# YunjiKim/Unsupervised-Keypoint-Learning-for-Guiding-Class-conditional-Video-Prediction

Measured on AMD Instinct MI355X. Metric: detector_translator train frames/sec @128x128 K=15, higher is better.
Workload: dtype f32

## Files before the change

### include/kpx.h

```cpp
#ifndef KPX_H
#define KPX_H

#include <stddef.h>
#include <stdint.h>

#ifdef __cplusplus
extern "C" {
#endif

#define KPX_EINVAL (-1)
#define KPX_ABI_VERSION 15

enum { KPX_ACT_NONE = 0, KPX_ACT_RELU = 1, KPX_ACT_LRELU = 2 , KPX_ACT_TANH = 3  };

int kpx_abi_version(void);

int kpx_reload_env(void);

enum { KPX_ARITH_F32 = 0, KPX_ARITH_BF16 = 1 };

size_t kpx_conv2d_fwd_workspace_bytes(int N, int Ho, int Wo, int Cin, int Cout, int KH, int KW);
int kpx_conv2d_fwd_f32(const float* x, int N, int Hi, int Wi, int Cin, int ldx,
                       const float* w_hwio, int KH, int KW, const float* bias,
                       float* y, int Ho, int Wo, int Cout, int ldy,
                       int stride, int pad_t, int pad_l, int act, int arith,
                       void* workspace, size_t workspace_bytes, void* stream);

typedef struct KpxWinoDesc { const float* w; float* u; int cin, cout, dgrad, reserved; } KpxWinoDesc;
size_t kpx_wino_u_bytes(int Cin, int Cout);
int kpx_wino_filter_transform_f32(const float* w_hwio, int Cin, int Cout, int dgrad, float* u, void* stream);
int kpx_wino_filter_transform_batch_f32(const void* descs, int n, void* stream);
int kpx_conv3x3_wino_eligible(int N, int H, int W, int K, int Nn, int ldin, const void* in);
int kpx_conv3x3_wino_f32(const float* in, int N, int H, int W, int K, int ldin, const float* u, const float* bias,
                         float* out, int Nn, int ldout, int act, float* tile_stats, const float* bn_y, int ld_bn_y,
                         const float* bn_beta, void* stream);
size_t kpx_conv3x3_wino_stats_tiles(int N, int H, int W);

size_t kpx_conv3x3_bf16s_weights_bytes(int K, int Nn);
int kpx_conv3x3_bf16s_eligible(int N, int H, int W, int K, int Nn, int ldin, const void* in);
int kpx_conv3x3_bf16s_stats_tiles(int N, int H, int W, int K, int Nn);
int kpx_conv3x3_bf16s_prepare_f32(const float* w_hwio, int Cin, int Cout, int dgrad, void* wf, void* stream);
int kpx_conv3x3_bf16s_prepare_batch_f32(const void* table, int ndesc, void* stream);
int kpx_conv3x3_bf16s(const void* in, int N, int H, int W, int K, int ldin, const void* wf, const float* bias,
                      void* out, int Nn, int ldout, int out_f32, int act, const void* mask, int ldmask, float* stats, void* stream);
int kpx_conv3x3_bf16s_bnbwd(const void* in, int N, int H, int W, int K, int ldin, const void* wf, void* out, int Nn, int ldout,
                            const void* bn_y, int ld_bn_y, const float* beta, float* stats, void* stream);

size_t kpx_conv2d_dgrad_workspace_bytes(int N, int Hi, int Wi, int Cin, int Cout, int KH, int KW, int stride);
int kpx_conv2d_dgrad_f32(const float* dy, int N, int Ho, int Wo, int Cout, int lddy,
                         const float* w_hwio, int KH, int KW,
                         float* dx, int Hi, int Wi, int Cin, int lddx,
                         int stride, int pad_t, int pad_l, int arith,
                         void* workspace, size_t workspace_bytes, void* stream);

int kpx_conv2d_dgrad_act_f32(const float* dy, int N, int Ho, int Wo, int Cout, int lddy,
                             const float* w_hwio, int KH, int KW,
                             float* dx, int Hi, int Wi, int Cin, int lddx,
                             int stride, int pad_t, int pad_l, int arith,
                             const float* y_in, int ld_y_in, int act_in,
                             void* workspace, size_t workspace_bytes, void* stream);

size_t kpx_conv2d_wgrad_workspace_bytes(int N, int Ho, int Wo, int Cin, int Cout, int KH, int KW);
int kpx_conv2d_wgrad_f32(const float* x, int N, int Hi, int Wi, int Cin, int ldx,
                         const float* dy, int Ho, int Wo, int Cout, int lddy,
                         float* dw_hwio, int KH, int KW, int stride, int pad_t, int pad_l, int arith,
                         void* workspace, size_t workspace_bytes, void* stream);

enum KpxWgradFamily {
    KPX_WGRAD_WSMALL = 0,
    KPX_WGRAD_WINO,
    KPX_WGRAD_ROWS_MERGED,
    KPX_WGRAD_ROWS,
    KPX_WGRAD_GEMM3,
    KPX_WGRAD_TAP_ROWS,
    KPX_WGRAD_GENERIC
};
int kpx_conv2d_wgrad_plan(const float* x, int N, int Hi, int Wi, int Cin, int ldx,
                          const float* dy, int Ho, int Wo, int Cout, int lddy,
                          int KH, int KW, int stride, int pad_t, int pad_l, int arith,
                          int* family, int* splits, size_t* workspace_bytes);

int kpx_act_bwd_f32(const float* dy, const float* y, float* dz, size_t n, int act, void* stream);

size_t kpx_chan_reduce_scratch_bytes(int C);
int kpx_chan_sum_f32(const float* x, size_t P, int C, int ldx, float* sum_out, void* scratch, void* stream);

size_t kpx_bn_train_scratch_bytes(int C, int groups);
int kpx_bn_train_fwd_f32(const float* x, size_t P, int groups, int C, int ldx, const float* tile_stats, size_t tiles_per_group,
                         float eps, const float* gamma, const float* beta, float* mean, float* invstd,
                         float* moving_mean, float* moving_var, float decay, float* y, int ldy, int act, void* scratch, void* stream);
int kpx_bn_train_bwd_f32(const float* dy, int lddy, const float* x, int ldx, size_t P, int groups, int C,
                         const float* mean, const float* invstd, const float* gamma, const float* beta, int act,
                         float* dx, int lddx, float* dgamma, float* dbeta, int accumulate,
                         const float* tile_stats, size_t tiles_per_group, void* scratch, void* stream);
int kpx_bn_train_fwd_bf16(const void* x, size_t P, int groups, int C, int ldx, const float* tile_stats, size_t tiles_per_group,
                          float eps, const float* gamma, const float* beta, float* mean, float* invstd,
                          float* moving_mean, float* moving_var, float decay, void* y, int ldy, int y_f32, int act, void* scratch, void* stream);
int kpx_bn_train_bwd_bf16(const void* dy, int lddy, int dy_f32, const void* x, int ldx, size_t P, int groups, int C,
                          const float* mean, const float* invstd, const float* gamma, const float* beta, int act,
                          void* dx, int lddx, float* dgamma, float* dbeta, int accumulate,
                          const float* tile_stats, size_t tiles_per_group, void* scratch, void* stream);
int kpx_bn_invstd_f32(const float* var, int C, float eps, float* invstd, void* stream);
int kpx_bn_apply_f32(const float* x, size_t P, int C, int ldx, const float* mean, const float* invstd,
                     const float* gamma, const float* beta, float* y, int ldy, int act, void* stream);
int kpx_bn_fold_conv_f32(const float* w, const float* bias, size_t rows, int C, const float* gamma, const float* beta,
                         const float* moving_mean, const float* moving_var, float eps, float* w_out, float* b_out, void* stream);

int kpx_conv3x3_wino43_eligible(int N, int H, int W, int K, int Nn, int ldin, const void* in_ptr);
size_t kpx_wino43_u_bytes(int Cin, int Cout);
int kpx_wino43_filter_transform_f32(const float* w_hwio, int Cin, int Cout, int dgrad, float* u, void* stream);
int kpx_wino43_filter_transform_batch_f32(const void* descs_dev, int n, void* stream);
int kpx_conv3x3_wino43_f32(const float* in, int N, int H, int W, int K, int ldin, const float* u, const float* bias,
                           float* out, int Nn, int ldout, int act, const float* mask_y, int ld_mask, float* pool_y, int ld_pool,
                           float* tile_stats, const float* bn_y, int ld_bn_y, const float* bn_beta, void* stream);
size_t kpx_conv3x3_wino43_stats_tiles(int N, int H, int W);
int kpx_conv3x3_wino43b_eligible(int N, int H, int W, int K, int Nn, int ldin, const void* in_ptr);
size_t kpx_wino43b_u_bytes(int Cin, int Cout);
int kpx_wino43b_filter_transform_f32(const float* w_hwio, int Cin, int Cout, int dgrad, void* u, void* stream);
int kpx_wino43b_filter_transform_batch_f32(const void* descs_dev, int n, void* stream);
int kpx_conv3x3_wino43b_f32(const float* in, int N, int H, int W, int K, int ldin, const void* u, const float* bias,
                            float* out, int Nn, int ldout, int act, const float* mask_y, int ld_mask, float* pool_y, int ld_pool,
                            float* tile_stats, const float* bn_y, int ld_bn_y, const float* bn_beta, void* stream);
int kpx_conv3x3_c16_eligible(int N, int H, int W, int K, int Nn, int ldin, int ldout, const void* in_ptr);
int kpx_conv3x3_c16_f32(const float* in, int N, int H, int W, int K, int ldin, const float* w_hwio, int dgrad, const float* bias,
                        float* out, int ldout, int act, float* tile_stats, void* stream);
int kpx_resize2x_fwd_f32(const float* x, int N, int H, int W, int C, int ldx, float* y, int ldy, void* stream);
int kpx_resize2x_bwd_f32(const float* dy, int N, int H, int W, int C, int lddy, float* dx, int lddx, void* stream);

int kpx_copy_channels_f32(const float* src, int ldsrc, float* dst, int lddst, size_t P, int C, void* stream);

size_t kpx_keypoint_head_scratch_bytes(int B, int H, int W, int K);
int kpx_keypoint_head_fwd_f32(const float* logits, int B, int H, int W, int K,
                              float* mu, float* prob_y, float* prob_x, void* scratch, void* stream);
int kpx_keypoint_head_bwd_f32(const float* dmu, const float* mu, const float* prob_y, const float* prob_x,
                              int B, int H, int W, int K, float* dlogits, void* stream);

size_t kpx_keypoint_head_proj_scratch_bytes(int B, int H, int W, int C, int K);
int kpx_keypoint_head_proj_eligible(int B, int H, int W, int C, int K);
int kpx_keypoint_head_proj_fwd_f32(const float* x, const float* wk, const float* bias, int B, int H, int W, int C, int K,
                                   float* mu, float* prob_y, float* prob_x, float* xs_y, float* xs_x, void* scratch, void* stream);
int kpx_keypoint_head_proj_bwd_f32(const float* dmu, const float* mu, const float* prob_y, const float* prob_x,
                                   const float* xs_y, const float* xs_x, const float* wk, int B, int H, int W, int C, int K,
                                   float* dx, float* dw, float* db, int accumulate, void* scratch, void* stream);

int kpx_gaussian_maps_fwd_f32(const float* mu, int B, int K, int H, int W, double inv_std, float* maps, int ldy, void* stream);
int kpx_gaussian_maps_bwd_f32(const float* dmaps, int lddy, const float* mu, int B, int K, int H, int W, double inv_std,
                              float* dmu, void* stream);

int kpx_point_maps_rgb_f32(const float* mu, int N, int K, int H, int W, double inv_std, const float* colors, float* out, void* stream);

int kpx_point_seq_strip_rgb_f32(const float* mu, int N, int T, int K, int H, int W, double inv_std, const float* colors, int recolour,
                                float* out, void* stream);

#define KPX_SUMMARY_SLICES 64
enum { KPX_PREMAP_IDENTITY = 0, KPX_PREMAP_X255 = 1, KPX_PREMAP_UNIT255 = 2, KPX_PREMAP_UNIT255_CLIP = 3 };
int kpx_summary_image_u8_f32(const float* x, int N, int H, int W, int C, int premap, float* work, uint8_t* out, void* stream);

int kpx_frame_metrics_f32(const float* a, const float* b, int N, int H, int W, int C, float L, int png8, float* out, void* stream);

size_t kpx_feature_pair_metrics_workspace_bytes(int N, int H, int W, int C);
int kpx_feature_pair_metrics_f32(const float* fa, const float* fb, int N, int H, int W, int C, float* work, float* out, void* stream);

int kpx_draw_moments_add_f32(const float* x, size_t n, uint32_t* sum, uint32_t* sumsq, void* stream);
int kpx_draw_diversity_f32(const uint32_t* sum, const uint32_t* sumsq, int N, int H, int W, int C, int D, float* div_mse ,
                           uint8_t* std_map , void* stream);
int kpx_keypoint_draw_metrics_f32(const float* pts , const float* real , int D, int N, int T, int K,
                                  float* l2 , float* div , void* stream);

#define KPX_SHEET_MAX_FRAMES 64
enum { KPX_SHEET_UNIT = 0, KPX_SHEET_RAW = 1 };
int kpx_sheet_paste_u8_f32(const float* src , int B, int F, int H, int W, int C, const int* frames , int J,
                           uint8_t* canvas , int rows, int cols, int row, int col, int premap, void* stream);

enum { KPX_RETARGET_HOLD = 0, KPX_RETARGET_ABSOLUTE = 1, KPX_RETARGET_RELATIVE = 2, KPX_RETARGET_RELATIVE_SCALED = 3 };
int kpx_points_retarget_f32(const float* src_first , const float* drv_first , const float* drv_seq ,
                            int B, int T, int K, int shift, int mode, float* out , void* stream);

int kpx_head_blend_fwd_f32(const float* im, const float* raw4, size_t P, float* final_out, float* crude_out, float* mask_out, void* stream);
int kpx_head_blend_bwd_f32(const float* dfinal, const float* im, const float* raw4, size_t P, float* draw4, void* stream);

int kpx_vgg_prep_fwd_f32(const float* rgb, size_t P, float* bgr, void* stream);
int kpx_vgg_prep_bwd_f32(const float* dbgr, size_t P, float* drgb, void* stream);
int kpx_vgg_prep_png8_f32(const float* rgb, size_t P, float* bgr, void* stream);

int kpx_maxpool2_fwd_f32(const float* x, int N, int H, int W, int C, float* y, void* stream);
int kpx_maxpool2_bwd_f32(const float* dy, const float* x, int N, int H, int W, int C, float* dx, void* stream);

int kpx_l1_pair_fwd_f32(const float* f, size_t half, float* loss_out, void* scratch, void* stream);
int kpx_l1_pair_bwd_f32(const float* f, size_t half, const float* gscale_dev, float gscale_host, float* dpred, void* stream);
int kpx_vgg_feat_bwd_f32(const float* f, size_t half, const float* gscale_dev, float gscale_host, const float* dy_pooled,
                         int B, int H, int W, int C, float* d, void* stream);

int kpx_sigmoid_xent_fwd_f32(const float* logits, size_t n0, float label0, size_t n1, float label1, float* loss_out, void* stream);
int kpx_sigmoid_xent_bwd_f32(const float* logits, size_t n0, float label0, size_t n1, float label1,
                             const float* gscale_dev, float gscale_host, float* dlogits, void* stream);

int kpx_adam_tf_flat_f32(float* p, const float* g, float* m, float* v, size_t n,
                         float alpha, float beta1, float beta2, float eps, float gscale, void* stream);
int kpx_adam_tf_flat_dev_alpha_f32(float* p, const float* g, float* m, float* v, size_t n,
                                   const float* alpha_dev, float beta1, float beta2, float eps, float gscale, void* stream);

int kpx_lstm_pointwise_f32(const float* gates, const float* c_prev, float forget_bias, float* c_out, float* h_out,
                           int B, int U, void* stream);
int kpx_tile_batch_f32(const float* src, int ldsrc, int B, int T, int pix, int C, float* dst, int lddst, void* stream);
int kpx_head_blend_tiled_fwd_f32(const float* im, const float* raw4, size_t P, int HW, int T, int clip,
                                 float* final_out, float* crude_out, float* mask_out, void* stream);

int kpx_fill_f32(float* p, size_t n, float value, void* stream);
int kpx_axpy_f32(float* y, const float* x, size_t n, float a, void* stream);

int kpx_lstm_pointwise_bwd_f32(const float* gates, const float* c_prev, const float* dh, const float* dc_in, float forget_bias,
                               float* dgates, float* dc_prev, int B, int U, void* stream);
int kpx_lstm_layer_fwd_f32(const float* x, int T, int B, int In, const float* kernel, const float* bias, int U,
// ... 78 lines not shown
```

### unsupervised-keypoint-learning-for-guiding-class-conditional-video-prediction_amd/_lib.py

```python
import ctypes
import os
from ctypes import c_double, c_float, c_int, c_size_t, c_void_p

import torch

_HERE = os.path.dirname(os.path.abspath(__file__))
LIB_PATH = os.environ.get('KPX_LIB') or os.path.join(_HERE, 'libkpx_hip.so')


class KpxError(RuntimeError):
    pass


if not os.path.exists(LIB_PATH):
    raise ImportError(
        'libkpx_hip.so not found at %s -- build it first: python -c "import __graft_entry__ as g; g.build()" '
        '(or `make -C %s/csrc`). There is no CPU / PyTorch fallback for the hot path.' % (LIB_PATH, _HERE))

lib = ctypes.CDLL(LIB_PATH)

P = c_void_p
ABI_VERSION = 15
SIGNATURES = {
    'kpx_abi_version': (c_int, []),
    'kpx_reload_env': (c_int, []),
    'kpx_conv2d_fwd_workspace_bytes': (c_size_t, [c_int, c_int, c_int, c_int, c_int, c_int, c_int]),
    'kpx_conv2d_fwd_f32': (c_int, [P, c_int, c_int, c_int, c_int, c_int, P, c_int, c_int, P,
                                   P, c_int, c_int, c_int, c_int, c_int, c_int, c_int, c_int, c_int, P, c_size_t, P]),
    'kpx_conv2d_dgrad_workspace_bytes': (c_size_t, [c_int, c_int, c_int, c_int, c_int, c_int, c_int, c_int]),
    'kpx_conv2d_dgrad_f32': (c_int, [P, c_int, c_int, c_int, c_int, c_int, P, c_int, c_int,
                                     P, c_int, c_int, c_int, c_int, c_int, c_int, c_int, c_int, P, c_size_t, P]),
    'kpx_conv2d_dgrad_act_f32': (c_int, [P, c_int, c_int, c_int, c_int, c_int, P, c_int, c_int,
                                         P, c_int, c_int, c_int, c_int, c_int, c_int, c_int, c_int, P, c_int, c_int, P, c_size_t, P]),
    'kpx_conv2d_wgrad_workspace_bytes': (c_size_t, [c_int, c_int, c_int, c_int, c_int, c_int, c_int]),
    'kpx_conv2d_wgrad_f32': (c_int, [P, c_int, c_int, c_int, c_int, c_int, P, c_int, c_int, c_int, c_int,
                                     P, c_int, c_int, c_int, c_int, c_int, c_int, P, c_size_t, P]),
    'kpx_conv2d_wgrad_plan': (c_int, [P, c_int, c_int, c_int, c_int, c_int, P, c_int, c_int, c_int, c_int,
                                      c_int, c_int, c_int, c_int, c_int, c_int, P, P, P]),
    'kpx_wino_u_bytes': (c_size_t, [c_int, c_int]),
    'kpx_wino_filter_transform_f32': (c_int, [P, c_int, c_int, c_int, P, P]),
    'kpx_wino_filter_transform_batch_f32': (c_int, [P, c_int, P]),
    'kpx_conv3x3_wino_eligible': (c_int, [c_int, c_int, c_int, c_int, c_int, c_int, P]),
    'kpx_conv3x3_wino_f32': (c_int, [P, c_int, c_int, c_int, c_int, c_int, P, P, P, c_int, c_int, c_int, P, P, c_int, P, P]),
    'kpx_conv3x3_c16_eligible': (c_int, [c_int, c_int, c_int, c_int, c_int, c_int, c_int, P]),
    'kpx_conv3x3_c16_f32': (c_int, [P, c_int, c_int, c_int, c_int, c_int, P, c_int, P, P, c_int, c_int, P, P]),
    'kpx_conv3x3_wino43_eligible': (c_int, [c_int, c_int, c_int, c_int, c_int, c_int, P]),
    'kpx_wino43_u_bytes': (c_size_t, [c_int, c_int]),
    'kpx_wino43_filter_transform_f32': (c_int, [P, c_int, c_int, c_int, P, P]),
    'kpx_wino43_filter_transform_batch_f32': (c_int, [P, c_int, P]),
    'kpx_conv3x3_wino43_f32': (c_int, [P, c_int, c_int, c_int, c_int, c_int, P, P, P, c_int, c_int, c_int, P, c_int, P, c_int, P, P, c_int, P, P]),
    'kpx_conv3x3_wino43b_eligible': (c_int, [c_int, c_int, c_int, c_int, c_int, c_int, P]),
    'kpx_wino43b_u_bytes': (c_size_t, [c_int, c_int]),
    'kpx_wino43b_filter_transform_f32': (c_int, [P, c_int, c_int, c_int, P, P]),
    'kpx_wino43b_filter_transform_batch_f32': (c_int, [P, c_int, P]),
    'kpx_conv3x3_wino43b_f32': (c_int, [P, c_int, c_int, c_int, c_int, c_int, P, P, P, c_int, c_int, c_int, P, c_int, P, c_int, P, P, c_int, P, P]),
    'kpx_conv3x3_wino43_stats_tiles': (c_size_t, [c_int, c_int, c_int]),
    'kpx_conv3x3_wino_stats_tiles': (c_size_t, [c_int, c_int, c_int]),
    'kpx_conv3x3_bf16s_weights_bytes': (c_size_t, [c_int, c_int]),
    'kpx_conv3x3_bf16s_eligible': (c_int, [c_int, c_int, c_int, c_int, c_int, c_int, P]),
    'kpx_conv3x3_bf16s_stats_tiles': (c_int, [c_int, c_int, c_int, c_int, c_int]),
    'kpx_conv3x3_bf16s_prepare_f32': (c_int, [P, c_int, c_int, c_int, P, P]),
    'kpx_conv3x3_bf16s_prepare_batch_f32': (c_int, [P, c_int, P]),
    'kpx_conv3x3_bf16s': (c_int, [P, c_int, c_int, c_int, c_int, c_int, P, P, P, c_int, c_int, c_int, c_int, P, c_int, P, P]),
    'kpx_conv2d_fwd_bf16': (c_int, [P, c_int, c_int, c_int, c_int, c_int, P, c_int, c_int, P, P, c_int, c_int, c_int, c_int, c_int, c_int, c_int, c_int, c_int, P, c_size_t, P]),
    'kpx_conv2d_dgrad_bf16': (c_int, [P, c_int, c_int, c_int, c_int, c_int, P, c_int, c_int, P, c_int, c_int, c_int, c_int, c_int, c_int, c_int, c_int, P, c_int, c_int, P, c_size_t, P]),
    'kpx_conv2d_wgrad_bf16': (c_int, [P, c_int, c_int, c_int, c_int, c_int, P, c_int, c_int, c_int, c_int, P, c_int, c_int, c_int, c_int, c_int, P, c_size_t, P]),
    'kpx_conv_image_fwd_bf16': (c_int, [P, c_int, c_int, c_int, c_int, P, c_int, c_int, P, P, c_int, c_int, c_int, c_int, c_int, c_int, c_int, c_int, P]),
    'kpx_conv_image_dgrad_bf16': (c_int, [P, c_int, c_int, c_int, c_int, c_int, P, c_int, c_int, P, c_int, c_int, c_int, c_int, c_int, c_int, c_int, P]),
    'kpx_conv_image_wgrad_bf16': (c_int, [P, c_int, c_int, c_int, c_int, c_int, P, c_int, c_int, c_int, c_int, P, c_int, c_int, c_int, c_int, c_int, P, c_size_t, P]),
    'kpx_conv3x3_wgrad_bf16_eligible': (c_int, [c_int, c_int, c_int, c_int, c_int, c_int, c_int, P, P]),
    'kpx_conv3x3_wgrad_bf16_workspace_bytes': (c_size_t, [c_int, c_int, c_int, c_int, c_int]),
    'kpx_conv3x3_wgrad_bf16': (c_int, [P, c_int, c_int, c_int, c_int, c_int, P, c_int, c_int, P, P, c_size_t, P]),
    'kpx_conv3x3_bf16s_bnbwd': (c_int, [P, c_int, c_int, c_int, c_int, c_int, P, P, c_int, c_int, P, c_int, P, P, P]),
    'kpx_cast_channels': (c_int, [P, c_int, P, c_int, c_size_t, c_int, c_int, P]),
    'kpx_chan_sum_bf16': (c_int, [P, c_size_t, c_int, c_int, P, P, P]),
    'kpx_bn_train_fwd_bf16': (c_int, [P, c_size_t, c_int, c_int, c_int, P, c_size_t, c_float, P, P, P, P, P, P, c_float, P, c_int, c_int, c_int, P, P]),
    'kpx_bn_train_bwd_bf16': (c_int, [P, c_int, c_int, P, c_int, c_size_t, c_int, c_int, P, P, P, P, c_int, P, c_int, P, P, c_int, P, c_size_t, P, P]),
    'kpx_act_bwd_bf16': (c_int, [P, P, P, c_size_t, c_int, P]),
    'kpx_resize2x_fwd_bf16': (c_int, [P, c_int, c_int, c_int, c_int, c_int, P, c_int, P]),
    'kpx_resize2x_bwd_bf16': (c_int, [P, c_int, c_int, c_int, c_int, c_int, P, c_int, P]),
    'kpx_maxpool2_fwd_bf16': (c_int, [P, c_int, c_int, c_int, c_int, P, P]),
    'kpx_vgg_feat_bwd_bf16': (c_int, [P, c_size_t, P, c_float, P, c_int, c_int, c_int, c_int, P, P]),
    'kpx_l1_pair_fwd_bf16': (c_int, [P, c_size_t, P, P, P]),
    'kpx_act_bwd_f32': (c_int, [P, P, P, c_size_t, c_int, P]),
    'kpx_chan_reduce_scratch_bytes': (c_size_t, [c_int]),
    'kpx_chan_sum_f32': (c_int, [P, c_size_t, c_int, c_int, P, P, P]),
    'kpx_bn_invstd_f32': (c_int, [P, c_int, c_float, P, P]),
    'kpx_bn_fold_conv_f32': (c_int, [P, P, c_size_t, c_int, P, P, P, P, c_float, P, P, P]),
    'kpx_bn_train_scratch_bytes': (c_size_t, [c_int, c_int]),
    'kpx_bn_train_fwd_f32': (c_int, [P, c_size_t, c_int, c_int, c_int, P, c_size_t, c_float, P, P, P, P, P, P, c_float, P, c_int, c_int, P, P]),
    'kpx_bn_train_bwd_f32': (c_int, [P, c_int, P, c_int, c_size_t, c_int, c_int, P, P, P, P, c_int, P, c_int, P, P, c_int, P, c_size_t, P, P]),
    'kpx_bn_apply_f32': (c_int, [P, c_size_t, c_int, c_int, P, P, P, P, P, c_int, c_int, P]),
    'kpx_resize2x_fwd_f32': (c_int, [P, c_int, c_int, c_int, c_int, c_int, P, c_int, P]),
    'kpx_resize2x_bwd_f32': (c_int, [P, c_int, c_int, c_int, c_int, c_int, P, c_int, P]),
    'kpx_copy_channels_f32': (c_int, [P, c_int, P, c_int, c_size_t, c_int, P]),
    'kpx_keypoint_head_scratch_bytes': (c_size_t, [c_int, c_int, c_int, c_int]),
    'kpx_keypoint_head_fwd_f32': (c_int, [P, c_int, c_int, c_int, c_int, P, P, P, P, P]),
    'kpx_keypoint_head_bwd_f32': (c_int, [P, P, P, P, c_int, c_int, c_int, c_int, P, P]),
    'kpx_keypoint_head_proj_scratch_bytes': (c_size_t, [c_int, c_int, c_int, c_int, c_int]),
    'kpx_keypoint_head_proj_eligible': (c_int, [c_int, c_int, c_int, c_int, c_int]),
    'kpx_keypoint_head_proj_fwd_f32': (c_int, [P, P, P, c_int, c_int, c_int, c_int, c_int, P, P, P, P, P, P, P]),
    'kpx_keypoint_head_proj_bwd_f32': (c_int, [P, P, P, P, P, P, P, c_int, c_int, c_int, c_int, c_int, P, P, P, c_int, P, P]),
    'kpx_gaussian_maps_fwd_f32': (c_int, [P, c_int, c_int, c_int, c_int, c_double, P, c_int, P]),
    'kpx_gaussian_maps_bwd_f32': (c_int, [P, c_int, P, c_int, c_int, c_int, c_int, c_double, P, P]),
    'kpx_point_maps_rgb_f32': (c_int, [P, c_int, c_int, c_int, c_int, c_double, P, P, P]),
    'kpx_point_seq_strip_rgb_f32': (c_int, [P, c_int, c_int, c_int, c_int, c_int, c_double, P, c_int, P, P]),
    'kpx_summary_image_u8_f32': (c_int, [P, c_int, c_int, c_int, c_int, c_int, P, P, P]),
    'kpx_frame_metrics_f32': (c_int, [P, P, c_int, c_int, c_int, c_int, c_float, c_int, P, P]),
    'kpx_feature_pair_metrics_workspace_bytes': (c_size_t, [c_int, c_int, c_int, c_int]),
    'kpx_feature_pair_metrics_f32': (c_int, [P, P, c_int, c_int, c_int, c_int, P, P, P]),
    'kpx_draw_moments_add_f32': (c_int, [P, c_size_t, P, P, P]),
    'kpx_draw_diversity_f32': (c_int, [P, P, c_int, c_int, c_int, c_int, c_int, P, P, P]),
    'kpx_keypoint_draw_metrics_f32': (c_int, [P, P, c_int, c_int, c_int, c_int, P, P, P]),
    'kpx_sheet_paste_u8_f32': (c_int, [P, c_int, c_int, c_int, c_int, c_int, P, c_int, P, c_int, c_int, c_int, c_int, c_int, P]),
    'kpx_points_retarget_f32': (c_int, [P, P, P, c_int, c_int, c_int, c_int, c_int, P, P]),
    'kpx_head_blend_fwd_f32': (c_int, [P, P, c_size_t, P, P, P, P]),
    'kpx_head_blend_bwd_f32': (c_int, [P, P, P, c_size_t, P, P]),
    'kpx_vgg_prep_fwd_f32': (c_int, [P, c_size_t, P, P]),
    'kpx_vgg_prep_bwd_f32': (c_int, [P, c_size_t, P, P]),
    'kpx_vgg_prep_png8_f32': (c_int, [P, c_size_t, P, P]),
    'kpx_maxpool2_fwd_f32': (c_int, [P, c_int, c_int, c_int, c_int, P, P]),
    'kpx_maxpool2_bwd_f32': (c_int, [P, P, c_int, c_int, c_int, c_int, P, P]),
    'kpx_l1_pair_fwd_f32': (c_int, [P, c_size_t, P, P, P]),
    'kpx_l1_pair_bwd_f32': (c_int, [P, c_size_t, P, c_float, P, P]),
    'kpx_vgg_feat_bwd_f32': (c_int, [P, c_size_t, P, c_float, P, c_int, c_int, c_int, c_int, P, P]),
    'kpx_sigmoid_xent_fwd_f32': (c_int, [P, c_size_t, c_float, c_size_t, c_float, P, P]),
    'kpx_sigmoid_xent_bwd_f32': (c_int, [P, c_size_t, c_float, c_size_t, c_float, P, c_float, P, P]),
    'kpx_adam_tf_flat_f32': (c_int, [P, P, P, P, c_size_t, c_float, c_float, c_float, c_float, c_float, P]),
    'kpx_adam_tf_flat_dev_alpha_f32': (c_int, [P, P, P, P, c_size_t, P, c_float, c_float, c_float, c_float, P]),
    'kpx_lstm_pointwise_f32': (c_int, [P, P, c_float, P, P, c_int, c_int, P]),
    'kpx_tile_batch_f32': (c_int, [P, c_int, c_int, c_int, c_int, c_int, P, c_int, P]),
    'kpx_head_blend_tiled_fwd_f32': (c_int, [P, P, c_size_t, c_int, c_int, c_int, P, P, P, P]),
    'kpx_fill_f32': (c_int, [P, c_size_t, c_float, P]),
    'kpx_axpy_f32': (c_int, [P, P, c_size_t, c_float, P]),
    'kpx_lstm_pointwise_bwd_f32': (c_int, [P, P, P, P, c_float, P, P, c_int, c_int, P]),
    'kpx_lstm_layer_fwd_f32': (c_int, [P, c_int, c_int, c_int, P, P, c_int, P, P, P, P, P, P, c_size_t, P]),
    'kpx_lstm_layer_bwd_f32': (c_int, [P, c_int, c_int, c_int, P, c_int, P, P, P, P, P, P, P, P, P, c_size_t, P]),
    'kpx_vae_sample_kl_fwd_f32': (c_int, [P, P, P, P, c_int, c_int, P]),
    'kpx_vae_sample_kl_bwd_f32': (c_int, [P, P, P, P, c_float, P, c_int, c_int, P]),
    'kpx_u8_to_unit_f32': (c_int, [P, c_size_t, P, P]),
    'kpx_crc32c_host': (ctypes.c_uint, [ctypes.c_uint, P, c_size_t]),
    'kpx_augment_geometry_u8': (c_int, [P, P, P, c_int, P, c_int, P, P, P]),
    'kpx_augment_filter_f32': (c_int, [P, P, P, c_int, P, P, P]),
    'kpx_keypoint_seq_augment_f32': (c_int, [P, P, P, c_int, c_int, c_int, P, P, P, P, P]),
}

for _name, (_res, _args) in SIGNATURES.items():
    try:
        _fn = getattr(lib, _name)
    except AttributeError as e:
        raise ImportError('libkpx_hip.so does not export %s (stale build?)' % _name) from e
    _fn.restype = _res
    _fn.argtypes = _args

if lib.kpx_abi_version() != ABI_VERSION:
    raise ImportError('libkpx_hip.so ABI version mismatch')


abi_calls = [0]


def check(rc, what):
    abi_calls[0] += 1
    if rc != 0:
        raise KpxError('%s failed with code %d (%s)' % (what, rc, 'bad argument' if rc == -1 else 'hipError %d' % -rc))
```

### unsupervised-keypoint-learning-for-guiding-class-conditional-video-prediction_amd/csrc/conv_gemm3.hip

```cpp
#include "kpx_internal.h"
#include "kpx_bf16.h"
#include "kpx_env.h"

#define G3_PITCH 80

template <int BM, int BN, int WM, int WN, bool BT, int TERMS, bool IO16 = false>
__global__ __launch_bounds__(WM * WN * 64, 2) void conv_gemm3_kernel(const ConvGeom g) {
    static_assert(!IO16 || TERMS == 1, "bf16 tensors carry one term");
    constexpr int NT = WM * WN * 64, BK = 32, ESZ = IO16 ? 2 : 4;
    constexpr int TM = BM / (WM * 32), TN = BN / (WN * 32);
    constexpr int APL = BM * G3_PITCH, BPL = BN * G3_PITCH;
    constexpr int ASZ = TERMS * APL;
    constexpr int RA = BM * 4 / NT;
    constexpr int KU = BN * 4 >= NT ? 8 : 4, CW = BN * 4 >= NT ? 4 : 2;
    constexpr int RB = BT ? BN * 32 / KU / NT : 16 * BN / CW / NT;
    static_assert(TM >= 1 && TN >= 1 && BM % (WM * 32) == 0 && BN % (WN * 32) == 0 && RA >= 1 && RB >= 1, "tile shape");
    static_assert(RA * NT == BM * 4 && RB * NT == (BT ? BN * 32 / KU : 16 * BN / CW), "whole units per thread");
    extern __shared__ __attribute__((aligned(16))) unsigned char smem[];
    unsigned char* const Asm = smem;
    unsigned char* const Bsm = smem + ASZ;

    const int t = threadIdx.x, lane = t & 63, wave = t >> 6;
    const int li = lane & 31, lh = lane >> 5;
    const int wm = wave / WN, wn = wave % WN;
    const ConvClass k = g.cls[blockIdx.y];
    const int L = kpx_xcd_remap(blockIdx.x, gridDim.x);
    if (L >= k.mt * g.nt) return;
    const int m0 = (L / g.nt) * BM, n0 = (L % g.nt) * BN;
    const int HW = k.Ha * k.Wa;
    const int wrow = wm * TM * 32, wcol = wn * TN * 32;

    const __amdgpu_buffer_rsrc_t rs_a = __builtin_amdgcn_make_buffer_rsrc(const_cast<float*>(g.x), 0,
                                            (int)((size_t)g.N * g.Hi * g.Wi * g.ldx * ESZ), 0x00020000);
    const size_t w_bytes = (size_t)g.KW * ((size_t)k.wr0 + (size_t)(k.Tr > 0 ? k.Tr - 1 : 0) * g.wrs + 1) * g.wts * 4;
    const __amdgpu_buffer_rsrc_t rs_b = __builtin_amdgcn_make_buffer_rsrc(const_cast<float*>(g.w), 0, (int)(w_bytes < 0x7fffffffu ? w_bytes : 0x7fffffffu), 0x00020000);

    int a_voff[RA], a_st[RA], a_k[RA];
    unsigned a_vm[RA];
#pragma unroll
    for (int i = 0; i < RA; ++i) {
        const int u = t + NT * i, oct = u & 3, row = u >> 2;
        const int m = m0 + row;
        const bool ok = m < k.M;
        const int mm = ok ? m : 0;
        const int n = mm / HW, rem = mm - n * HW, a = rem / k.Wa, b = rem - a * k.Wa;
        const int ih0 = a * g.isy + k.iy0, iw0 = b * g.isx + k.ix0;
        a_voff[i] = ((n * g.Hi * g.Wi + ih0 * g.Wi + iw0) * g.ldx + oct * 8) * ESZ;
        unsigned vm = 0;
        for (int r = 0; r < k.Tr; ++r)
            for (int q = 0; q < k.Tq; ++q)
                if (ok && (unsigned)(ih0 + r * g.ity) < (unsigned)g.Hi && (unsigned)(iw0 + q * g.itx) < (unsigned)g.Wi) vm |= 1u << (r * k.Tq + q);
        a_vm[i] = vm;
        a_st[i] = row * G3_PITCH + oct * 16;
        a_k[i] = oct * 8;
    }
    int b_voff[RB], b_st[RB], b_k[RB];
    bool b_ok[RB];
#pragma unroll
    for (int i = 0; i < RB; ++i) {
        const int u = t + NT * i;
        if (BT) {
            const int ku = u % (32 / KU), nn = u / (32 / KU), n = n0 + nn;
            b_ok[i] = n < g.Cout;
            b_voff[i] = (n * g.ldw + ku * KU) * 4;
            b_st[i] = nn * G3_PITCH + ku * KU * 2;
            b_k[i] = ku * KU;
        } else {
            const int kp = u & 15, nq = u >> 4, n = n0 + nq * CW;
            b_ok[i] = n < g.Cout;
            b_voff[i] = ((kp * 2) * g.ldw + n) * 4;
            b_st[i] = (nq * CW) * G3_PITCH + kp * 4;
            b_k[i] = kp * 2;
        }
    }
    int a_rd[TM], b_rd[TN];
#pragma unroll
    for (int i = 0; i < TM; ++i) a_rd[i] = (wrow + i * 32 + li) * G3_PITCH + lh * 16;
#pragma unroll
    for (int j = 0; j < TN; ++j) b_rd[j] = (wcol + j * 32 + li) * G3_PITCH + lh * 16;

    f32x16 acc[TM][TN];
#pragma unroll
    for (int i = 0; i < TM; ++i)
#pragma unroll
        for (int j = 0; j < TN; ++j)
#pragma unroll
            for (int r = 0; r < 16; ++r) acc[i][j][r] = 0.f;

    const int nck = (g.Cin + BK - 1) / BK;
    int nchunks = k.Tr * k.Tq * nck;
    int tr = 0, tq = 0, c0 = 0;
    if (g.ksplit > 1) {
        const int cps = (nchunks + g.ksplit - 1) / g.ksplit;
        const int cb = blockIdx.z * cps, ce = min(nchunks, cb + cps);
        const int tap0 = cb / nck;
        c0 = (cb - tap0 * nck) * BK; tr = tap0 / k.Tq; tq = tap0 - tr * k.Tq;
        nchunks = ce > cb ? ce - cb : 0;
    }
    int left = nchunks;

    f32x4 ra[RA][2], rb[RB][2];
    auto load_chunk = [&]() {
        const int a_off = (((tr * g.ity) * g.Wi + tq * g.itx) * g.ldx + c0) * ESZ;
        const int tapbit = tr * k.Tq + tq;
        const int tap = (k.wr0 + tr * g.wrs) * g.KW + (k.wq0 + tq * g.wqs);
        const int b_off = (tap * g.wts + (BT ? c0 : c0 * g.ldw)) * 4;
        const bool live = left > 0;
#pragma unroll
        for (int i = 0; i < RA; ++i) {
            const bool va = live & (((a_vm[i] >> tapbit) & 1u) != 0) & (c0 + a_k[i] < g.Cin);
            const int av = va ? a_voff[i] + a_off : KPX_BUF_OOB;
            ra[i][0] = __builtin_bit_cast(f32x4, __builtin_amdgcn_raw_buffer_load_b128(rs_a, av, 0, 0));
            if (!IO16) ra[i][1] = __builtin_bit_cast(f32x4, __builtin_amdgcn_raw_buffer_load_b128(rs_a, av + 16, 0, 0));
        }
#pragma unroll
        for (int i = 0; i < RB; ++i) {
            if (BT) {
                const bool vb = live & b_ok[i] & (c0 + b_k[i] < g.Cin);
                const int bv = vb ? b_voff[i] + b_off : KPX_BUF_OOB;
                rb[i][0] = __builtin_bit_cast(f32x4, __builtin_amdgcn_raw_buffer_load_b128(rs_b, bv, 0, 0));
                if (KU == 8) rb[i][1] = __builtin_bit_cast(f32x4, __builtin_amdgcn_raw_buffer_load_b128(rs_b, bv + 16, 0, 0));
            } else {
#pragma unroll
                for (int j = 0; j < 2; ++j) {
                    const bool vb = live & b_ok[i] & (c0 + b_k[i] + j < g.Cin);
                    const int bv = vb ? b_voff[i] + b_off + j * g.ldw * 4 : KPX_BUF_OOB;
                    if (CW == 4) rb[i][j] = __builtin_bit_cast(f32x4, __builtin_amdgcn_raw_buffer_load_b128(rs_b, bv, 0, 0));
                    else {
                        rb[i][j][0] = __builtin_bit_cast(float, __builtin_amdgcn_raw_buffer_load_b32(rs_b, bv, 0, 0));
                        rb[i][j][1] = __builtin_bit_cast(float, __builtin_amdgcn_raw_buffer_load_b32(rs_b, bv + 4, 0, 0));
                    }
                }
            }
        }
        --left;
        c0 += BK;
        const bool wrap = c0 >= g.Cin;
        c0 = wrap ? 0 : c0;
        tq += wrap ? 1 : 0;
        const bool wrapq = tq == k.Tq;
        tq = wrapq ? 0 : tq;
        tr += wrapq ? 1 : 0;
    };
    auto store_ab = [&]() {
#pragma unroll
        for (int i = 0; i < RA; ++i) {
            unsigned char* const Ab = Asm + a_st[i];
            if (IO16) { *reinterpret_cast<u32x4*>(Ab) = __builtin_bit_cast(u32x4, ra[i][0]); continue; }
            unsigned p[4][3];
            kpx_split2<TERMS>(ra[i][0][0], ra[i][0][1], p[0]); kpx_split2<TERMS>(ra[i][0][2], ra[i][0][3], p[1]);
            kpx_split2<TERMS>(ra[i][1][0], ra[i][1][1], p[2]); kpx_split2<TERMS>(ra[i][1][2], ra[i][1][3], p[3]);
#pragma unroll
            for (int tm = 0; tm < TERMS; ++tm) *reinterpret_cast<u32x4*>(Ab + tm * APL) = u32x4{p[0][tm], p[1][tm], p[2][tm], p[3][tm]};
        }
#pragma unroll
        for (int i = 0; i < RB; ++i) {
            unsigned char* const Bb = Bsm + b_st[i];
            if (BT) {
                unsigned p[4][3];
                kpx_split2<TERMS>(rb[i][0][0], rb[i][0][1], p[0]); kpx_split2<TERMS>(rb[i][0][2], rb[i][0][3], p[1]);
                if (KU == 8) {
                    kpx_split2<TERMS>(rb[i][1][0], rb[i][1][1], p[2]); kpx_split2<TERMS>(rb[i][1][2], rb[i][1][3], p[3]);
#pragma unroll
                    for (int tm = 0; tm < TERMS; ++tm) *reinterpret_cast<u32x4*>(Bb + tm * BPL) = u32x4{p[0][tm], p[1][tm], p[2][tm], p[3][tm]};
                } else {
#pragma unroll
                    for (int tm = 0; tm < TERMS; ++tm) *reinterpret_cast<u32x2*>(Bb + tm * BPL) = u32x2{p[0][tm], p[1][tm]};
                }
            } else {
#pragma unroll
                for (int c = 0; c < CW; ++c) {
                    unsigned p[3];
                    kpx_split2<TERMS>(rb[i][0][c], rb[i][1][c], p);
#pragma unroll
                    for (int tm = 0; tm < TERMS; ++tm) *reinterpret_cast<unsigned*>(Bb + tm * BPL + c * G3_PITCH) = p[tm];
                }
            }
        }
    };

    struct Frag { bf16x8 a[TM][TERMS], b[TN][TERMS]; };
    auto read_frag = [&](int s, Frag& f) {
        const unsigned char* const Ab = Asm + s * 32;
        const unsigned char* const Bb = Bsm + s * 32;
#pragma unroll
        for (int i = 0; i < TM; ++i)
#pragma unroll
            for (int tm = 0; tm < TERMS; ++tm) f.a[i][tm] = *reinterpret_cast<const bf16x8*>(Ab + tm * APL + a_rd[i]);
#pragma unroll
        for (int j = 0; j < TN; ++j)
#pragma unroll
            for (int tm = 0; tm < TERMS; ++tm) f.b[j][tm] = *reinterpret_cast<const bf16x8*>(Bb + tm * BPL + b_rd[j]);
    };
    auto mfma_frag = [&](const Frag& f) {
#pragma unroll
        for (int i = 0; i < TM; ++i)
#pragma unroll
            for (int j = 0; j < TN; ++j) {
                f32x16 c = acc[i][j];
                if (TERMS > 2) {
                    c = __builtin_amdgcn_mfma_f32_32x32x16_bf16(f.a[i][2], f.b[j][0], c, 0, 0, 0);
                    c = __builtin_amdgcn_mfma_f32_32x32x16_bf16(f.a[i][0], f.b[j][2], c, 0, 0, 0);
                    c = __builtin_amdgcn_mfma_f32_32x32x16_bf16(f.a[i][1], f.b[j][1], c, 0, 0, 0);
                }
                if (TERMS > 1) {
                    c = __builtin_amdgcn_mfma_f32_32x32x16_bf16(f.a[i][1], f.b[j][0], c, 0, 0, 0);
                    c = __builtin_amdgcn_mfma_f32_32x32x16_bf16(f.a[i][0], f.b[j][1], c, 0, 0, 0);
                }
                acc[i][j] = __builtin_amdgcn_mfma_f32_32x32x16_bf16(f.a[i][0], f.b[j][0], c, 0, 0, 0);
            }
    };
    auto chunk = [&]() {
        Frag f;
        read_frag(0, f);
        load_chunk();
        mfma_frag(f);
        read_frag(1, f);
        mfma_frag(f);
        __syncthreads();
        store_ab();
        __syncthreads();
    };

    load_chunk();
    store_ab();
    __syncthreads();
    for (int ch = 0; ch < nchunks; ++ch) chunk();

    int* rowpix = reinterpret_cast<int*>(smem);
    if (t < BM) {
        const int m = m0 + t;
        int pix = -1;
        if (m < k.M) {
            const int n = m / HW, rem = m - n * HW, a = rem / k.Wa, b = rem - a * k.Wa;
            pix = (n * g.Ho + a * g.osy + k.oy0) * g.Wo + b * g.osx + k.ox0;
        }
        rowpix[t] = pix;
    }
    __syncthreads();
    if (g.ksplit > 1) {
        float* wsl = g.ws + (size_t)blockIdx.z * g.ws_slab;
#pragma unroll
        for (int n = 0; n < TN; ++n) {
            const int col = n0 + wcol + n * 32 + li;
#pragma unroll
            for (int i = 0; i < TM; ++i)
#pragma unroll
                for (int r = 0; r < 16; ++r) {
                    const int pix = rowpix[wrow + i * 32 + (r & 3) + 8 * (r >> 2) + 4 * lh];
                    if (col < g.Cout && pix >= 0) wsl[(size_t)pix * g.Cout + col] = acc[i][n][r];
                }
        }
        return;
    }
#pragma unroll
    for (int n = 0; n < TN; ++n) {
        const int col = n0 + wcol + n * 32 + li;
        const bool cok = col < g.Cout;
        const float bv = (cok && g.bias) ? g.bias[col] : 0.f;
#pragma unroll
        for (int i = 0; i < TM; ++i) {
#pragma unroll
            for (int r = 0; r < 16; ++r) {
                const int pix = rowpix[wrow + i * 32 + (r & 3) + 8 * (r >> 2) + 4 * lh];
                if (cok && pix >= 0) {
                    float v = acc[i][n][r] + bv;
                    if (g.act == KPX_ACT_RELU) v = fmaxf(v, 0.f);
                    else if (g.act == KPX_ACT_LRELU) v = v > 0.f ? v : 0.01f * v;
                    else if (g.act == KPX_ACT_TANH) v = tanhf(v);
                    if (g.mul_y) {
                        const float my = (g.io16 & 4) ? kpx_float((unsigned)reinterpret_cast<const unsigned short*>(g.mul_y)[(size_t)pix * g.ld_mul + col] << 16)
                                                      : g.mul_y[(size_t)pix * g.ld_mul + col];
                        v *= kpx_act_grad_from_y(my, g.mul_act);
                    }
                    if (g.io16 & 2) { const __bf16 b = (__bf16)v; reinterpret_cast<unsigned short*>(g.y)[(size_t)pix * g.ldy + col] = __builtin_bit_cast(unsigned short, b); }
                    else g.y[(size_t)pix * g.ldy + col] = v;
                }
            }
        }
    }
}

static std::atomic<unsigned long long> g3_attr_mask{0};

template <int BN> struct g3_waves { static constexpr int wm = BN == 128 ? 2 : 4, wn = BN == 128 ? 4 : 2; };
template <int BM, int BN, bool BT, int TERMS, bool IO16 = false>
static int g3_launch_one(const ConvGeom& g, dim3 grid, hipStream_t s) {
    constexpr int lds = TERMS * (BM + BN) * G3_PITCH;
    hipLaunchKernelGGL((conv_gemm3_kernel<BM, BN, g3_waves<BN>::wm, g3_waves<BN>::wn, BT, TERMS, IO16>), grid, dim3(g3_waves<BN>::wm * g3_waves<BN>::wn * 64), lds, s, g);
    return kpx_launch_status();
}
template <int BM, int BN, bool BT, int TERMS, bool IO16 = false>
static hipError_t g3_set_attr() {
    constexpr int lds = TERMS * (BM + BN) * G3_PITCH;
    return hipFuncSetAttribute(reinterpret_cast<const void*>(conv_gemm3_kernel<BM, BN, g3_waves<BN>::wm, g3_waves<BN>::wn, BT, TERMS, IO16>),
                               hipFuncAttributeMaxDynamicSharedMemorySize, lds);
}

extern "C" __attribute__((visibility("hidden"))) int kpx_gemm3_eligible(const ConvGeom* g) {
    const KpxEnv* e = kpx_env();
    if (e->no_gemm3 || g->merge || !g->vecA || !g->vecB) return 0;
    if (g->Cin % 8 != 0 || g->Cin < 16 || g->Cout % 4 != 0 || g->Cout < 16 || g->ldx % 4 != 0 || g->ldw % 4 != 0) return 0;
    if ((g->io16 & 1) && (g->ldx % 8 != 0 || g->terms != 1)) return 0;
    return 1;
}

extern "C" __attribute__((visibility("hidden"))) int kpx_gemm3_launch(ConvGeom g, int bt, int terms, hipStream_t s) {
    if (kpx_first_use_on_device(&g3_attr_mask)) {
        hipError_t e = g3_set_attr<128, 128, false, 3>();
        if (e == hipSuccess) e = g3_set_attr<128, 128, true, 3>();
        if (e == hipSuccess) e = g3_set_attr<128, 64, false, 3>();
        if (e == hipSuccess) e = g3_set_attr<128, 64, true, 3>();
        if (e == hipSuccess) e = g3_set_attr<128, 128, false, 1>();
        if (e == hipSuccess) e = g3_set_attr<128, 128, true, 1>();
        if (e == hipSuccess) e = g3_set_attr<128, 64, false, 1>();
        if (e == hipSuccess) e = g3_set_attr<128, 64, true, 1>();
        if (e == hipSuccess) e = g3_set_attr<128, 128, false, 1, true>();
        if (e == hipSuccess) e = g3_set_attr<128, 128, true, 1, true>();
        if (e == hipSuccess) e = g3_set_attr<128, 64, false, 1, true>();
        if (e == hipSuccess) e = g3_set_attr<128, 64, true, 1, true>();
        if (e != hipSuccess) return -(int)e;
    }
    if (g.ncls <= 0) { g.ncls = 1; g.cls[0] = ConvClass{g.Ha, g.Wa, g.oy0, g.ox0, g.Tr, g.Tq, g.iy0, g.ix0, g.wr0, g.wq0, 0, 0}; }
    g.M = 0;
    for (int i = 0; i < g.ncls; ++i) { g.cls[i].M = g.N * g.cls[i].Ha * g.cls[i].Wa; if (g.cls[i].M > g.M) g.M = g.cls[i].M; }
    if (g.M <= 0 || g.Cout <= 0) return 0;
    const int BM = 128, BN = g.Cout > 64 ? 128 : 64;
    g.nt = (g.Cout + BN - 1) / BN;
    int mtmax = 0;
    for (int i = 0; i < g.ncls; ++i) { g.cls[i].mt = (g.cls[i].M + BM - 1) / BM; if (g.cls[i].mt > mtmax) mtmax = g.cls[i].mt; }
    g.mt = mtmax;
    const dim3 grid((unsigned)(g.mt * g.nt), (unsigned)g.ncls, (unsigned)(g.ksplit > 1 ? g.ksplit : 1));
#define G3_GO(bn, btv, tv) return g3_launch_one<128, bn, btv, tv>(g, grid, s)
    if (g.io16 & 1) {
        if (BN == 128) { if (bt) return g3_launch_one<128, 128, true, 1, true>(g, grid, s); return g3_launch_one<128, 128, false, 1, true>(g, grid, s); }
        if (bt) return g3_launch_one<128, 64, true, 1, true>(g, grid, s);
        return g3_launch_one<128, 64, false, 1, true>(g, grid, s);
    }
    if (terms == 1) {
        if (BN == 128) { if (bt) G3_GO(128, true, 1); else G3_GO(128, false, 1); }
        else { if (bt) G3_GO(64, true, 1); else G3_GO(64, false, 1); }
    }
    if (BN == 128) { if (bt) G3_GO(128, true, 3); else G3_GO(128, false, 3); }
    if (bt) G3_GO(64, true, 3);
    G3_GO(64, false, 3);
#undef G3_GO
}

template <int BM, int WM, int WN, int TERMS, bool IO16 = false>
__global__ __launch_bounds__(WM * WN * 64, 2) void conv_wgrad3_kernel(const WgradGeom g) {
    static_assert(!IO16 || TERMS == 1, "bf16 tensors carry one term");
    constexpr int NT = WM * WN * 64, BKP = 32, BN = BM, ESZ = IO16 ? 2 : 4;
    constexpr int TM = BM / (WM * 32), TN = BN / (WN * 32);
    constexpr int APL = BM * G3_PITCH, BPL = BN * G3_PITCH;
    constexpr int ASZ = TERMS * APL;
    static_assert(NT == 16 * (BM / 4), "one A unit and one B unit (2 pixels x 4 channels) per thread");
    extern __shared__ __attribute__((aligned(16))) unsigned char smem[];
    unsigned char* const Asm = smem;
    unsigned char* const Bsm = smem + ASZ;

    const int t = threadIdx.x, lane = t & 63, wave = t >> 6;
    const int li = lane & 31, lh = lane >> 5;
    const int wm = wave / WN, wn = wave % WN;
    int L = kpx_xcd_remap(blockIdx.x, gridDim.x);
    const int taps = g.KH * g.KW;
    const int kti = L % g.kt; L /= g.kt;
    const int cti = L % g.ct; L /= g.ct;
    const int tap = L % taps; L /= taps;
    const int split = L;
    const int r = tap / g.KW, q = tap - r * g.KW;
    const int cbase = cti * BM, kbase = kti * BN;
    const int pbeg = split * g.pps;
    const int pend = min(g.P, pbeg + g.pps);
    const int wrow = wm * TM * 32, wcol = wn * TN * 32;

    const __amdgpu_buffer_rsrc_t rs_a = __builtin_amdgcn_make_buffer_rsrc(const_cast<float*>(g.x), 0, (int)((size_t)g.N * g.Hi * g.Wi * g.ldx * ESZ), 0x00020000);
    const __amdgpu_buffer_rsrc_t rs_b = __builtin_amdgcn_make_buffer_rsrc(const_cast<float*>(g.dy), 0, (int)((size_t)g.P * g.lddy * ESZ), 0x00020000);
    const bool isB16 = IO16 && t >= NT / 2;
    const int tt = IO16 ? (isB16 ? t - NT / 2 : t) : t;
    const int kp = tt & 15, cq = tt >> 4;
    const int ac = cbase + cq * (IO16 ? 8 : 4), bc = kbase + cq * (IO16 ? 8 : 4);
    const bool a_cok = ac < g.Cin, b_cok = bc < g.Cout;
    const int a_st = (cq * (IO16 ? 8 : 4)) * G3_PITCH + kp * 4, b_st = a_st;
    int pn[2], pho[2], pwo[2];
#pragma unroll
    for (int j = 0; j < 2; ++j) {
        const int p = pbeg + 2 * kp + j;
        pn[j] = p / (g.Ho * g.Wo);
        const int rem = p - pn[j] * g.Ho * g.Wo;
        pho[j] = rem / g.Wo;
        pwo[j] = rem - pho[j] * g.Wo;
    }
    int p0 = pbeg + 2 * kp;

    int a_rd[TM], b_rd[TN];
#pragma unroll
    for (int i = 0; i < TM; ++i) a_rd[i] = (wrow + i * 32 + li) * G3_PITCH + lh * 16;
#pragma unroll
    for (int j = 0; j < TN; ++j) b_rd[j] = (wcol + j * 32 + li) * G3_PITCH + lh * 16;

    f32x16 acc[TM][TN];
#pragma unroll
    for (int i = 0; i < TM; ++i)
#pragma unroll
        for (int j = 0; j < TN; ++j)
#pragma unroll
            for (int e = 0; e < 16; ++e) acc[i][j][e] = 0.f;

    f32x4 ra[2], rb[2];
    auto load_chunk = [&]() {
#pragma unroll
        for (int j = 0; j < 2; ++j) {
            const int ih = pho[j] * g.stride + r - g.pad_t, iw = pwo[j] * g.stride + q - g.pad_l;
            const bool va = a_cok & (p0 + j < pend) & ((unsigned)ih < (unsigned)g.Hi) & ((unsigned)iw < (unsigned)g.Wi);
            const int av = va ? (((pn[j] * g.Hi + ih) * g.Wi + iw) * g.ldx + ac) * ESZ : KPX_BUF_OOB;
            const bool vb = b_cok & (p0 + j < pend);
            const int bv = vb ? ((p0 + j) * g.lddy + bc) * ESZ : KPX_BUF_OOB;
            if (IO16) {
                ra[j] = __builtin_bit_cast(f32x4, isB16 ? __builtin_amdgcn_raw_buffer_load_b128(rs_b, bv, 0, 0) : __builtin_amdgcn_raw_buffer_load_b128(rs_a, av, 0, 0));
            } else {
                ra[j] = __builtin_bit_cast(f32x4, __builtin_amdgcn_raw_buffer_load_b128(rs_a, av, 0, 0));
                rb[j] = __builtin_bit_cast(f32x4, __builtin_amdgcn_raw_buffer_load_b128(rs_b, bv, 0, 0));
            }
            pwo[j] += BKP;
            while (pwo[j] >= g.Wo) {
                pwo[j] -= g.Wo;
                if (++pho[j] == g.Ho) { pho[j] = 0; ++pn[j]; }
            }
        }
        p0 += BKP;
    };
    auto store_ab = [&]() {
        unsigned char* const Ab = Asm + a_st;
        unsigned char* const Bb = Bsm + b_st;
        if (IO16) {
            unsigned char* const Ob = isB16 ? Bb : Ab;
            const u32x4 v0 = __builtin_bit_cast(u32x4, ra[0]), v1 = __builtin_bit_cast(u32x4, ra[1]);
#pragma unroll
            for (int c = 0; c < 8; ++c) {
                const unsigned pr = (c & 1) ? __builtin_amdgcn_perm(v1[c >> 1], v0[c >> 1], 0x07060302u) : __builtin_amdgcn_perm(v1[c >> 1], v0[c >> 1], 0x05040100u);
                *reinterpret_cast<unsigned*>(Ob + c * G3_PITCH) = pr;
            }
            return;
        }
#pragma unroll
        for (int c = 0; c < 4; ++c) {
            unsigned pa[3], pb[3];
            kpx_split2<TERMS>(ra[0][c], ra[1][c], pa);
            kpx_split2<TERMS>(rb[0][c], rb[1][c], pb);
#pragma unroll
            for (int tm = 0; tm < TERMS; ++tm) {
                *reinterpret_cast<unsigned*>(Ab + tm * APL + c * G3_PITCH) = pa[tm];
                *reinterpret_cast<unsigned*>(Bb + tm * BPL + c * G3_PITCH) = pb[tm];
            }
        }
    };
    struct Frag { bf16x8 a[TM][TERMS], b[TN][TERMS]; };
    auto read_frag = [&](int s, Frag& f) {
        const unsigned char* const Ab = Asm + s * 32;
        const unsigned char* const Bb = Bsm + s * 32;
#pragma unroll
        for (int i = 0; i < TM; ++i)
#pragma unroll
            for (int tm = 0; tm < TERMS; ++tm) f.a[i][tm] = *reinterpret_cast<const bf16x8*>(Ab + tm * APL + a_rd[i]);
#pragma unroll
        for (int j = 0; j < TN; ++j)
#pragma unroll
            for (int tm = 0; tm < TERMS; ++tm) f.b[j][tm] = *reinterpret_cast<const bf16x8*>(Bb + tm * BPL + b_rd[j]);
    };
    auto mfma_frag = [&](const Frag& f) {
#pragma unroll
        for (int i = 0; i < TM; ++i)
#pragma unroll
            for (int j = 0; j < TN; ++j) {
                f32x16 c = acc[i][j];
                if (TERMS > 2) {
                    c = __builtin_amdgcn_mfma_f32_32x32x16_bf16(f.a[i][2], f.b[j][0], c, 0, 0, 0);
                    c = __builtin_amdgcn_mfma_f32_32x32x16_bf16(f.a[i][0], f.b[j][2], c, 0, 0, 0);
                    c = __builtin_amdgcn_mfma_f32_32x32x16_bf16(f.a[i][1], f.b[j][1], c, 0, 0, 0);
                }
                if (TERMS > 1) {
                    c = __builtin_amdgcn_mfma_f32_32x32x16_bf16(f.a[i][1], f.b[j][0], c, 0, 0, 0);
                    c = __builtin_amdgcn_mfma_f32_32x32x16_bf16(f.a[i][0], f.b[j][1], c, 0, 0, 0);
                }
                acc[i][j] = __builtin_amdgcn_mfma_f32_32x32x16_bf16(f.a[i][0], f.b[j][0], c, 0, 0, 0);
// ... 60 lines not shown
```

### unsupervised-keypoint-learning-for-guiding-class-conditional-video-prediction_amd/csrc/conv_geom.h

```cpp
#pragma once
#include "kpx_common.h"

struct ConvClass { int Ha, Wa, oy0, ox0, Tr, Tq, iy0, ix0, wr0, wq0, M, mt; };

struct ConvGeom {
    const float* x; float* y; const float* w; const float* bias;
    int N, Hi, Wi, Cin, ldx;
    int Ho, Wo, Cout, ldy;
    int Ha, Wa;
    int osy, oy0, osx, ox0;
    int isy, iy0, isx, ix0;
    int Tr, Tq, ity, itx;
    int wr0, wrs, wq0, wqs, KW;
    int wts, ldw;
    int act, vecA, vecB;
    int M, mt, nt;
    ConvClass cls[4]; int ncls;
    int ksplit; float* ws;
    size_t ws_slab;
    const float* mul_y; int ld_mul, mul_act;
    int terms;
    int merge;
    int io16;
};


struct WgradGeom {
    const float* x; const float* dy; float* out;
    int N, Hi, Wi, Cin, ldx;
    int Ho, Wo, Cout, lddy;
    int KH, KW, stride, pad_t, pad_l;
    int P, S, pps;
    int ct, kt;
    int vecA, vecB;
    int terms;
    int merge;
    size_t slab;
    int io16;
};
```

### unsupervised-keypoint-learning-for-guiding-class-conditional-video-prediction_amd/csrc/conv_igemm.hip

```cpp
#include "kpx_internal.h"
#include "kpx_bf16.h"

__device__ __attribute__((aligned(16))) float kpx_zero16[4] = {0.f, 0.f, 0.f, 0.f};

template <int BM, int BN, int WM, int WN, bool BT, bool VEC, bool MERGE, bool TAIL>
__global__ __launch_bounds__(WM * WN * 64) void conv_igemm_kernel(const ConvGeom g) {
    constexpr int NT = WM * WN * 64;
    constexpr int BK = 32;
    constexpr int TM = BM / (WM * 32), TN = BN / (WN * 32);
    constexpr int RA = (BM * 8) / NT;
    constexpr int RB = (BN * 8 + NT - 1) / NT;
    constexpr int BU = BN * 8;
    constexpr int ASZ = BM * BK, BSZ = BK * BN;
    static_assert(TM >= 1 && TN >= 1 && RA >= 1 && (BM * 8) % NT == 0, "tile/wave shape");
    __shared__ __attribute__((aligned(16))) float As[2 * ASZ];
    __shared__ __attribute__((aligned(16))) float Bs[2 * BSZ];

    const int t = threadIdx.x, lane = t & 63, wave = t >> 6;
    const int li = lane & 31, lh = lane >> 5;
    const int wm = wave / WN, wn = wave % WN;
    const ConvClass k = g.cls[blockIdx.y];
    const int L = kpx_xcd_remap(blockIdx.x, gridDim.x);
    if (L >= k.mt * g.nt) return;
    const int m0 = (L / g.nt) * BM, n0 = (L % g.nt) * BN;
// ... 302 lines not shown
    const size_t npix = (size_t)g.N * g.Ho * g.Wo;
    size_t nb = (npix * (g.Cout / 4) + 255) / 256; if (nb > 2048) nb = 2048;
    hipLaunchKernelGGL(splitk_reduce_kernel, dim3((unsigned)nb), dim3(256), 0, s, (const float*)g.ws, g.ws_slab, g.ksplit, npix, g.Cout,
                       g.bias, g.act, g.y, g.ldy, g.mul_y, g.ld_mul, g.mul_act, g.io16);
    return kpx_launch_status();
}

template <bool BT, bool VEC, bool MERGE, bool TAIL>
static int launch_gather_conv_v(ConvGeom g, hipStream_t s) {
    if (g.ncls <= 0) { g.ncls = 1; g.cls[0] = ConvClass{g.Ha, g.Wa, g.oy0, g.ox0, g.Tr, g.Tq, g.iy0, g.ix0, g.wr0, g.wq0, 0, 0}; }
    g.M = 0;
    for (int i = 0; i < g.ncls; ++i) { g.cls[i].M = g.N * g.cls[i].Ha * g.cls[i].Wa; if (g.cls[i].M > g.M) g.M = g.cls[i].M; }
    if (g.M <= 0 || g.Cout <= 0) return 0;
    if (g.ksplit > 1) {
        const int BMs = 128, BNs = g.Cout > 64 ? 128 : 64;
        g.nt = (g.Cout + BNs - 1) / BNs;
        int mtmax = 0;
        for (int i = 0; i < g.ncls; ++i) { g.cls[i].mt = (g.cls[i].M + BMs - 1) / BMs; if (g.cls[i].mt > mtmax) mtmax = g.cls[i].mt; }
        g.mt = mtmax;
        const dim3 nblk((unsigned)(g.mt * g.nt), (unsigned)g.ncls, (unsigned)g.ksplit);
        if (BNs == 128) hipLaunchKernelGGL((conv_igemm_kernel<128, 128, 2, 4, BT, VEC, MERGE, TAIL>), nblk, dim3(512), 0, s, g);
        else hipLaunchKernelGGL((conv_igemm_kernel<128, 64, 4, 2, BT, VEC, MERGE, TAIL>), nblk, dim3(512), 0, s, g);
        const int rc = kpx_launch_status();
        return rc ? rc : launch_splitk_reduce(g, s);
    }
    int BN = 128;
    {
        auto pad = [&](int b) { return (g.Cout + b - 1) / b * b; };
        if (pad(64) < pad(BN)) BN = 64;
        if (pad(32) < pad(BN)) BN = 32;
    }
    auto blocks = [&](int bm, int bn) {
        long b = 0;
        for (int i = 0; i < g.ncls; ++i) b += (long)((g.cls[i].M + bm - 1) / bm) * ((g.Cout + bn - 1) / bn);
        return b;
    };
    int BM = 128;
    if (BN != 32) {
        struct Cand { int bm, bn, occ; double eff; };
        const Cand c128[] = {{128, 128, 2, 1.0}, {64, 128, 3, 0.92}, {128, 64, 3, 0.92}, {64, 64, 5, 0.85}};
        const Cand c64[] = {{128, 64, 3, 1.0}, {64, 64, 5, 0.92}};
        const Cand* cs = BN == 128 ? c128 : c64;
        const int nc = BN == 128 ? 4 : 2;
        double best = -1;
        for (int i = 0; i < nc; ++i) {
            const long nb = blocks(cs[i].bm, cs[i].bn), slots = 256L * cs[i].occ;
            const long rounds = (nb + slots - 1) / slots;
            const double score = cs[i].eff * (double)nb / (double)(rounds * slots);
            if (score > best) { best = score; BM = cs[i].bm; BN = cs[i].bn; }
        }
    }
    g.nt = (g.Cout + BN - 1) / BN;
    int mtmax = 0;
    for (int i = 0; i < g.ncls; ++i) { g.cls[i].mt = (g.cls[i].M + BM - 1) / BM; if (g.cls[i].mt > mtmax) mtmax = g.cls[i].mt; }
    g.mt = mtmax;
    const dim3 nblk((unsigned)(g.mt * g.nt), (unsigned)g.ncls);
#define KPX_LAUNCH(bm, bn, wm, wn) \
    hipLaunchKernelGGL((conv_igemm_kernel<bm, bn, wm, wn, BT, VEC, MERGE, TAIL>), nblk, dim3((wm) * (wn) * 64), 0, s, g)
    if (BM == 128 && BN == 128) KPX_LAUNCH(128, 128, 2, 4);
    else if (BM == 64 && BN == 128) KPX_LAUNCH(64, 128, 2, 4);
    else if (BM == 128 && BN == 64) KPX_LAUNCH(128, 64, 4, 2);
    else if (BM == 64 && BN == 64) KPX_LAUNCH(64, 64, 2, 2);
    else KPX_LAUNCH(128, 32, 4, 1);
#undef KPX_LAUNCH
    return kpx_launch_status();
}

template <bool BT>
static int launch_gather_conv(const ConvGeom& g, hipStream_t s) {
    if (kpx_gemm3_eligible(&g)) {
        int rc = kpx_gemm3_launch(g, BT ? 1 : 0, g.terms == 1 ? 1 : 3, s);
        return rc || g.ksplit <= 1 ? rc : launch_splitk_reduce(g, s);
    }
    if (g.io16) return KPX_EINVAL;
    if (g.merge) return launch_gather_conv_v<false, false, true, true>(g, s);
    if (g.vecA && g.vecB) {
        if (g.Cin % 4 == 0 && g.Cout % 4 == 0) return launch_gather_conv_v<BT, true, false, false>(g, s);
        return launch_gather_conv_v<BT, true, false, true>(g, s);
    }
    return launch_gather_conv_v<BT, false, false, true>(g, s);
}

__global__ __launch_bounds__(256) void conv_small_cout_kernel(const ConvGeom g) {
    const int lane = threadIdx.x & 63;
    const int m = blockIdx.x * 4 + (threadIdx.x >> 6);
    if (m >= g.M) return;
    const int HW = g.Ha * g.Wa;
    const int n = m / HW, rem = m - n * HW, a = rem / g.Wa, b = rem - a * g.Wa;
    float acc[4] = {0.f, 0.f, 0.f, 0.f};
    for (int tr = 0; tr < g.Tr; ++tr) {
        const int ih = a * g.isy + g.iy0 + tr * g.ity;
        if ((unsigned)ih >= (unsigned)g.Hi) continue;
        for (int tq = 0; tq < g.Tq; ++tq) {
            const int iw = b * g.isx + g.ix0 + tq * g.itx;
            if ((unsigned)iw >= (unsigned)g.Wi) continue;
            const float* xp = g.x + ((size_t)(n * g.Hi + ih) * g.Wi + iw) * g.ldx;
            const float* wp = g.w + (size_t)((g.wr0 + tr * g.wrs) * g.KW + g.wq0 + tq * g.wqs) * g.wts;
            for (int c = lane * 4; c < g.Cin; c += 256) {
                const f32x4 xv = *reinterpret_cast<const f32x4*>(xp + c);
#pragma unroll
                for (int j = 0; j < 4; ++j)
                    for (int o = 0; o < g.Cout; ++o) acc[o] = fmaf(xv[j], wp[(size_t)(c + j) * g.ldw + o], acc[o]);
            }
        }
    }
    const int pix = (n * g.Ho + a * g.osy + g.oy0) * g.Wo + b * g.osx + g.ox0;
    for (int o = 0; o < g.Cout; ++o) {
        float v = kpx_wave_sum(acc[o]);
        if (lane == 0) {
            v += g.bias ? g.bias[o] : 0.f;
            if (g.act == KPX_ACT_RELU) v = fmaxf(v, 0.f);
            else if (g.act == KPX_ACT_LRELU) v = v > 0.f ? v : 0.01f * v;
            else if (g.act == KPX_ACT_TANH) v = tanhf(v);
            g.y[(size_t)pix * g.ldy + o] = v;
        }
    }
}
static int launch_small_cout(ConvGeom g, hipStream_t s) {
    g.M = g.N * g.Ha * g.Wa;
    hipLaunchKernelGGL(conv_small_cout_kernel, dim3((unsigned)((g.M + 3) / 4)), dim3(256), 0, s, g);
    return kpx_launch_status();
}

static int dgrad_splitk_plan(int N, int Hi, int Wi, int Cin, int Cout, int KH, int KW, int stride) {
    const long Mcls = (long)N * ((Hi + stride - 1) / stride) * ((Wi + stride - 1) / stride);
    const long chunks = (long)(KH / stride > 0 ? KH / stride : 1) * (KW / stride > 0 ? KW / stride : 1) * ((Cout + 31) / 32);
    if (Cin % 4 != 0) return 1;
    int S = conv_splitk_plan(Mcls * stride * stride, Cin, chunks);
    return S;
}

static inline size_t wino_ws_bytes(int Cin, int Cout) {
    const size_t a = (size_t)((Cin + 7) & ~7) * ((Cout + 31) & ~31), b = (size_t)((Cout + 7) & ~7) * ((Cin + 31) & ~31);
    return 16 * 4 * (a > b ? a : b);
}

extern "C" size_t kpx_conv2d_fwd_workspace_bytes(int N, int Ho, int Wo, int Cin, int Cout, int KH, int KW) {
    if (Cin % 4 != 0) return 0;
    const int S = conv_splitk_plan((long)N * Ho * Wo, Cout, (long)KH * KW * ((Cin + 31) / 32));
    size_t b = S > 1 ? (size_t)S * N * Ho * Wo * Cout * 4 : 0;
    if (KH == 3 && KW == 3 && b < wino_ws_bytes(Cin, Cout)) b = wino_ws_bytes(Cin, Cout);
    return b;
}

extern "C" size_t kpx_conv2d_dgrad_workspace_bytes(int N, int Hi, int Wi, int Cin, int Cout, int KH, int KW, int stride) {
    const int S = dgrad_splitk_plan(N, Hi, Wi, Cin, Cout, KH, KW, stride);
    size_t b = S > 1 ? (size_t)S * N * Hi * Wi * Cin * 4 : 0;
    if (KH == 3 && KW == 3 && stride == 1 && b < wino_ws_bytes(Cin, Cout)) b = wino_ws_bytes(Cin, Cout);
    return b;
}

static int fwd_impl(const float* x, int N, int Hi, int Wi, int Cin, int ldx, const float* w, int KH, int KW, const float* bias,
                    float* y, int Ho, int Wo, int Cout, int ldy, int stride, int pad_t, int pad_l, int act, int arith, int io16,
                    void* workspace, size_t workspace_bytes, void* stream);
extern "C" int kpx_conv2d_fwd_f32(const float* x, int N, int Hi, int Wi, int Cin, int ldx,
                                  const float* w, int KH, int KW, const float* bias,
                                  float* y, int Ho, int Wo, int Cout, int ldy,
                                  int stride, int pad_t, int pad_l, int act, int arith, void* workspace, size_t workspace_bytes, void* stream) {
    return fwd_impl(x, N, Hi, Wi, Cin, ldx, w, KH, KW, bias, y, Ho, Wo, Cout, ldy, stride, pad_t, pad_l, act, arith, 0, workspace, workspace_bytes, stream);
}
extern "C" int kpx_conv2d_fwd_bf16(const void* x, int N, int Hi, int Wi, int Cin, int ldx, const float* w, int KH, int KW, const float* bias,
                                   void* y, int y_f32, int Ho, int Wo, int Cout, int ldy, int stride, int pad_t, int pad_l, int act,
                                   void* workspace, size_t workspace_bytes, void* stream) {
    if (ldx % 8 || !kpx_aligned16(x) || !kpx_aligned16(y) || (!y_f32 && ldy % 4)) return KPX_EINVAL;
    return fwd_impl((const float*)x, N, Hi, Wi, Cin, ldx, w, KH, KW, bias, (float*)y, Ho, Wo, Cout, ldy, stride, pad_t, pad_l, act, KPX_ARITH_BF16, 1 | (y_f32 ? 0 : 2),
                    workspace, workspace_bytes, stream);
}
static int fwd_impl(const float* x, int N, int Hi, int Wi, int Cin, int ldx, const float* w, int KH, int KW, const float* bias,
                    float* y, int Ho, int Wo, int Cout, int ldy, int stride, int pad_t, int pad_l, int act, int arith, int io16,
                    void* workspace, size_t workspace_bytes, void* stream) {
    if (!x || !w || !y || N <= 0 || Hi <= 0 || Wi <= 0 || Cin <= 0 || Cout <= 0 || Ho <= 0 || Wo <= 0 ||
        KH <= 0 || KW <= 0 || stride <= 0 || ldx < Cin || ldy < Cout || act < 0 || act > 3 || arith < 0 || arith > 1)
        return KPX_EINVAL;
    if (io16) goto gather;
    if (KH == 3 && KW == 3 && stride == 1 && pad_t == 1 && pad_l == 1 && Ho == Hi && Wo == Wi && act != KPX_ACT_TANH &&
        kpx_conv3x3_c16_eligible(N, Hi, Wi, Cin, Cout, ldx, ldy, x))
        return kpx_conv3x3_c16_f32(x, N, Hi, Wi, Cin, ldx, w, 0, bias, y, ldy, act, nullptr, stream);
    if (Cout <= 4 && Cin <= 128 && (size_t)N * Ho * Wo >= 65536) {
        const int rc = kpx_conv_few_fwd(x, N, Hi, Wi, Cin, ldx, w, KH, KW, bias, y, Ho, Wo, Cout, ldy, stride, pad_t, pad_l, act, kpx_stream(stream));
        if (rc != -2) return rc;
    }
    if (KH == 3 && KW == 3 && stride == 1 && pad_t == 1 && pad_l == 1 && Ho == Hi && Wo == Wi && act != KPX_ACT_TANH && kpx_aligned16(w) &&
        workspace && workspace_bytes >= wino_ws_bytes(Cin, Cout) && kpx_wino_eligible(N, Hi, Wi, Cin, Cout, ldx, x))
        return kpx_wino_conv3x3(x, N, Hi, Wi, Cin, ldx, w, Cin, Cout, 0, bias, act, y, Cout, ldy, (float*)workspace, kpx_stream(stream));
    if (Cin <= 4 && ldx == Cin && stride <= 2 && Cout <= 64 && Ho * Wo >= 256) {
        const int rc = kpx_conv_rgb_fwd(x, N, Hi, Wi, Cin, w, KH, KW, bias, y, Ho, Wo, Cout, ldy, stride, pad_t, pad_l, act, kpx_stream(stream));
        if (rc != -2) return rc;
    }
gather:
    ConvGeom g{};
    g.x = x; g.y = y; g.w = w; g.bias = bias; g.io16 = io16;
    g.N = N; g.Hi = Hi; g.Wi = Wi; g.Cin = Cin; g.ldx = ldx;
    g.Ho = Ho; g.Wo = Wo; g.Cout = Cout; g.ldy = ldy;
    g.Ha = Ho; g.Wa = Wo; g.osy = 1; g.oy0 = 0; g.osx = 1; g.ox0 = 0;
    g.isy = stride; g.iy0 = -pad_t; g.isx = stride; g.ix0 = -pad_l;
    g.Tr = KH; g.Tq = KW; g.ity = 1; g.itx = 1;
    g.wr0 = 0; g.wrs = 1; g.wq0 = 0; g.wqs = 1; g.KW = KW;
    g.wts = Cin * Cout; g.ldw = Cout; g.act = act; g.terms = arith == KPX_ARITH_BF16 ? 1 : 3;
    g.vecA = (ldx % 4 == 0) && kpx_aligned16(x);
    g.vecB = (Cout % 4 == 0) && kpx_aligned16(w);
    if (Cin % 4 != 0 && ldx == Cin && KW > 1 && KW * Cin <= 64) {
        g.merge = Cin; g.Tq = 1; g.KW = 1; g.Cin = KW * Cin; g.wts = KW * Cin * Cout; g.vecA = 0;
    }
    if (io16 && !kpx_gemm3_eligible(&g)) return KPX_EINVAL;
    if (!io16 && Cout <= 4 && Cin % 4 == 0 && Cin >= 256 && g.vecA && g.vecB == (Cout == 4))
        return launch_small_cout(g, kpx_stream(stream));
    if (g.vecA && g.vecB && !g.merge && Cin % 4 == 0) {
        const int S = conv_splitk_plan((long)N * Ho * Wo, Cout, (long)KH * KW * ((Cin + 31) / 32));
        g.ws_slab = (size_t)N * Ho * Wo * Cout;
        if (S > 1 && workspace && workspace_bytes >= (size_t)S * g.ws_slab * 4) { g.ksplit = S; g.ws = (float*)workspace; }
    }
    return launch_gather_conv<false>(g, kpx_stream(stream));
}

static int dgrad_impl(const float* dy, int N, int Ho, int Wo, int Cout, int lddy, const float* w, int KH, int KW,
                      float* dx, int Hi, int Wi, int Cin, int lddx, int stride, int pad_t, int pad_l, int arith,
                      const float* y_in, int ld_y_in, int act_in, void* workspace, size_t workspace_bytes, void* stream, int io16 = 0);

extern "C" int kpx_conv2d_dgrad_f32(const float* dy, int N, int Ho, int Wo, int Cout, int lddy,
                                    const float* w, int KH, int KW,
                                    float* dx, int Hi, int Wi, int Cin, int lddx,
                                    int stride, int pad_t, int pad_l, int arith, void* workspace, size_t workspace_bytes, void* stream) {
    return dgrad_impl(dy, N, Ho, Wo, Cout, lddy, w, KH, KW, dx, Hi, Wi, Cin, lddx, stride, pad_t, pad_l, arith, nullptr, 0, KPX_ACT_NONE,
                      workspace, workspace_bytes, stream);
}

extern "C" int kpx_conv2d_dgrad_act_f32(const float* dy, int N, int Ho, int Wo, int Cout, int lddy,
                                        const float* w, int KH, int KW,
                                        float* dx, int Hi, int Wi, int Cin, int lddx,
                                        int stride, int pad_t, int pad_l, int arith,
                                        const float* y_in, int ld_y_in, int act_in, void* workspace, size_t workspace_bytes, void* stream) {
    if (!y_in || ld_y_in < Cin || (act_in != KPX_ACT_RELU && act_in != KPX_ACT_LRELU)) return KPX_EINVAL;
    return dgrad_impl(dy, N, Ho, Wo, Cout, lddy, w, KH, KW, dx, Hi, Wi, Cin, lddx, stride, pad_t, pad_l, arith, y_in, ld_y_in, act_in,
                      workspace, workspace_bytes, stream);
}

extern "C" int kpx_conv_image_fwd_bf16(const float* x, int N, int Hi, int Wi, int Cin, const float* w, int KH, int KW, const float* bias,
                                       void* y, int Ho, int Wo, int Cout, int ldy, int stride, int pad_t, int pad_l, int act, void* stream) {
    if (!x || !w || !y || N <= 0 || Hi <= 0 || Wi <= 0 || Cin <= 0 || Cin > 4 || Cout <= 0 || Cout > 64 || Ho * Wo < 256 || stride < 1 || stride > 2 ||
        ldy < Cout || act < 0 || act > 3)
        return KPX_EINVAL;
    const int rc = kpx_conv_rgb_fwd(x, N, Hi, Wi, Cin, w, KH, KW, bias, (float*)y, Ho, Wo, Cout, ldy, stride, pad_t, pad_l, act, kpx_stream(stream), 1);
    return rc == -2 ? KPX_EINVAL : rc;
}
extern "C" int kpx_conv_image_dgrad_bf16(const void* dy, int N, int Ho, int Wo, int Cout, int lddy, const float* w, int KH, int KW,
                                         float* dx, int Hi, int Wi, int Cin, int lddx, int stride, int pad_t, int pad_l, void* stream) {
    if (!dy || !w || !dx || N <= 0 || Hi <= 0 || Wi <= 0 || Cin <= 0 || Cin > 4 || Cout <= 0 || Ho <= 0 || Wo <= 0 || lddy < Cout || lddx < Cin)
        return KPX_EINVAL;
    const int rc = kpx_conv_rgb_dgrad((const float*)dy, N, Ho, Wo, Cout, lddy, w, KH, KW, dx, Hi, Wi, Cin, lddx, stride, pad_t, pad_l, kpx_stream(stream), 1);
    return rc == -2 ? KPX_EINVAL : rc;
}

extern "C" int kpx_conv2d_dgrad_bf16(const void* dy, int N, int Ho, int Wo, int Cout, int lddy, const float* w, int KH, int KW,
                                     void* dx, int dx_f32, int Hi, int Wi, int Cin, int lddx, int stride, int pad_t, int pad_l,
                                     const void* y_in, int ld_y_in, int act_in, void* workspace, size_t workspace_bytes, void* stream) {
    if (lddy % 8 || !kpx_aligned16(dy) || !kpx_aligned16(dx) || (!dx_f32 && lddx % 4)) return KPX_EINVAL;
    if (y_in && (ld_y_in < Cin || (act_in != KPX_ACT_RELU && act_in != KPX_ACT_LRELU))) return KPX_EINVAL;
    return dgrad_impl((const float*)dy, N, Ho, Wo, Cout, lddy, w, KH, KW, (float*)dx, Hi, Wi, Cin, lddx, stride, pad_t, pad_l, KPX_ARITH_BF16,
                      (const float*)y_in, ld_y_in, y_in ? act_in : KPX_ACT_NONE, workspace, workspace_bytes, stream, 1 | (dx_f32 ? 0 : 2) | (y_in ? 4 : 0));
}

static int dgrad_act_pass(int rc, float* dx, int N, int Hi, int Wi, int Cin, int lddx, const float* y_in, int ld_y_in, int act_in, void* stream) {
    if (rc || !y_in) return rc;
    if (lddx != Cin || ld_y_in != Cin) return KPX_EINVAL;
    return kpx_act_bwd_f32(dx, y_in, dx, (size_t)N * Hi * Wi * Cin, act_in, stream);
}

static int dgrad_impl(const float* dy, int N, int Ho, int Wo, int Cout, int lddy, const float* w, int KH, int KW,
                      float* dx, int Hi, int Wi, int Cin, int lddx, int stride, int pad_t, int pad_l, int arith,
                      const float* y_in, int ld_y_in, int act_in, void* workspace, size_t workspace_bytes, void* stream, int io16) {
    if (!dy || !w || !dx || N <= 0 || Hi <= 0 || Wi <= 0 || Cin <= 0 || Cout <= 0 || Ho <= 0 || Wo <= 0 ||
        KH <= 0 || KW <= 0 || stride <= 0 || lddy < Cout || lddx < Cin || arith < 0 || arith > 1)
        return KPX_EINVAL;
    if (stride > 2) return KPX_EINVAL;
    if (io16) goto gather;
    if (KH == 3 && KW == 3 && stride == 1 && pad_t == 1 && pad_l == 1 && Ho == Hi && Wo == Wi &&
        kpx_conv3x3_c16_eligible(N, Hi, Wi, Cout, Cin, lddy, lddx, dy))
        return dgrad_act_pass(kpx_conv3x3_c16_f32(dy, N, Hi, Wi, Cout, lddy, w, 1, nullptr, dx, lddx, KPX_ACT_NONE, nullptr, stream),
                              dx, N, Hi, Wi, Cin, lddx, y_in, ld_y_in, act_in, stream);
    if (Cin <= 4) {
        const int rc = kpx_conv_rgb_dgrad(dy, N, Ho, Wo, Cout, lddy, w, KH, KW, dx, Hi, Wi, Cin, lddx, stride, pad_t, pad_l, kpx_stream(stream));
        if (rc != -2) return dgrad_act_pass(rc, dx, N, Hi, Wi, Cin, lddx, y_in, ld_y_in, act_in, stream);
    }
    if (KH == 3 && KW == 3 && stride == 1 && pad_t == 1 && pad_l == 1 && Ho == Hi && Wo == Wi &&
        workspace && workspace_bytes >= wino_ws_bytes(Cin, Cout) && kpx_wino_eligible(N, Hi, Wi, Cout, Cin, lddy, dy))
        return dgrad_act_pass(kpx_wino_conv3x3(dy, N, Hi, Wi, Cout, lddy, w, Cin, Cout, 1, nullptr, KPX_ACT_NONE, dx, Cin, lddx, (float*)workspace, kpx_stream(stream)),
                              dx, N, Hi, Wi, Cin, lddx, y_in, ld_y_in, act_in, stream);
gather:
    ConvGeom g{};
    g.x = dy; g.y = dx; g.w = w; g.bias = nullptr; g.io16 = io16;
    g.mul_y = y_in; g.ld_mul = ld_y_in; g.mul_act = act_in;
    g.N = N; g.Hi = Ho; g.Wi = Wo; g.Cin = Cout; g.ldx = lddy;
    g.Ho = Hi; g.Wo = Wi; g.Cout = Cin; g.ldy = lddx;
    g.osy = stride; g.osx = stride;
    g.isy = 1; g.ity = -1; g.isx = 1; g.itx = -1;
    g.wrs = stride; g.wqs = stride; g.KW = KW;
    g.wts = Cin * Cout; g.ldw = Cout; g.act = KPX_ACT_NONE; g.terms = arith == KPX_ARITH_BF16 ? 1 : 3;
    g.vecA = (lddy % 4 == 0) && kpx_aligned16(dy);
    g.vecB = (Cout % 4 == 0) && kpx_aligned16(w);
    g.ncls = 0;
    for (int ph = 0; ph < stride; ++ph) {
        for (int pw = 0; pw < stride; ++pw) {
            if (ph >= Hi || pw >= Wi) continue;
            ConvClass c{};
            c.Ha = (Hi - ph + stride - 1) / stride; c.Wa = (Wi - pw + stride - 1) / stride;
            c.oy0 = ph; c.ox0 = pw;
            const int r0 = (ph + pad_t) % stride, q0 = (pw + pad_l) % stride;
            c.Tr = r0 < KH ? (KH - r0 + stride - 1) / stride : 0;
            c.Tq = q0 < KW ? (KW - q0 + stride - 1) / stride : 0;
            if (c.Tr == 0 || c.Tq == 0) { c.Tr = 0; c.Tq = 0; }
            c.iy0 = (ph + pad_t - r0) / stride;
            c.ix0 = (pw + pad_l - q0) / stride;
            c.wr0 = r0; c.wq0 = q0;
            g.cls[g.ncls++] = c;
        }
    }
    if (io16 && !kpx_gemm3_eligible(&g)) return KPX_EINVAL;
    if (g.vecA && g.vecB && Cout % 4 == 0) {
        const int S = dgrad_splitk_plan(N, Hi, Wi, Cin, Cout, KH, KW, stride);
        g.ws_slab = (size_t)N * Hi * Wi * Cin;
        if (S > 1 && workspace && workspace_bytes >= (size_t)S * g.ws_slab * 4) { g.ksplit = S; g.ws = (float*)workspace; }
    }
    return launch_gather_conv<true>(g, kpx_stream(stream));
}
```

### unsupervised-keypoint-learning-for-guiding-class-conditional-video-prediction_amd/csrc/pointwise.hip

```cpp
#include "kpx_bf16.h"

#define KPX_MAX_BLOCKS 2048
#define KPX_RED_BLOCKS 1024

static inline unsigned grid_for(size_t work_items) {
    size_t b = (work_items + 255) / 256;
    if (b < 1) b = 1;
    if (b > KPX_MAX_BLOCKS) b = KPX_MAX_BLOCKS;
    return (unsigned)b;
}

__global__ __launch_bounds__(256) void fill_kernel(float* p, size_t n, float v) {
    for (size_t i = (size_t)blockIdx.x * 256 + threadIdx.x; i < n; i += (size_t)gridDim.x * 256) p[i] = v;
}
extern "C" int kpx_fill_f32(float* p, size_t n, float value, void* stream) {
    if (!p) return KPX_EINVAL;
    if (n == 0) return 0;
    hipLaunchKernelGGL(fill_kernel, dim3(grid_for(n)), dim3(256), 0, kpx_stream(stream), p, n, value);
    return kpx_launch_status();
}

__global__ __launch_bounds__(256) void u8_to_unit_kernel(const unsigned char* __restrict__ src, size_t n, float* __restrict__ dst) {
    for (size_t i = (size_t)blockIdx.x * 256 + threadIdx.x; i < n; i += (size_t)gridDim.x * 256) dst[i] = kpx_u8_to_unit(src[i]);
}
// ... 57 lines not shown

struct RedArgs {
    const float* x; int ldx; const float* dy; int lddy;
    size_t P; int C;
    const float* mean; const float* invstd; const float* gamma; const float* beta; int act;
    double* part;
    size_t part_gstride;
};

template <int MODE, bool VEC>
__global__ __launch_bounds__(256) void chan_reduce_kernel(const RedArgs a) {
    constexpr int W = VEC ? 4 : 1;
    const int G = VEC ? a.C / 4 : a.C;
    const int Gb = G < 256 ? G : 256;
    const int PPB = 256 / Gb;
    const int t = threadIdx.x;
    const int cgl = t % Gb, prow = t / Gb;
    const int cg = blockIdx.y * Gb + cgl;
    const bool active = prow < PPB && cg < G;
    const int grp = blockIdx.z;
    const float* const gx = a.x + (size_t)grp * a.P * a.ldx;
    const float* const gdy = MODE == 2 ? a.dy + (size_t)grp * a.P * a.lddy : nullptr;
    double s0[W], s1[W];
#pragma unroll
    for (int j = 0; j < W; ++j) { s0[j] = 0.0; s1[j] = 0.0; }
    float mu[W], is[W], ga[W], be[W];
    if (MODE == 2 && active) {
#pragma unroll
        for (int j = 0; j < W; ++j) {
            const int c = cg * W + j;
            mu[j] = a.mean[grp * a.C + c]; is[j] = a.invstd[grp * a.C + c]; ga[j] = a.gamma[c]; be[j] = a.beta[c];
        }
    }
    if (active) {
        constexpr int U = VEC ? 4 : 1;
        const size_t step = (size_t)gridDim.x * PPB;
        for (size_t p0 = (size_t)blockIdx.x * PPB + prow; p0 < a.P; p0 += step * U) {
            float xv[U][W], gv[U][W];
#pragma unroll
            for (int u = 0; u < U; ++u) {
                const size_t p = p0 + u * step;
                const bool in = p < a.P;
                if (VEC) {
                    const f32x4 v = in ? *reinterpret_cast<const f32x4*>(gx + p * a.ldx + cg * 4) : f32x4{0.f, 0.f, 0.f, 0.f};
#pragma unroll
                    for (int j = 0; j < W; ++j) xv[u][j] = v[j];
                    if (MODE == 2) {
                        const f32x4 d = in ? *reinterpret_cast<const f32x4*>(gdy + p * a.lddy + cg * 4) : f32x4{0.f, 0.f, 0.f, 0.f};
#pragma unroll
                        for (int j = 0; j < W; ++j) gv[u][j] = d[j];
                    }
                } else {
                    xv[u][0] = gx[p * a.ldx + cg];
                    if (MODE == 2) gv[u][0] = gdy[p * a.lddy + cg];
                }
            }
#pragma unroll
            for (int u = 0; u < U; ++u) {
                if (p0 + u * step >= a.P) break;
#pragma unroll
                for (int j = 0; j < W; ++j) {
                    if (MODE == 0) s0[j] += (double)xv[u][j];
                    if (MODE == 1) { s0[j] += (double)xv[u][j]; s1[j] += (double)xv[u][j] * (double)xv[u][j]; }
                    if (MODE == 2) {
                        const float xh = (xv[u][j] - mu[j]) * is[j];
                        const float yv = fmaf(xh, ga[j], be[j]);
                        const float dz = (a.act == KPX_ACT_RELU && !(yv > 0.f)) ? 0.f : gv[u][j];
                        s0[j] += (double)dz; s1[j] += (double)dz * (double)xh;
                    }
                }
            }
        }
    }
    __shared__ double sm[2][256 * W];
#pragma unroll
    for (int j = 0; j < W; ++j) { sm[0][t * W + j] = s0[j]; sm[1][t * W + j] = s1[j]; }
    __syncthreads();
    if (t < Gb && blockIdx.y * Gb + t < G) {
#pragma unroll
        for (int j = 0; j < W; ++j) {
            double r0 = 0.0, r1 = 0.0;
            for (int pr = 0; pr < PPB; ++pr) { r0 += sm[0][(pr * Gb + t) * W + j]; r1 += sm[1][(pr * Gb + t) * W + j]; }
            const int c = (blockIdx.y * Gb + t) * W + j;
            double* const gp = a.part + (size_t)grp * a.part_gstride;
            gp[((size_t)blockIdx.x * 2 + 0) * a.C + c] = r0;
            gp[((size_t)blockIdx.x * 2 + 1) * a.C + c] = r1;
        }
    }
}

static dim3 chan_reduce_grid(size_t P, int G, int groups, int* nb_out) {
    const int Gb = G < 256 ? G : 256, PPB = 256 / Gb;
    size_t nb = P / ((size_t)PPB * 8);
    if (nb < 1) nb = 1;
    if (nb > KPX_RED_BLOCKS) nb = KPX_RED_BLOCKS;
    *nb_out = (int)nb;
    return dim3((unsigned)nb, (unsigned)((G + Gb - 1) / Gb), (unsigned)groups);
}

static int launch_chan_reduce(int mode, RedArgs a, int* nb_out, hipStream_t s, int groups = 1) {
    const bool vec = (a.C % 4 == 0) && (a.ldx % 4 == 0) && (((uintptr_t)a.x) & 15) == 0 &&
                     (mode != 2 || ((a.lddy % 4 == 0) && (((uintptr_t)a.dy) & 15) == 0));
    const dim3 grid = chan_reduce_grid(a.P, vec ? a.C / 4 : a.C, groups, nb_out), block(256);
#define KPX_RED(M) \
    do { if (vec) hipLaunchKernelGGL((chan_reduce_kernel<M, true>), grid, block, 0, s, a); \
         else hipLaunchKernelGGL((chan_reduce_kernel<M, false>), grid, block, 0, s, a); } while (0)
    if (mode == 0) KPX_RED(0); else if (mode == 1) KPX_RED(1); else KPX_RED(2);
#undef KPX_RED
    return kpx_launch_status();
}

extern "C" size_t kpx_chan_reduce_scratch_bytes(int C) {
    const size_t c = (size_t)(C > 0 ? C : 1);
    return (size_t)KPX_RED_BLOCKS * 2 * c * sizeof(double) + ((2 * c * sizeof(float) + 15) & ~(size_t)15);
}

__device__ __forceinline__ void chan_wave_sums(const double* part, int nb, const float* ts, size_t t0, size_t ntiles, bool on, int C, int c,
                                               double (&w)[2][4]) {
    const int t = threadIdx.x & 255;
    double a0 = 0.0, a1 = 0.0;
    if (on) {
        if (ts) {
            for (size_t b = t; b < ntiles; b += 256) {
                a0 += (double)ts[((t0 + b) * 2) * C + c];
                a1 += (double)ts[((t0 + b) * 2 + 1) * C + c];
            }
        } else {
            for (int b = t; b < nb; b += 256) {
                a0 += part[((size_t)b * 2) * C + c];
                a1 += part[((size_t)b * 2 + 1) * C + c];
            }
        }
    }
    a0 = kpx_wave_sum_d(a0);
    a1 = kpx_wave_sum_d(a1);
    __syncthreads();
    if ((t & 63) == 0) { w[0][t >> 6] = a0; w[1][t >> 6] = a1; }
    __syncthreads();
}
__device__ __forceinline__ double chan_sum4(const double (&w)[4]) { return (w[0] + w[1]) + (w[2] + w[3]); }

__global__ __launch_bounds__(256) void chan_sum_finalize_kernel(const double* part, int nb, int C, float* out) {
    const int c = blockIdx.x;
    __shared__ double sm[2][4];
    chan_wave_sums(part, nb, nullptr, 0, 0, true, C, c, sm);
    if (threadIdx.x == 0) out[c] = (float)chan_sum4(sm[0]);
}
extern "C" int kpx_chan_sum_f32(const float* x, size_t P, int C, int ldx, float* sum_out, void* scratch, void* stream) {
    if (!x || !sum_out || !scratch || C <= 0 || ldx < C || P == 0) return KPX_EINVAL;
    RedArgs a{}; a.x = x; a.ldx = ldx; a.P = P; a.C = C; a.part = (double*)scratch;
    int nb; int rc = launch_chan_reduce(0, a, &nb, kpx_stream(stream));
    if (rc) return rc;
    hipLaunchKernelGGL(chan_sum_finalize_kernel, dim3(C), dim3(256), 0, kpx_stream(stream), (const double*)scratch, nb, C, sum_out);
    return kpx_launch_status();
}

__global__ void bn_invstd_kernel(const float* var, int C, float eps, float* invstd) {
    const int c = blockIdx.x * blockDim.x + threadIdx.x;
    if (c < C) invstd[c] = 1.0f / sqrtf(var[c] + eps);
}
extern "C" int kpx_bn_invstd_f32(const float* var, int C, float eps, float* invstd, void* stream) {
    if (!var || !invstd || C <= 0) return KPX_EINVAL;
    hipLaunchKernelGGL(bn_invstd_kernel, dim3((C + 63) / 64), dim3(64), 0, kpx_stream(stream), var, C, eps, invstd);
    return kpx_launch_status();
}

__global__ __launch_bounds__(256) void bn_apply_kernel(const float* x, size_t P, int C, int ldx, const float* mean, const float* invstd,
                                                       const float* gamma, const float* beta, float* y, int ldy, int act) {
    x += (size_t)blockIdx.z * P * ldx; y += (size_t)blockIdx.z * P * ldy; mean += blockIdx.z * C; invstd += blockIdx.z * C;
    const size_t total = P * (size_t)C;
    for (size_t i = (size_t)blockIdx.x * 256 + threadIdx.x; i < total; i += (size_t)gridDim.x * 256) {
        const size_t p = i / C;
        const int c = (int)(i - p * C);
        const float xh = (x[p * ldx + c] - mean[c]) * invstd[c];
        float r = fmaf(xh, gamma[c], beta[c]);
        if (act == KPX_ACT_RELU) r = fmaxf(r, 0.f);
        y[p * ldy + c] = r;
    }
}
__global__ __launch_bounds__(256) void bn_bwd_apply_kernel(const float* dy, int lddy, const float* x, int ldx, size_t P, int C,
                                                           const float* mean, const float* invstd, const float* gamma, const float* beta,
                                                           int act, const float* sums, float inv_count, float* dx, int lddx) {
    dy += (size_t)blockIdx.z * P * lddy; x += (size_t)blockIdx.z * P * ldx; dx += (size_t)blockIdx.z * P * lddx;
    mean += blockIdx.z * C; invstd += blockIdx.z * C; sums += blockIdx.z * 2 * C;
    const size_t total = P * (size_t)C;
    for (size_t i = (size_t)blockIdx.x * 256 + threadIdx.x; i < total; i += (size_t)gridDim.x * 256) {
        const size_t p = i / C;
        const int c = (int)(i - p * C);
        const float xh = (x[p * ldx + c] - mean[c]) * invstd[c];
        const float yv = fmaf(xh, gamma[c], beta[c]);
        const float dz = (act == KPX_ACT_RELU && !(yv > 0.f)) ? 0.f : dy[p * lddy + c];
        dx[p * lddx + c] = gamma[c] * invstd[c] * (dz - sums[c] * inv_count - xh * (sums[C + c] * inv_count));
    }
}
__global__ __launch_bounds__(256) void bn_apply_strip_kernel(const float* __restrict__ x, size_t P, int C, int ldx, const float* __restrict__ mean,
                                                             const float* __restrict__ invstd, const float* __restrict__ gamma, const float* __restrict__ beta,
                                                             float* __restrict__ y, int ldy, int act) {
    const int G = C >> 2, Gb = G < 256 ? G : 256, PPB = 256 / Gb;
    const int t = threadIdx.x, cgl = t % Gb, prow = t / Gb;
    const int cg = blockIdx.y * Gb + cgl;
    if (prow >= PPB || cg >= G) return;
    x += (size_t)blockIdx.z * P * ldx; y += (size_t)blockIdx.z * P * ldy; mean += blockIdx.z * C; invstd += blockIdx.z * C;
    const f32x4 mu = *reinterpret_cast<const f32x4*>(mean + cg * 4), is = *reinterpret_cast<const f32x4*>(invstd + cg * 4);
    const f32x4 ga = *reinterpret_cast<const f32x4*>(gamma + cg * 4), be = *reinterpret_cast<const f32x4*>(beta + cg * 4);
    const size_t step = (size_t)gridDim.x * PPB;
    for (size_t p0 = (size_t)blockIdx.x * PPB + prow; p0 < P; p0 += step * 4) {
        f32x4 v[4];
#pragma unroll
        for (int u = 0; u < 4; ++u) { const size_t p = p0 + u * step; if (p < P) v[u] = *reinterpret_cast<const f32x4*>(x + p * ldx + cg * 4); }
#pragma unroll
        for (int u = 0; u < 4; ++u) {
            const size_t p = p0 + u * step;
            if (p >= P) break;
            f32x4 r;
#pragma unroll
            for (int j = 0; j < 4; ++j) {
                const float xh = (v[u][j] - mu[j]) * is[j];
                r[j] = fmaf(xh, ga[j], be[j]);
                if (act == KPX_ACT_RELU) r[j] = fmaxf(r[j], 0.f);
            }
            *reinterpret_cast<f32x4*>(y + p * ldy + cg * 4) = r;
        }
    }
}
__global__ __launch_bounds__(256) void bn_bwd_apply_strip_kernel(const float* __restrict__ dy, int lddy, const float* __restrict__ x, int ldx, size_t P, int C,
                                                                 const float* __restrict__ mean, const float* __restrict__ invstd, const float* __restrict__ gamma,
                                                                 const float* __restrict__ beta, int act, const float* __restrict__ sums, float inv_count,
                                                                 float* __restrict__ dx, int lddx) {
    const int G = C >> 2, Gb = G < 256 ? G : 256, PPB = 256 / Gb;
    const int t = threadIdx.x, cgl = t % Gb, prow = t / Gb;
    const int cg = blockIdx.y * Gb + cgl;
    if (prow >= PPB || cg >= G) return;
    dy += (size_t)blockIdx.z * P * lddy; x += (size_t)blockIdx.z * P * ldx; dx += (size_t)blockIdx.z * P * lddx;
    mean += blockIdx.z * C; invstd += blockIdx.z * C; sums += blockIdx.z * 2 * C;
    const f32x4 mu = *reinterpret_cast<const f32x4*>(mean + cg * 4), is = *reinterpret_cast<const f32x4*>(invstd + cg * 4);
    const f32x4 ga = *reinterpret_cast<const f32x4*>(gamma + cg * 4), be = *reinterpret_cast<const f32x4*>(beta + cg * 4);
    const f32x4 s0 = *reinterpret_cast<const f32x4*>(sums + cg * 4), s1 = *reinterpret_cast<const f32x4*>(sums + C + cg * 4);
    f32x4 gi, m0, m1;
#pragma unroll
    for (int j = 0; j < 4; ++j) { gi[j] = ga[j] * is[j]; m0[j] = s0[j] * inv_count; m1[j] = s1[j] * inv_count; }
    const size_t step = (size_t)gridDim.x * PPB;
    for (size_t p0 = (size_t)blockIdx.x * PPB + prow; p0 < P; p0 += step * 4) {
        f32x4 xv[4], gv[4];
#pragma unroll
        for (int u = 0; u < 4; ++u) {
            const size_t p = p0 + u * step;
            if (p < P) { xv[u] = *reinterpret_cast<const f32x4*>(x + p * ldx + cg * 4); gv[u] = *reinterpret_cast<const f32x4*>(dy + p * lddy + cg * 4); }
        }
#pragma unroll
        for (int u = 0; u < 4; ++u) {
            const size_t p = p0 + u * step;
            if (p >= P) break;
            f32x4 r;
#pragma unroll
            for (int j = 0; j < 4; ++j) {
                const float xh = (xv[u][j] - mu[j]) * is[j];
                const float yv = fmaf(xh, ga[j], be[j]);
                const float dz = (act == KPX_ACT_RELU && !(yv > 0.f)) ? 0.f : gv[u][j];
                r[j] = gi[j] * (dz - m0[j] - xh * m1[j]);
            }
            *reinterpret_cast<f32x4*>(dx + p * lddx + cg * 4) = r;
        }
    }
}
static inline dim3 strip_grid(size_t P, int C, int W, int groups) {
    const int G = C / W, Gb = G < 256 ? G : 256, PPB = 256 / Gb;
    size_t nb = (P + (size_t)PPB * 4 - 1) / ((size_t)PPB * 4);
    if (nb < 1) nb = 1;
    if (nb > KPX_MAX_BLOCKS) nb = KPX_MAX_BLOCKS;
    return dim3((unsigned)nb, (unsigned)((G + Gb - 1) / Gb), (unsigned)groups);
}

extern "C" int kpx_bn_apply_f32(const float* x, size_t P, int C, int ldx, const float* mean, const float* invstd,
                                const float* gamma, const float* beta, float* y, int ldy, int act, void* stream) {
    if (!x || !y || !mean || !invstd || !gamma || !beta || C <= 0 || ldx < C || ldy < C || act < 0 || act > 1) return KPX_EINVAL;
    if (P == 0) return 0;
    const bool vec = (C % 4 == 0) && (ldx % 4 == 0) && (ldy % 4 == 0) && ((((uintptr_t)x) | ((uintptr_t)y)) & 15) == 0;
    if (vec) hipLaunchKernelGGL(bn_apply_strip_kernel, strip_grid(P, C, 4, 1), dim3(256), 0, kpx_stream(stream), x, P, C, ldx, mean, invstd, gamma, beta, y, ldy, act);
    else hipLaunchKernelGGL(bn_apply_kernel, dim3(grid_for(P * C)), dim3(256), 0, kpx_stream(stream), x, P, C, ldx, mean, invstd, gamma, beta, y, ldy, act);
    return kpx_launch_status();
}

__global__ __launch_bounds__(256) void bn_fold_conv_kernel(const float* __restrict__ w, const float* __restrict__ bias, size_t rows, int C,
                                                          const float* __restrict__ gamma, const float* __restrict__ beta, const float* __restrict__ mm,
                                                          const float* __restrict__ mv, float eps, float* __restrict__ w_out, float* __restrict__ b_out) {
    const size_t total = rows * (size_t)C;
    for (size_t i = (size_t)blockIdx.x * 256 + threadIdx.x; i < total; i += (size_t)gridDim.x * 256) {
        const int c = (int)(i % C);
        const float sc = gamma[c] * (1.0f / sqrtf(mv[c] + eps));
        w_out[i] = w[i] * sc;
        if (i < (size_t)C) b_out[c] = ((bias ? bias[c] : 0.f) - mm[c]) * sc + beta[c];
    }
}
extern "C" int kpx_bn_fold_conv_f32(const float* w, const float* bias, size_t rows, int C, const float* gamma, const float* beta,
                                    const float* moving_mean, const float* moving_var, float eps, float* w_out, float* b_out, void* stream) {
    if (!w || !gamma || !beta || !moving_mean || !moving_var || !w_out || !b_out || rows == 0 || C <= 0) return KPX_EINVAL;
    hipLaunchKernelGGL(bn_fold_conv_kernel, dim3(grid_for(rows * C)), dim3(256), 0, kpx_stream(stream), w, bias, rows, C, gamma, beta,
                       moving_mean, moving_var, eps, w_out, b_out);
    return kpx_launch_status();
}

__global__ __launch_bounds__(1024) void bn_stats_finalize_groups_kernel(const double* part, size_t part_gstride, int nb, const float* __restrict__ ts, size_t tiles_per_group,
                                                                       int groups, int C, double count, float eps, float* mean, float* invstd,
                                                                       float* mm, float* mv, float decay) {
    const int c = blockIdx.x, sg = threadIdx.x >> 8, nseg = blockDim.x >> 8;
    __shared__ double sm[4][2][4];
// ... 912 lines not shown
```

### unsupervised-keypoint-learning-for-guiding-class-conditional-video-prediction_amd/layers.py

```python
import torch

from . import ops
from .variables import Sym, default_store, is_sym

ACT_NONE, ACT_RELU, ACT_LRELU = ops.ACT_NONE, ops.ACT_RELU, ops.ACT_LRELU
EXACT_ZERO_BIAS_GRAD = True
import os as _os
FOLD_BN_INFERENCE = True
TRACE = None
F32_OUT_SCOPES = set()


def conv(x, channels, kernel=4, stride=2, pad=0, use_bias=True, scope='conv_0', act=ACT_NONE, cin=None, head31=False, bias_grad=True, bn_stats=False,
         f43_fwd=True, input_act=ACT_NONE, act_bwd_by_consumer=False, out_f32=False):
    st = default_store()
    channels = int(channels)
    cin_ = int(cin) if cin is not None else int(x.shape[-1])
    with st.variable_scope(scope), st.variable_scope('conv2d'):
        kname = st.get_variable('kernel', (kernel, kernel, cin_, channels), 'kernel_head31' if head31 else 'kernel')
        bname = st.get_variable('bias', (channels,), 'zeros') if use_bias else None
    if not st.materialised:
        st.layer_attrs.setdefault(kname, {})['f43_fwd'] = bool(f43_fwd)
    if is_sym(x):
        n, h, w, _ = x.shape
        _, _, ho = ops.same_pad(h + 2 * pad, kernel, stride)
        _, _, wo = ops.same_pad(w + 2 * pad, kernel, stride)
        return Sym(n, ho, wo, channels)
    w_, wg = st.param(kname)
    b_, bg = st.param(bname) if use_bias else (None, None)
    return ops.conv2d(x, w_, b_, stride=stride, pad=pad, act=act, cin=cin, w_grad_out=wg, b_grad_out=bg, bias_grad=bias_grad, bn_stats=bn_stats,
                      input_act=input_act, act_bwd_by_consumer=act_bwd_by_consumer, out_dtype=torch.float32 if out_f32 else None)


def conv1x1_keypoints(x, channels, scope='conv_0'):
    st = default_store()
    channels = int(channels)
    cin_ = int(x.shape[-1])
    with st.variable_scope(scope), st.variable_scope('conv2d'):
        kname = st.get_variable('kernel', (1, 1, cin_, channels), 'kernel')
        bname = st.get_variable('bias', (channels,), 'zeros')
    if is_sym(x):
        n, h, w, _ = x.shape
        return Sym(n, channels, 2), Sym(n, h, channels), Sym(n, w, channels)
    w_, wg = st.param(kname)
    b_, bg = st.param(bname)
    return ops.keypoint_head_proj(x, w_, b_, w_grad_out=wg, b_grad_out=bg)


def batch_norm(x, train_mode, scope='batch_norm', act=ACT_NONE, groups=1, update_moving=True, out_f32=False):
    st = default_store()
    c = int(x.shape[-1])
    with st.variable_scope(scope):
        beta = st.get_variable('beta', (c,), 'zeros')
        gamma = st.get_variable('gamma', (c,), 'ones')
        mm = st.get_variable('moving_mean', (c,), 'moving_zeros')
        mv = st.get_variable('moving_variance', (c,), 'moving_ones')
    if is_sym(x):
        return Sym(*x.shape)
    g_, gg = st.param(gamma)
    b_, bg = st.param(beta)
    return ops.batch_norm(x, g_, b_, st[mm], st[mv], train=bool(train_mode), act=act, groups=groups,
                          update_moving=update_moving and bool(train_mode), g_grad_out=gg, b_grad_out=bg, out_f32=out_f32)


def conv_bn_relu(x, channels, kernel, stride, train_mode, conv_scope, bn_scope, groups=1, update_moving=True, cin=None, f43_fwd=True, out_f32=False):
    if not train_mode and not is_sym(x) and FOLD_BN_INFERENCE and x.is_cuda and not torch.is_grad_enabled():
        st = default_store()
        with st.variable_scope(conv_scope), st.variable_scope('conv2d'):
            kname, bname = st.scoped('kernel'), st.scoped('bias')
        with st.variable_scope(bn_scope):
            names = [st.scoped(n) for n in ('gamma', 'beta', 'moving_mean', 'moving_variance')]
        if all(n in st.vars for n in [kname, bname] + names):
            wf, bf = st.folded_conv_bn(kname, bname, names[0], names[1], names[2], names[3], ops.BN_EPS)
            return ops.conv2d(x, wf, bf, stride=stride, pad=0, act=ACT_RELU, cin=cin)
    x = conv(x, channels, kernel=kernel, stride=stride, scope=conv_scope, cin=cin, bias_grad=not (EXACT_ZERO_BIAS_GRAD and train_mode),
             bn_stats=bool(train_mode), f43_fwd=f43_fwd)
    if (TRACE is not None or F32_OUT_SCOPES) and not is_sym(x):
        st = default_store()
        with st.variable_scope(conv_scope):
            full = st.scoped('')
        y = batch_norm(x, train_mode, scope=bn_scope, act=ACT_RELU, groups=groups, update_moving=update_moving, out_f32=out_f32 or full.rstrip('/') in F32_OUT_SCOPES)
        if TRACE is not None:
            TRACE.append((full.rstrip('/'), y.detach()))
        return y
    return batch_norm(x, train_mode, scope=bn_scope, act=ACT_RELU, groups=groups, update_moving=update_moving, out_f32=out_f32)


def fully_connected(x, num_outputs, scope='fully_connected', act=ACT_RELU, trainable=False):
    st = default_store()
    with st.variable_scope(scope):
        wn = st.get_variable('weights', (int(x.shape[-1]), int(num_outputs)), 'glorot2d')
        bn = st.get_variable('biases', (int(num_outputs),), 'zeros')
    if is_sym(x):
        return Sym(x.shape[0], num_outputs)
    if trainable:
        (w_, wg), (b_, bg) = st.param(wn), st.param(bn)
        return ops.dense_train(x, w_, b_, act=act, w_grad_out=wg, b_grad_out=bg)
    return ops.dense(x, st[wn].detach(), st[bn].detach(), act=act)


class _LstmStack:

    def __init__(self, units):
        self.units = [int(u) for u in units]

    def zero_state(self, batch, device):
        return [(torch.zeros((batch, u), dtype=torch.float32, device=device), torch.zeros((batch, u), dtype=torch.float32, device=device))
                for u in self.units]

    def declare(self, input_size):
        st = default_store()
        names, prev = [], int(input_size)
        for i, u in enumerate(self.units):
            with st.variable_scope('multi_rnn_cell'), st.variable_scope('cell_%d' % i), st.variable_scope('basic_lstm_cell'):
                names.append((st.get_variable('kernel', (prev + u, 4 * u), 'glorot2d'), st.get_variable('bias', (4 * u,), 'zeros')))
            prev = u
        return names

    def sequence(self, x_seq, scope_prefix=None):
        st = default_store()
        names = self.declare(x_seq.shape[-1])
        if is_sym(x_seq):
            return Sym(x_seq.shape[0], x_seq.shape[1], self.units[-1])
        for kn, bn in names:
            (k_, kg), (b_, bg) = st.param(kn), st.param(bn)
            x_seq = ops.lstm_layer(x_seq, k_, b_, w_grad_out=kg, b_grad_out=bg)
        return x_seq

    def __call__(self, x, state):
        st = default_store()
        names = self.declare(x.shape[-1])
        new_state = []
        for (kn, bn), (c, h) in zip(names, state):
            h2, c2 = ops.lstm_cell(x, h, c, st[kn].detach(), st[bn].detach())
            new_state.append((c2, h2))
            x = h2
        return x, new_state


def lstm_model(layers_):
    return _LstmStack(layers_)


def to_coord(input_, input_size, output_size, stddev=0.02, bias_start=0.0, trainable=False):
    st = default_store()
    with st.variable_scope('fully_connected'):
        wn = st.get_variable('W', (int(input_size), int(output_size)), 'normal002')
        bn = st.get_variable('b', (int(output_size),), 'zeros')
    if is_sym(input_):
        return Sym(input_.shape[0], output_size)
    if trainable:
        (w_, wg), (b_, bg) = st.param(wn), st.param(bn)
        return ops.dense_train(input_, w_, b_, act=ops.ACT_TANH, w_grad_out=wg, b_grad_out=bg)
    return ops.dense(input_, st[wn].detach(), st[bn].detach(), act=ops.ACT_TANH)
```

### unsupervised-keypoint-learning-for-guiding-class-conditional-video-prediction_amd/ops.py

```python
import collections as _collections
import os as _os
import struct as _struct
import weakref as _weakref
from fractions import Fraction

import torch

from . import _lib
from ._lib import lib, check

ACT_NONE, ACT_RELU, ACT_LRELU, ACT_TANH = 0, 1, 2, 3
BN_EPS = 1e-5
BN_DECAY = 0.999


_raw_stream = getattr(torch._C, '_cuda_getCurrentRawStream', None)
_cur_device = getattr(torch._C, '_cuda_getDevice', None)


def _stream():
    if _raw_stream is not None and _cur_device is not None:
        return _raw_stream(_cur_device())
    return torch.cuda.current_stream().cuda_stream


def _ptr(t):
    return t.data_ptr() if t is not None else None


def _require_gpu(t):
    if not t.is_cuda:
        raise _lib.KpxError('kpx ops run on MI355X only (got a %s tensor); there is no CPU fallback' % t.device)
    if t.dtype != torch.float32 and t.dtype != torch.bfloat16:
        raise _lib.KpxError('kpx ops take fp32 tensors, or bf16 activation tensors in the bf16 configuration (got %s)' % t.dtype)


def same_pad(in_size, k, s):
    out = -(-in_size // s)
    total = max((out - 1) * s + k - in_size, 0)
    return total // 2, total - total // 2, out


def _nhwc(t):
    _require_gpu(t)
    assert t.dim() == 4
    n, h, w, c = t.shape
    ld = t.stride(2) if w > 1 else (t.stride(1) if h > 1 else (t.stride(0) if n > 1 else c))
    ok = (c == 1 or t.stride(3) == 1) and ld >= c
    ok = ok and (w == 1 or t.stride(2) == ld) and (h == 1 or t.stride(1) == w * ld) and (n == 1 or t.stride(0) == h * w * ld)
    if not ok:
        t = t.contiguous()
        ld = c
    return t, ld


class _Scratch:

    def __init__(self):
        self._bufs = {}

    def get(self, key, nbytes, device):
        k = (key, device, _stream())
        b = self._bufs.get(k)
        if b is None or b.numel() < nbytes:
            b = torch.empty(int(max(nbytes, 1 << 16)), dtype=torch.uint8, device=device)
            self._bufs[k] = b
        return b

    def reduce(self, c, device):
        return self.get('reduce', lib.kpx_chan_reduce_scratch_bytes(int(c)), device)


scratch = _Scratch()


def _workspace(key, nbytes, device):
    return (scratch.get(key, nbytes, device).data_ptr() if nbytes else None), nbytes


def _took(rc, entry):
    if rc == -1:
        return False
    check(rc, entry)
    return True

SIDE_WGRAD = True
FUSE_BN_STATS = True
FUSE_ACT_BWD = True
FUSE_BN_BWD = True
FORK_BEFORE_DGRAD = 'capture'
_side_streams = {}
_side_dirty = {}
_side_keep = []


_inline_wgrad = [False]


class inline_wgrad:

    def __enter__(self):
        self.old, _inline_wgrad[0] = _inline_wgrad[0], True

    def __exit__(self, *exc):
        _inline_wgrad[0] = self.old
        return False


def _side_stream(device, origin):
    key = (device, origin)
    st = _side_streams.get(key)
    if st is None:
        st = torch.cuda.Stream(device=device)
        _side_streams[key] = st
    return key, st


_grad_epoch = [0]
_grad_written = {}


def begin_backward():
    _grad_epoch[0] += 1
    if len(_grad_written) > 4096:
        _grad_written.clear()
    _pending_bwd_stats.clear()


def _claim_grad(dst):
    key = (dst.data_ptr(), dst.numel())
    first = _grad_written.get(key) != _grad_epoch[0]
    _grad_written[key] = _grad_epoch[0]
    return first


def reset_after_failed_capture():
    _side_dirty.clear()
    _side_keep.clear()
    _pending_stats.clear()
    _pending_bwd_stats.clear()


def graph_knobs():
    return (_compute_dtype[0], SIDE_WGRAD, FUSE_BN_STATS, FUSE_BN_BWD, FUSE_ACT_BWD, FORK_BEFORE_DGRAD, WINO43, WINO43_MIN_WORKGROUPS, WINO43_NMIN)


def normalize_device(device):
    dev = torch.device(device)
    if dev.type == 'cuda' and dev.index is None:
        dev = torch.device('cuda', torch.cuda.current_device())
    return dev


def join_side_stream(device=None):
    if device is not None:
        device = normalize_device(device)
    for key in list(_side_dirty):
        dev, origin = key
        if device is not None and dev != device:
            continue
        torch.cuda.current_stream(dev).wait_stream(_side_streams[key])
        del _side_dirty[key]
    if not _side_dirty:
        _side_keep.clear()


_compute_dtype = [_os.environ.get('KPX_DTYPE', 'f32')]
BF16 = torch.bfloat16
fallback_uses = {'conv_fwd': 0, 'conv_dgrad': 0, 'conv_wgrad': 0, 'other': 0}


def set_compute_dtype(name):
    if name not in ('f32', 'bf16'):
        raise ValueError("compute dtype must be 'f32' or 'bf16'")
    _compute_dtype[0] = name


def compute_dtype():
    return _compute_dtype[0]


def act_dtype():
    return BF16 if _compute_dtype[0] == 'bf16' else torch.float32


def _arith():
    return 1 if _compute_dtype[0] == 'bf16' else 0


def cast_channels_raw(src_ptr, ldsrc, dst_ptr, lddst, pixels, c, kind):
    check(lib.kpx_cast_channels(src_ptr, ldsrc, dst_ptr, lddst, pixels, c, kind, _stream()), 'kpx_cast_channels')


def cast(t, dtype):
    if t.dtype == dtype:
        return t
    t = t.contiguous()
    out = torch.empty(t.shape, dtype=dtype, device=t.device)
    n = t.numel()
    c = next(k for k in (4096, 512, 64, 8, 1) if n % k == 0)
    if n:
        cast_channels_raw(t.data_ptr(), c, out.data_ptr(), c, n // c, c, 0 if dtype == BF16 else 1)
    return out


def _esz(t):
    return 2 if t.dtype == BF16 else 4


def _slice_f32(x, ldx, cin):
    n, h, w = x.shape[0], x.shape[1], x.shape[2]
    out = torch.empty((n, h, w, cin), dtype=torch.float32, device=x.device)
    if x.dtype == BF16:
        cast_channels_raw(x.data_ptr(), ldx, out.data_ptr(), cin, n * h * w, cin, 1)
    else:
        copy_channels_raw(x.data_ptr(), ldx, out.data_ptr(), cin, n * h * w, cin)
    return out


Launched = _collections.namedtuple('Launched', 'stats')


def _bf16s_gathered(inp, ld_in, k):
    if k % 32 == 0 or k in (8, 16):
        return k
    k0, k = k, 8 if k < 8 else 16 if k < 16 else (k + 31) // 32 * 32
    if ld_in < k:
        return 0
    if DEBUG_FINITE and not bool(torch.isfinite(inp.reshape(-1, inp.shape[-1])[:, k0:k].float()).all()):
        raise _lib.KpxError('bf16 3x3 conv: non-finite values in the pad channels %d..%d of a %d-wide buffer' % (k0, k, inp.shape[-1]))
    return k


def _bf16s_bnbwd(dy, lddy, k, w, dx, lddx, nn, bn_y, beta):
    n, h, wd = dy.shape[0], dy.shape[1], dy.shape[2]
    k = _bf16s_gathered(dy, lddy, k)
    if (not k or bn_y.dtype != BF16 or not bn_y.is_contiguous() or bn_y.shape[3] != nn or nn % 8 or lddx % 8
            or not lib.kpx_conv3x3_bf16s_eligible(n, h, wd, k, nn, lddy, dy.data_ptr())):
        return None
    wf = _bf16s_prepared(w, True)
    tiles = lib.kpx_conv3x3_bf16s_stats_tiles(n, h, wd, k, nn)
    slab = torch.empty(tiles * 2 * nn, dtype=torch.float32, device=dy.device)
    rc = lib.kpx_conv3x3_bf16s_bnbwd(dy.data_ptr(), n, h, wd, k, lddy, wf.data_ptr(), dx.data_ptr(), nn, lddx, bn_y.data_ptr(), nn, beta.data_ptr(), slab.data_ptr(), _stream())
    if not _took(rc, 'kpx_conv3x3_bf16s_bnbwd'):
        return None
    conv_kernel_uses_bf16s[0] += 1
    return Launched((slab, Fraction(tiles, n)))


conv_kernel_uses_bf16s = [0]


def _bf16s_prepared(w, dgrad):
    ent = _cached_u('bf16s', w, dgrad)
    if ent is None:
        cin, cout = int(w.shape[2]), int(w.shape[3])
        k, nn = (cout, cin) if dgrad else (cin, cout)
        wf = scratch.get('bf16s_w%d' % (1 if dgrad else 0), lib.kpx_conv3x3_bf16s_weights_bytes(k, nn), w.device)
        check(lib.kpx_conv3x3_bf16s_prepare_f32(w.data_ptr(), cin, cout, 1 if dgrad else 0, wf.data_ptr(), _stream()), 'kpx_conv3x3_bf16s_prepare_f32')
        return wf
    if ent[1] is not None:
        ent[1].ensure_fresh('bf16s')
    return ent[0]


def _bf16s_conv(inp, ld_in, k, w, bias, out, ld_out, nn, act, dgrad, want_stats=False, mask=None):
    n, h, wd = inp.shape[0], inp.shape[1], inp.shape[2]
    out_f32 = out.dtype == torch.float32
    k = _bf16s_gathered(inp, ld_in, k)
    if not k:
        return None
    g = 4 if out_f32 else 8
    if nn % g:
        nn = (nn + g - 1) // g * g
        if ld_out < nn:
            return None
    if ld_out % g or not lib.kpx_conv3x3_bf16s_eligible(n, h, wd, k, nn, ld_in, inp.data_ptr()):
        return None
    if out.data_ptr() % 16 or (mask is not None and (out_f32 or mask.dtype != BF16 or mask.data_ptr() % 16)):
        return None
    wf = _bf16s_prepared(w, dgrad)
    slab = None
    if want_stats:
        tiles = lib.kpx_conv3x3_bf16s_stats_tiles(n, h, wd, k, nn)
        slab = torch.empty(tiles * 2 * nn, dtype=torch.float32, device=inp.device)
    check(lib.kpx_conv3x3_bf16s(inp.data_ptr(), n, h, wd, k, ld_in, wf.data_ptr(), _ptr(bias), out.data_ptr(), nn, ld_out, 1 if out_f32 else 0, act,
                                _ptr(mask), mask.stride(2) if mask is not None else 0, _ptr(slab), _stream()), 'kpx_conv3x3_bf16s')
    conv_kernel_uses_bf16s[0] += 1
    return Launched((slab, Fraction(tiles, n)) if want_stats else None)


conv_kernel_uses ={'wino43': 0, 'wino43b': 0}

WINO43 = _os.environ.get('KPX_WINO43', '1') != '0'
DEBUG_FINITE = _os.environ.get('KPX_DEBUG_FINITE', '0') == '1'
WINO43_MIN_WORKGROUPS = 0
WINO43_NMIN = 33
# ... 79 lines not shown
    def _refresh(self, form):
        _, table, n = self.tables[form]
        if n:
            check(getattr(lib, _FORMS[form].transform_batch)(table.data_ptr(), n, _stream()), _FORMS[form].transform_batch)

    def ensure_fresh(self, form=None):
        if not self.filters:
            return
        if form is None:
            form = 'bf16s' if _compute_dtype[0] == 'bf16' else 'wino'
            if form == 'bf16s' and FilterBank.wino_needed_in_bf16:
                self.ensure_fresh('wino')
        if form == 'bf16s':
            if self.synced['bf16s'] != self.version:
                if 'bf16s' not in self.tables:
                    self._build('bf16s')
                self._refresh('bf16s')
                self.synced['bf16s'] = self.version
            return
        if self.synced['wino'] != self.version:
            for f in _WINO_FORMS:
                self._refresh(f)
            self.synced['wino'] = self.version
            self._wino_fresh_ev = None
            if _compute_dtype[0] == 'bf16' and not torch.cuda.is_current_stream_capturing():
                ev = torch.cuda.Event()
                ev.record(torch.cuda.current_stream())
                self._wino_fresh_ev = (ev, torch.cuda.current_stream().cuda_stream)
                FilterBank.wino_needed_in_bf16 = True
        elif self._wino_fresh_ev is not None and torch.cuda.current_stream().cuda_stream != self._wino_fresh_ev[1]:
            torch.cuda.current_stream().wait_event(self._wino_fresh_ev[0])

    def keys(self):
        return [(w.data_ptr(), dgrad) for _, w in self.filters for dgrad in (0, 1)]


def register_constant_filter(w, name='', f43_fwd=True):
    if w.dim() != 4 or w.shape[0] != 3 or w.shape[1] != 3 or not w.is_cuda:
        return []
    cin, cout = int(w.shape[2]), int(w.shape[3])
    for dgrad in (0, 1):
        for form, f in _FORMS.items():
            if not f.wanted(*_kn(cin, cout, dgrad), dgrad, f43_fwd) or (form == 'bf16s' and not (_compute_dtype[0] == 'bf16' and cin % 8 == 0)):
                continue
            u = torch.empty(f.nbytes(cin, cout, dgrad) // f.dtype.itemsize, dtype=f.dtype, device=w.device)
            check(getattr(lib, f.transform)(w.data_ptr(), cin, cout, dgrad, u.data_ptr(), _stream()), f.transform)
            _filter_forms[(form, w.data_ptr(), dgrad)] = (u, None, _weakref.ref(w.untyped_storage()), (cin, cout))
    return [(w.data_ptr(), dgrad) for dgrad in (0, 1)]


def release_filters(keys):
    for ptr, dgrad in keys:
        for form in _FORMS:
            _filter_forms.pop((form, ptr, dgrad), None)


def _wino43_plan(n, h, wd, k, nn, ld_in, in_ptr, dgrad, forms, want_stats=False, bn_src=False, vgg=False):
    if not (WINO43 and 'wino43' in forms):
        return []
    wgs = (n // 2 if wd == 16 else n * (h // 16) * (wd // 32)) * ((nn + 63) // 64)
    f32 = bool(lib.kpx_conv3x3_wino43_eligible(n, h, wd, k, nn, ld_in, in_ptr))
    if wgs <= WINO43_MIN_WORKGROUPS or (vgg and (nn % 64 or not f32)):
        return []
    if want_stats and not lib.kpx_conv3x3_wino43_stats_tiles(n, h, wd):
        return []
    bn = bool(bn_src and dgrad and nn % 64 == 0 and wd != 16)
    plan = []
    if WINO43B and 'wino43b' in forms and lib.kpx_conv3x3_wino43b_eligible(n, h, wd, k, nn, ld_in, in_ptr):
        plan.append(('wino43b', bn))
    if f32:
        plan += [('wino43', bn)] + ([('wino43', False)] if bn else [])
    return plan


def _wino43_run(plan, forms, inp, ld_in, k, bias, out, ld_out, nn, act, want_stats=False, bn_src=None, mask=None, pool=None):
    n, h, wd = inp.shape[0], inp.shape[1], inp.shape[2]
    for form, bn in plan:
        entry = 'kpx_conv3x3_wino43b_f32' if form == 'wino43b' else 'kpx_conv3x3_wino43_f32'
        tiles = lib.kpx_conv3x3_wino43_stats_tiles(n, h, wd)
        slab = torch.empty(tiles * 2 * nn, dtype=torch.float32, device=inp.device) if (want_stats or bn) else None
        rc = getattr(lib, entry)(inp.data_ptr(), n, h, wd, k, ld_in, forms[form][0].data_ptr(), None if bn else _ptr(bias), out.data_ptr(), nn,
                                 ld_out, ACT_NONE if bn else act, _ptr(mask), mask.shape[3] if mask is not None else 0, _ptr(pool),
                                 pool.shape[3] if pool is not None else 0, _ptr(slab), bn_src[0].data_ptr() if bn else None,
                                 bn_src[0].shape[3] if bn else 0, bn_src[1].data_ptr() if bn else None, _stream())
        if _took(rc, entry):
            conv_kernel_uses['wino43'] += 1
            if form == 'wino43b':
                conv_kernel_uses['wino43b'] += 1
            return Launched((slab, Fraction(tiles, n)) if slab is not None else None)
    return None


def _f43_forms(w, dgrad):
    return {form: ent for form in ('wino43', 'wino43b') if (ent := _cached_u(form, w, dgrad)) is not None}


def _wino_pretransformed(inp, ld_in, k, w, bias, out, ld_out, nn, act, dgrad, want_stats=False, bn_src=None, mask=None, pool_out=None):
    n, h, wd = inp.shape[0], inp.shape[1], inp.shape[2]
    vgg = mask is not None or pool_out is not None
    ent = _cached_u('wino', w, dgrad)
    if not vgg and (ent is None or not lib.kpx_conv3x3_wino_eligible(n, h, wd, k, nn, ld_in, inp.data_ptr())):
        return None
    forms = _f43_forms(w, dgrad)
    plan = _wino43_plan(n, h, wd, k, nn, ld_in, inp.data_ptr(), dgrad, forms, want_stats=want_stats, bn_src=bn_src is not None, vgg=vgg)
    if vgg and not plan:
        return None
    bank = (forms['wino43'] if vgg else ent)[1]
    if bank is not None:
        bank.ensure_fresh('wino')
    r = _wino43_run(plan, forms, inp, ld_in, k, bias, out, ld_out, nn, act, want_stats=want_stats, bn_src=bn_src, mask=mask, pool=pool_out)
    if r is not None or vgg:
        return r
    bn = bn_src is not None and dgrad and h % 16 == 0 and wd % 16 == 0
    stats = bn or (want_stats and h % 16 == 0 and wd % 16 == 0)
    tiles = lib.kpx_conv3x3_wino_stats_tiles(n, h, wd)
    slab = torch.empty(tiles * 2 * nn, dtype=torch.float32, device=inp.device) if stats else None
    check(lib.kpx_conv3x3_wino_f32(inp.data_ptr(), n, h, wd, k, ld_in, ent[0].data_ptr(), None if bn else _ptr(bias), out.data_ptr(), nn, ld_out,
                                   ACT_NONE if bn else act, _ptr(slab), bn_src[0].data_ptr() if bn else None, bn_src[0].shape[3] if bn else 0,
                                   bn_src[1].data_ptr() if bn else None, _stream()), 'kpx_conv3x3_wino_f32')
    return Launched((slab, Fraction(tiles, n)) if stats else None)


def conv3x3_same(inp, ld_in, k, w, bias, out, ld_out, nn, act, dgrad, *, want_stats=False, bn_src=None, mask=None, pool_out=None):
    if act == ACT_TANH:
        return None
    n, h, wd = inp.shape[0], inp.shape[1], inp.shape[2]
    if inp.dtype == BF16:
        if pool_out is not None:
            return None
        if dgrad and bn_src is not None and mask is None and out.dtype == BF16:
            r = _bf16s_bnbwd(inp, ld_in, k, w, out, ld_out, nn, bn_src[0], bn_src[1])
            if r is not None:
                return r
        return _bf16s_conv(inp, ld_in, k, w, bias, out, ld_out, nn, act, dgrad, want_stats=want_stats, mask=mask)
    if out.dtype != torch.float32:
        return None
    if mask is not None or pool_out is not None:
        return _wino_pretransformed(inp, ld_in, k, w, bias, out, ld_out, nn, act, dgrad, mask=mask, pool_out=pool_out)
    if nn == 16 and not (dgrad and bn_src is not None) and lib.kpx_conv3x3_c16_eligible(n, h, wd, k, nn, ld_in, ld_out, inp.data_ptr()):
        tiles = (h // 16) * (wd // 16)
        slab = torch.empty(n * tiles * 2 * 16, dtype=torch.float32, device=inp.device) if want_stats else None
        check(lib.kpx_conv3x3_c16_f32(inp.data_ptr(), n, h, wd, k, ld_in, w.data_ptr(), 1 if dgrad else 0, _ptr(bias), out.data_ptr(), ld_out, act,
                                      _ptr(slab), _stream()), 'kpx_conv3x3_c16_f32')
        return Launched((slab, Fraction(tiles)) if want_stats else None)
    if not dgrad and nn <= 4 and k <= 128 and n * h * wd >= 65536:
        return None
    return _wino_pretransformed(inp, ld_in, k, w, bias, out, ld_out, nn, act, dgrad, want_stats=want_stats, bn_src=bn_src)


def _is_3x3_same(kh, kw, stride, pad_t, pad_l, hi, wi, ho, wo):
    return kh == 3 and kw == 3 and stride == 1 and pad_t == 1 and pad_l == 1 and ho == hi and wo == wi


def conv_fwd_raw(x, ldx, cin, w, bias, y, ldy, stride, pad_t, pad_l, act, want_stats=False):
    n, hi, wi = x.shape[0], x.shape[1], x.shape[2]
    ho, wo = y.shape[1], y.shape[2]
    kh, kw, _, cout = w.shape
    same3 = _is_3x3_same(kh, kw, stride, pad_t, pad_l, hi, wi, ho, wo)
    yf, ldyf = y, ldy
    if x.dtype == BF16 or y.dtype == BF16:
        if same3 and (r := conv3x3_same(x, ldx, cin, w, bias, y, ldy, cout, act, False, want_stats=want_stats)) is not None:
            return r.stats
        if x.dtype == torch.float32 and cin <= 4 and ldx == cin and _took(lib.kpx_conv_image_fwd_bf16(
                x.data_ptr(), n, hi, wi, cin, w.data_ptr(), kh, kw, _ptr(bias), y.data_ptr(), ho, wo, cout, ldy, stride, pad_t, pad_l, act, _stream()),
                'kpx_conv_image_fwd_bf16'):
            return None
        if x.dtype == BF16 and act != ACT_TANH and _took(lib.kpx_conv2d_fwd_bf16(
                x.data_ptr(), n, hi, wi, cin, ldx, w.data_ptr(), kh, kw, _ptr(bias), y.data_ptr(), 1 if y.dtype == torch.float32 else 0, ho, wo, cout, ldy,
                stride, pad_t, pad_l, act, *_workspace('splitk', lib.kpx_conv2d_fwd_workspace_bytes(n, ho, wo, cin, cout, kh, kw), x.device), _stream()),
                'kpx_conv2d_fwd_bf16'):
            return None
        want_stats = False
        if x.dtype == BF16:
            fallback_uses['conv_fwd'] += 1
            x, ldx = _slice_f32(x, ldx, cin), cin
        if y.dtype == BF16:
            yf, ldyf = torch.empty((n, ho, wo, cout), dtype=torch.float32, device=x.device), cout
    r = conv3x3_same(x, ldx, cin, w, bias, yf, ldyf, cout, act, False, want_stats=want_stats) if same3 else None
    if r is None:
        check(lib.kpx_conv2d_fwd_f32(x.data_ptr(), n, hi, wi, cin, ldx, w.data_ptr(), kh, kw, _ptr(bias), yf.data_ptr(), ho, wo, cout, ldyf, stride, pad_t, pad_l, act,
                                     _arith(), *_workspace('splitk', lib.kpx_conv2d_fwd_workspace_bytes(n, ho, wo, cin, cout, kh, kw), x.device), _stream()),
              'kpx_conv2d_fwd_f32')
    if yf is not y:
        cast_channels_raw(yf.data_ptr(), cout, y.data_ptr(), ldy, n * ho * wo, cout, 0)
    return r.stats if r is not None else None


def conv_dgrad_raw(dy, lddy, w, dx, lddx, cin, stride, pad_t, pad_l, bn_src=None, mul=None):
    n, ho, wo = dy.shape[0], dy.shape[1], dy.shape[2]
    hi, wi = dx.shape[1], dx.shape[2]
    kh, kw, _, cout = w.shape
    same3 = mul is None and _is_3x3_same(kh, kw, stride, pad_t, pad_l, hi, wi, ho, wo)
    dxf, lddxf = dx, lddx
    if dy.dtype == BF16 or dx.dtype == BF16:
        if same3 and (r := conv3x3_same(dy, lddy, cout, w, None, dx, lddx, cin, ACT_NONE, True, bn_src=bn_src)) is not None:
            return r.stats
        if dy.dtype == BF16 and (mul is None or mul[0].dtype == BF16) and _took(lib.kpx_conv2d_dgrad_bf16(
                dy.data_ptr(), n, ho, wo, cout, lddy, w.data_ptr(), kh, kw, dx.data_ptr(), 1 if dx.dtype == torch.float32 else 0, hi, wi, cin, lddx,
                stride, pad_t, pad_l, *((mul[0].data_ptr(), mul[0].shape[3], mul[1]) if mul is not None else (None, 0, 0)),
                *_workspace('splitk', lib.kpx_conv2d_dgrad_workspace_bytes(n, hi, wi, cin, cout, kh, kw, stride), dy.device), _stream()), 'kpx_conv2d_dgrad_bf16'):
            return None
        if dy.dtype == BF16 and dx.dtype == torch.float32 and cin <= 4 and mul is None and _took(lib.kpx_conv_image_dgrad_bf16(
                dy.data_ptr(), n, ho, wo, cout, lddy, w.data_ptr(), kh, kw, dx.data_ptr(), hi, wi, cin, lddx, stride, pad_t, pad_l, _stream()),
                'kpx_conv_image_dgrad_bf16'):
            return None
        bn_src = None
        if dy.dtype == BF16:
            fallback_uses['conv_dgrad'] += 1
            dy, lddy = _slice_f32(dy, lddy, cout), cout
        if dx.dtype == BF16:
            dxf, lddxf = torch.empty((n, hi, wi, cin), dtype=torch.float32, device=dy.device), cin
        if mul is not None and mul[0].dtype == BF16:
            mul = (cast(mul[0], torch.float32), mul[1])
    r = conv3x3_same(dy, lddy, cout, w, None, dxf, lddxf, cin, ACT_NONE, True, bn_src=bn_src) if same3 else None
    if r is None:
        ws = _workspace('splitk', lib.kpx_conv2d_dgrad_workspace_bytes(n, hi, wi, cin, cout, kh, kw, stride), dy.device)
        geom = (dy.data_ptr(), n, ho, wo, cout, lddy, w.data_ptr(), kh, kw, dxf.data_ptr(), hi, wi, cin, lddxf, stride, pad_t, pad_l, _arith())
        if mul is not None:
            check(lib.kpx_conv2d_dgrad_act_f32(*geom, mul[0].data_ptr(), mul[0].shape[3], mul[1], *ws, _stream()), 'kpx_conv2d_dgrad_act_f32')
        else:
            check(lib.kpx_conv2d_dgrad_f32(*geom, *ws, _stream()), 'kpx_conv2d_dgrad_f32')
    if dxf is not dx:
        cast_channels_raw(dxf.data_ptr(), cin, dx.data_ptr(), lddx, n * hi * wi, cin, 0)
    return r.stats if r is not None else None


def conv_wgrad_raw(x, ldx, cin, dy, lddy, dw, stride, pad_t, pad_l):
    n, hi, wi = x.shape[0], x.shape[1], x.shape[2]
    ho, wo = dy.shape[1], dy.shape[2]
    kh, kw, _, cout = dw.shape

    def generic(entry, *arith):
        return getattr(lib, entry)(x.data_ptr(), n, hi, wi, cin, ldx, dy.data_ptr(), ho, wo, cout, lddy, dw.data_ptr(), kh, kw, stride, pad_t, pad_l, *arith,
                                   *_workspace('wgrad', lib.kpx_conv2d_wgrad_workspace_bytes(n, ho, wo, cin, cout, kh, kw), x.device), _stream())

    if x.dtype == BF16 and dy.dtype == BF16:
        if (_is_3x3_same(kh, kw, stride, pad_t, pad_l, hi, wi, ho, wo)
                and lib.kpx_conv3x3_wgrad_bf16_eligible(n, hi, wi, cin, ldx, cout, lddy, x.data_ptr(), dy.data_ptr())):
            check(lib.kpx_conv3x3_wgrad_bf16(x.data_ptr(), n, hi, wi, cin, ldx, dy.data_ptr(), cout, lddy, dw.data_ptr(),
                                             *_workspace('wgrad', lib.kpx_conv3x3_wgrad_bf16_workspace_bytes(n, hi, wi, cin, cout), x.device), _stream()),
                  'kpx_conv3x3_wgrad_bf16')
            return
        if _took(generic('kpx_conv2d_wgrad_bf16'), 'kpx_conv2d_wgrad_bf16'):
            return
    if x.dtype == torch.float32 and dy.dtype == BF16 and cin <= 4 and _took(generic('kpx_conv_image_wgrad_bf16'), 'kpx_conv_image_wgrad_bf16'):
        return
    if x.dtype == BF16 or dy.dtype == BF16:
        fallback_uses['conv_wgrad'] += 1
        if x.dtype == BF16:
            x, ldx = _slice_f32(x, ldx, cin), cin
        if dy.dtype == BF16:
            dy, lddy = _slice_f32(dy, lddy, cout), cout
    check(generic('kpx_conv2d_wgrad_f32', _arith()), 'kpx_conv2d_wgrad_f32')


def chan_sum_raw(x, ldx, pixels, c, out):
    if x.dtype == BF16:
        if c % 8 == 0 and ldx % 8 == 0 and x.data_ptr() % 16 == 0:
            check(lib.kpx_chan_sum_bf16(x.data_ptr(), pixels, c, ldx, out.data_ptr(), scratch.reduce(c, x.device).data_ptr(), _stream()), 'kpx_chan_sum_bf16')
            return
        fallback_uses['other'] += 1
        xf = torch.empty((pixels, c), dtype=torch.float32, device=x.device)
        cast_channels_raw(x.data_ptr(), ldx, xf.data_ptr(), c, pixels, c, 1)
        x, ldx = xf, c
    check(lib.kpx_chan_sum_f32(x.data_ptr(), pixels, c, ldx, out.data_ptr(), scratch.reduce(c, x.device).data_ptr(), _stream()),
          'kpx_chan_sum_f32')


def act_bwd_raw(dy, y, dz, act):
    if dy.dtype == BF16:
        assert y.dtype == BF16 and dz.dtype == BF16 and dy.numel() % 8 == 0
        check(lib.kpx_act_bwd_bf16(dy.data_ptr(), y.data_ptr(), dz.data_ptr(), dy.numel(), act, _stream()), 'kpx_act_bwd_bf16')
        return
    check(lib.kpx_act_bwd_f32(dy.data_ptr(), y.data_ptr(), dz.data_ptr(), dy.numel(), act, _stream()), 'kpx_act_bwd_f32')


def act_bwd_raw_(dy, y, act):
    act_bwd_raw(dy, y, dy, act)


def axpy_raw_(y, x, a=1.0):
    check(lib.kpx_axpy_f32(y.data_ptr(), x.data_ptr(), y.numel(), a, _stream()), 'kpx_axpy_f32')


def fill_raw_(t, v=0.0):
    if t.dtype == BF16:
        assert v == 0.0 and t.numel() % 2 == 0, 'bf16 tensors are only ever zero-filled'
        check(lib.kpx_fill_f32(t.data_ptr(), t.numel() // 2, 0.0, _stream()), 'kpx_fill_f32')
        return
    check(lib.kpx_fill_f32(t.data_ptr(), t.numel(), v, _stream()), 'kpx_fill_f32')


def copy_channels_raw(src_ptr, ldsrc, dst_ptr, lddst, pixels, c):
    check(lib.kpx_copy_channels_f32(src_ptr, ldsrc, dst_ptr, lddst, pixels, c, _stream()), 'kpx_copy_channels_f32')


def flat_copy_tensor(src, dst_ptr):
    nbytes = src.numel() * _esz(src)
    assert nbytes % 4 == 0
    flat_copy_raw(src.data_ptr(), dst_ptr, nbytes // 4)


def flat_copy_raw(src_ptr, dst_ptr, n):
    if n % 4 == 0 and src_ptr % 16 == 0 and dst_ptr % 16 == 0:
        copy_channels_raw(src_ptr, 4, dst_ptr, 4, n // 4, 4)
    else:
        copy_channels_raw(src_ptr, 1, dst_ptr, 1, n, 1)


class Conv2dFn(torch.autograd.Function):

    @staticmethod
    def forward(ctx, x, w, b, w_grad_out, b_grad_out, stride, pad, act, cin, bias_grad, bn_stats=False, bn_src=None, input_act=ACT_NONE,
                act_bwd_by_consumer=False, out_dtype=None):
        x, ldx = _nhwc(x)
        ctx.input_act = input_act if (input_act != ACT_NONE and x.is_contiguous() and (cin is None or cin == x.shape[3])) else ACT_NONE
        if input_act != ACT_NONE and ctx.input_act == ACT_NONE:
            raise _lib.KpxError('input_act needs the whole contiguous activated tensor as the convolution input')
        ctx.act_bwd_by_consumer = bool(act_bwd_by_consumer) and act != ACT_NONE
        ctx.bn_src = bn_src if (bn_src is not None and x.is_contiguous() and (cin is None or cin == x.shape[3])) else None
        _require_gpu(w)
        w = w.contiguous()
        n, h, wd, cx = x.shape
        kh, kw, wcin, cout = w.shape
        cin = cx if cin is None else cin
        assert wcin == cin and cin <= cx
        pt, _, ho = same_pad(h + 2 * pad, kh, stride)
        pl, _, wo = same_pad(wd + 2 * pad, kw, stride)
        pad_t, pad_l = pad + pt, pad + pl
        y = torch.empty((n, ho, wo, cout), dtype=out_dtype if out_dtype is not None else act_dtype(), device=x.device)
        st = conv_fwd_raw(x, ldx, cin, w, b, y, cout, stride, pad_t, pad_l, act, want_stats=bn_stats and act == ACT_NONE)
        if st is not None:
            _pending_stats[y.data_ptr()] = st
        ctx.geom = (stride, pad_t, pad_l, act, cin, ldx)
        ctx.has_bias = b is not None and bias_grad
        ctx.w_grad_out, ctx.b_grad_out = w_grad_out, b_grad_out
        ctx.save_for_backward(x, w, y if act != ACT_NONE else None)
        return y

    @staticmethod
    def backward(ctx, dy):
        x, w, y = ctx.saved_tensors
        stride, pad_t, pad_l, act, cin, ldx = ctx.geom
        dy = dy.contiguous()
        cout = w.shape[3]
        if act != ACT_NONE and not ctx.act_bwd_by_consumer:
            dz = torch.empty_like(dy)
            act_bwd_raw(dy, y, dz, act)
            dy = dz
        dx = dw = db = None
        want_w = ctx.needs_input_grad[1]
        want_b = ctx.has_bias and ctx.needs_input_grad[2]
        dy_sum = dy
        if (dy.dtype == torch.float32 and x.dtype == BF16 and cout < 8 and w.shape[0] == 3 and w.shape[1] == 3 and stride == 1
                and ctx.input_act == ACT_NONE):
            dy16 = torch.empty((dy.shape[0], dy.shape[1], dy.shape[2], 8), dtype=BF16, device=dy.device)
            cast_channels_raw(dy.data_ptr(), cout, dy16.data_ptr(), 8, dy.shape[0] * dy.shape[1] * dy.shape[2], cout, 3)
            dy = dy16
        lddy = dy.shape[3]
        side = (SIDE_WGRAD and not _inline_wgrad[0] and (want_w or want_b) and (not want_w or ctx.w_grad_out is not None)
                and (not want_b or ctx.b_grad_out is not None))
        fork = None
        if side and (FORK_BEFORE_DGRAD == 'before' or (FORK_BEFORE_DGRAD == 'capture' and torch.cuda.is_current_stream_capturing())):
            fork = torch.cuda.Event()
            fork.record(torch.cuda.current_stream(x.device))
        if ctx.needs_input_grad[0]:
            cx = x.shape[3]
            dx = torch.empty(x.shape, dtype=x.dtype, device=x.device)
            if cin < cx:
                fill_raw_(dx, 0.0)
            st = conv_dgrad_raw(dy, lddy, w, dx, cx, cin, stride, pad_t, pad_l,
                                bn_src=(x, ctx.bn_src[0]) if ctx.bn_src is not None else None,
                                mul=(x, ctx.input_act) if ctx.input_act != ACT_NONE else None)
            if st is not None:
                _pending_bwd_stats[dx.data_ptr()] = (st[0], st[1], ctx.bn_src[1], dx)
        if side:
            main = torch.cuda.current_stream(x.device)
            skey, st = _side_stream(x.device, main.cuda_stream)
            if fork is not None:
                st.wait_event(fork)
            else:
                st.wait_stream(main)
            _side_keep.append((dy, dy_sum, x))
            _side_dirty[skey] = True
            stream_ctx = torch.cuda.stream(st)
        else:
            import contextlib
            stream_ctx = contextlib.nullcontext()
        with stream_ctx:
            if want_w:
                direct = ctx.w_grad_out is not None and _claim_grad(ctx.w_grad_out)
                dw_buf = ctx.w_grad_out if direct else torch.empty_like(w)
                conv_wgrad_raw(x, ldx, cin, dy, lddy, dw_buf, stride, pad_t, pad_l)
                if ctx.w_grad_out is not None and not direct:
                    axpy_raw_(ctx.w_grad_out, dw_buf)
                dw = None if ctx.w_grad_out is not None else dw_buf
            if want_b:
                direct = ctx.b_grad_out is not None and _claim_grad(ctx.b_grad_out)
                db_buf = ctx.b_grad_out if direct else torch.empty(cout, dtype=torch.float32, device=x.device)
                chan_sum_raw(dy_sum, cout, dy.shape[0] * dy.shape[1] * dy.shape[2], cout, db_buf)
                if ctx.b_grad_out is not None and not direct:
                    axpy_raw_(ctx.b_grad_out, db_buf)
                db = None if ctx.b_grad_out is not None else db_buf
        return dx, dw, db, None, None, None, None, None, None, None, None, None, None, None, None


_pending_stats = {}
_pending_bwd_stats = {}
_bn_counter = [0]
fused_bn_uses = {'stats_from_conv_epilogue': 0, 'backward_sums_from_dgrad_epilogue': 0}


def conv2d(x, w, b=None, stride=1, pad=0, act=ACT_NONE, cin=None, w_grad_out=None, b_grad_out=None, bias_grad=True, bn_stats=False,
           input_act=ACT_NONE, act_bwd_by_consumer=False, out_dtype=None):
    y = Conv2dFn.apply(x, w, b, w_grad_out, b_grad_out, stride, pad, act, cin, bias_grad, bn_stats and FUSE_BN_STATS,
                       getattr(x, '_kpx_bn', None) if FUSE_BN_BWD else None, input_act if FUSE_ACT_BWD else ACT_NONE,
                       act_bwd_by_consumer and FUSE_ACT_BWD, out_dtype)
    if bn_stats:
        st = _pending_stats.pop(y.data_ptr(), None)
        if st is not None:
            y._kpx_tile_stats = st
    return y


def _whole_tiles_per_group(n, groups, tiles_per_image):
    return n % groups == 0 and (tiles_per_image * (n // groups)).denominator == 1


class BatchNormFn(torch.autograd.Function):

    @staticmethod
    def forward(ctx, x, gamma, beta, moving_mean, moving_var, g_grad_out, b_grad_out, train, act, groups, update_moving, tile_stats=None, bn_id=0, out_f32=False):
        ctx.bn_id = bn_id
        _require_gpu(x)
        x = x.contiguous()
        n, h, w, c = x.shape
        assert n % groups == 0
        dev = x.device
        if x.dtype == BF16 and not (train and c % 8 == 0):
            fallback_uses['other'] += 1
            x = cast(x, torch.float32)
        ctx.x16 = x.dtype == BF16
        y = torch.empty(x.shape, dtype=torch.float32 if (out_f32 or not ctx.x16) else BF16, device=dev)
        if train:
            mean = torch.empty((groups, c), dtype=torch.float32, device=dev)
            invstd = torch.empty((groups, c), dtype=torch.float32, device=dev)
            ng = n // groups
            pix = ng * h * w
            sc = scratch.get('bn%d' % groups, lib.kpx_bn_train_scratch_bytes(c, groups), dev)
            slab_ptr, tpg = None, 0
            if tile_stats is not None:
                slab, tpi = tile_stats
                fused_bn_uses['stats_from_conv_epilogue'] += groups
                slab_ptr, tpg = slab.data_ptr(), int(ng * tpi)
            entry = 'kpx_bn_train_fwd_bf16' if ctx.x16 else 'kpx_bn_train_fwd_f32'
            y_f32 = (1 if y.dtype == torch.float32 else 0,) if ctx.x16 else ()
            check(getattr(lib, entry)(x.data_ptr(), pix, groups, c, c, slab_ptr, tpg, BN_EPS, gamma.data_ptr(), beta.data_ptr(),
                                      mean.data_ptr(), invstd.data_ptr(), moving_mean.data_ptr() if update_moving else None,
                                      moving_var.data_ptr() if update_moving else None, BN_DECAY, y.data_ptr(), c, *y_f32, act,
                                      sc.data_ptr(), _stream()), entry)
        else:
            mean = moving_mean.reshape(1, c)
            invstd = torch.empty((1, c), dtype=torch.float32, device=dev)
            check(lib.kpx_bn_invstd_f32(moving_var.data_ptr(), c, BN_EPS, invstd.data_ptr(), _stream()), 'kpx_bn_invstd_f32')
            check(lib.kpx_bn_apply_f32(x.data_ptr(), n * h * w, c, c, mean.data_ptr(), invstd.data_ptr(),
                                       gamma.data_ptr(), beta.data_ptr(), y.data_ptr(), c, act, _stream()), 'kpx_bn_apply_f32')
        ctx.train, ctx.act, ctx.groups = train, act, groups
        ctx.g_grad_out, ctx.b_grad_out = g_grad_out, b_grad_out
        ctx.save_for_backward(x, gamma, beta, mean, invstd)
        return y

    @staticmethod
    def backward(ctx, dy):
        if not ctx.train:
            raise _lib.KpxError('backward through inference-mode batch norm is not part of the hot path')
        x, gamma, beta, mean, invstd = ctx.saved_tensors
        dy = dy.contiguous()
        n, h, w, c = x.shape
        groups = ctx.groups
        ng = n // groups
        pix = ng * h * w
        dev = x.device
        dx = torch.empty_like(x)
        dg = ctx.g_grad_out if ctx.g_grad_out is not None else torch.empty(c, dtype=torch.float32, device=dev)
        db = ctx.b_grad_out if ctx.b_grad_out is not None else torch.empty(c, dtype=torch.float32, device=dev)
        fresh = True
        if ctx.g_grad_out is not None:
            fresh = _claim_grad(ctx.g_grad_out)
            _claim_grad(ctx.b_grad_out)
        ent = _pending_bwd_stats.pop(dy.data_ptr(), None)
        if ent is not None and (ent[2] != ctx.bn_id or ctx.act != ACT_RELU or tuple(ent[0].shape) != (n * ent[1] * 2 * c,) or not _whole_tiles_per_group(n, groups, ent[1])):
            ent = None
        sc = scratch.get('bn%d' % groups, lib.kpx_bn_train_scratch_bytes(c, groups), dev)
        if ctx.x16:
            entry, dy_f32 = 'kpx_bn_train_bwd_bf16', (1 if dy.dtype == torch.float32 else 0,)
        else:
            if dy.dtype == BF16:
                dy = cast(dy, torch.float32)
            entry, dy_f32 = 'kpx_bn_train_bwd_f32', ()
        if ent is not None:
            fused_bn_uses['backward_sums_from_dgrad_epilogue'] += groups
        check(getattr(lib, entry)(dy.data_ptr(), c, *dy_f32, x.data_ptr(), c, pix, groups, c, mean.data_ptr(), invstd.data_ptr(),
                                  gamma.data_ptr(), beta.data_ptr(), ctx.act, dx.data_ptr(), c, dg.data_ptr(), db.data_ptr(), 0 if fresh else 1,
                                  ent[0].data_ptr() if ent is not None else None, int(ng * ent[1]) if ent is not None else 0,
                                  sc.data_ptr(), _stream()), entry)
        return (dx, None if ctx.g_grad_out is not None else dg, None if ctx.b_grad_out is not None else db,
                None, None, None, None, None, None, None, None, None, None, None)


def batch_norm(x, gamma, beta, moving_mean, moving_var, train=True, act=ACT_RELU, groups=1, update_moving=True,
               g_grad_out=None, b_grad_out=None, out_f32=False):
    ts = getattr(x, '_kpx_tile_stats', None) if train else None
    if ts is not None and (x.shape[0] % groups or tuple(ts[0].shape) != (x.shape[0] * ts[1] * 2 * x.shape[3],) or not _whole_tiles_per_group(x.shape[0], groups, ts[1])):
        ts = None
    _bn_counter[0] += 1
    y = BatchNormFn.apply(x, gamma, beta, moving_mean, moving_var, g_grad_out, b_grad_out, train, act, groups, update_moving, ts, _bn_counter[0], out_f32)
    if train and act == ACT_RELU:
        y._kpx_bn = (beta.detach(), _bn_counter[0])
    return y


class UpsampleConcatFn(torch.autograd.Function):

    @staticmethod
    def forward(ctx, x, skip):
        _require_gpu(x)
        x = x.contiguous()
        n, h, w, c1 = x.shape
        c2 = 0
        if skip is not None:
            skip = skip.contiguous()
            assert skip.shape[:3] == (n, 2 * h, 2 * w)
            c2 = skip.shape[3]
        ld = c1 + c2
        out = torch.empty((n, 2 * h, 2 * w, ld), dtype=x.dtype, device=x.device)
        if x.dtype == BF16:
            check(lib.kpx_resize2x_fwd_bf16(x.data_ptr(), n, h, w, c1, c1, out.data_ptr(), ld, _stream()), 'kpx_resize2x_fwd_bf16')
            if c2:
                skip = cast(skip, BF16)
                cast_channels_raw(skip.data_ptr(), c2, out.data_ptr() + 2 * c1, ld, n * 4 * h * w, c2, 2)
        else:
            check(lib.kpx_resize2x_fwd_f32(x.data_ptr(), n, h, w, c1, c1, out.data_ptr(), ld, _stream()), 'kpx_resize2x_fwd_f32')
            if c2:
                copy_channels_raw(cast(skip, torch.float32).data_ptr(), c2, out.data_ptr() + 4 * c1, ld, n * 4 * h * w, c2)
        ctx.dims = (n, h, w, c1, c2)
        return out

    @staticmethod
    def backward(ctx, dout):
        n, h, w, c1, c2 = ctx.dims
        dout = dout.contiguous()
        ld = c1 + c2
        dx = dskip = None
        if ctx.needs_input_grad[0]:
            dx = torch.empty((n, h, w, c1), dtype=dout.dtype, device=dout.device)
            if dout.dtype == BF16:
                check(lib.kpx_resize2x_bwd_bf16(dout.data_ptr(), n, h, w, c1, ld, dx.data_ptr(), c1, _stream()), 'kpx_resize2x_bwd_bf16')
            else:
                check(lib.kpx_resize2x_bwd_f32(dout.data_ptr(), n, h, w, c1, ld, dx.data_ptr(), c1, _stream()), 'kpx_resize2x_bwd_f32')
        if c2 and ctx.needs_input_grad[1]:
            dskip = torch.empty((n, 2 * h, 2 * w, c2), dtype=dout.dtype, device=dout.device)
            if dout.dtype == BF16:
                cast_channels_raw(dout.data_ptr() + 2 * c1, ld, dskip.data_ptr(), c2, n * 4 * h * w, c2, 2)
            else:
                copy_channels_raw(dout.data_ptr() + 4 * c1, ld, dskip.data_ptr(), c2, n * 4 * h * w, c2)
        return dx, dskip


def upsample2x_concat(x, skip=None):
    return UpsampleConcatFn.apply(x, skip)


class ConcatChannelsFn(torch.autograd.Function):

    @staticmethod
    def forward(ctx, a, b):
        a, b = a.contiguous(), b.contiguous()
        _require_gpu(a)
        n, h, w, c1 = a.shape
        c2 = b.shape[3]
        out = torch.empty((n, h, w, c1 + c2), dtype=a.dtype, device=a.device)
        if a.dtype == BF16:
            cast_channels_raw(a.data_ptr(), c1, out.data_ptr(), c1 + c2, n * h * w, c1, 2)
            cast_channels_raw(cast(b, BF16).data_ptr(), c2, out.data_ptr() + 2 * c1, c1 + c2, n * h * w, c2, 2)
        else:
            copy_channels_raw(a.data_ptr(), c1, out.data_ptr(), c1 + c2, n * h * w, c1)
            copy_channels_raw(cast(b, torch.float32).data_ptr(), c2, out.data_ptr() + 4 * c1, c1 + c2, n * h * w, c2)
        ctx.dims = (n, h, w, c1, c2)
        return out

    @staticmethod
    def backward(ctx, dout):
        n, h, w, c1, c2 = ctx.dims
        dout = dout.contiguous()
        da = torch.empty((n, h, w, c1), dtype=dout.dtype, device=dout.device)
        db = torch.empty((n, h, w, c2), dtype=dout.dtype, device=dout.device)
        if dout.dtype == BF16:
            cast_channels_raw(dout.data_ptr(), c1 + c2, da.data_ptr(), c1, n * h * w, c1, 2)
            cast_channels_raw(dout.data_ptr() + 2 * c1, c1 + c2, db.data_ptr(), c2, n * h * w, c2, 2)
        else:
            copy_channels_raw(dout.data_ptr(), c1 + c2, da.data_ptr(), c1, n * h * w, c1)
            copy_channels_raw(dout.data_ptr() + 4 * c1, c1 + c2, db.data_ptr(), c2, n * h * w, c2)
        return da, db


def concat_channels(a, b):
    return ConcatChannelsFn.apply(a, b)


class ConcatBatchFn(torch.autograd.Function):

    @staticmethod
    def forward(ctx, a, b):
        a, b = a.contiguous(), b.contiguous()
        _require_gpu(a)
        assert a.shape[1:] == b.shape[1:] and a.dtype == b.dtype
        out = torch.empty((a.shape[0] + b.shape[0],) + tuple(a.shape[1:]), dtype=a.dtype, device=a.device)
        flat_copy_tensor(a, out.data_ptr())
        flat_copy_tensor(b, out.data_ptr() + _esz(a) * a.numel())
        ctx.na = a.shape[0]
        return out

    @staticmethod
    def backward(ctx, dout):
        dout = dout.contiguous()
        return dout[:ctx.na], dout[ctx.na:]


def concat_batch(a, b):
    return ConcatBatchFn.apply(a, b)


class KeypointHeadFn(torch.autograd.Function):

    @staticmethod
    def forward(ctx, logits):
        _require_gpu(logits)
        logits = logits.contiguous()
        b, h, w, k = logits.shape
        dev = logits.device
        mu = torch.empty((b, k, 2), dtype=torch.float32, device=dev)
        py = torch.empty((b, h, k), dtype=torch.float32, device=dev)
        px = torch.empty((b, w, k), dtype=torch.float32, device=dev)
        sc = scratch.get('kphead', lib.kpx_keypoint_head_scratch_bytes(b, h, w, k), dev)
        check(lib.kpx_keypoint_head_fwd_f32(logits.data_ptr(), b, h, w, k, mu.data_ptr(), py.data_ptr(), px.data_ptr(),
                                            sc.data_ptr(), _stream()), 'kpx_keypoint_head_fwd_f32')
        ctx.dims = (b, h, w, k)
        ctx.save_for_backward(mu, py, px)
        ctx.mark_non_differentiable(py, px)
        return mu, py, px

    @staticmethod
    def backward(ctx, dmu, _dpy, _dpx):
        mu, py, px = ctx.saved_tensors
        b, h, w, k = ctx.dims
        dmu = dmu.contiguous()
        dl = torch.empty((b, h, w, k), dtype=torch.float32, device=dmu.device)
        check(lib.kpx_keypoint_head_bwd_f32(dmu.data_ptr(), mu.data_ptr(), py.data_ptr(), px.data_ptr(), b, h, w, k,
                                            dl.data_ptr(), _stream()), 'kpx_keypoint_head_bwd_f32')
        return dl


def keypoint_head(logits):
    return KeypointHeadFn.apply(logits)


class KeypointHeadProjFn(torch.autograd.Function):

    @staticmethod
    def forward(ctx, x, w, b, w_grad_out, b_grad_out):
        _require_gpu(x)
# ... 687 lines not shown
```

Before: 1417.

## Fuse BN statistics and bias-gradient sums into gemm3 conv epilogues

Adds epilogue variants to the gemm3 implicit-GEMM conv kernel. They produce per-tile channel sums, using double accumulation stored as hi/lo float pairs, for three cases: BN forward statistics, BN backward sums fused with the ReLU mask in dgrad, and bias-gradient sums from the activation-aware dgrad. The Python layer routes eligible fp32 non-3x3-stride-1 convs through these entry points and reduces the tile items with a small kernel. This replaces separate full passes over activations for statistics and channel sums. In exchange it adds epilogue work, LDS overlay and grouping constraints on tile counts.

```diff
diff --git a/include/kpx.h b/include/kpx.h
--- a/include/kpx.h
+++ b/include/kpx.h
@@ -9,7 +9,7 @@
 #endif
 
 #define KPX_EINVAL (-1)
-#define KPX_ABI_VERSION 15
+#define KPX_ABI_VERSION 16
 
 enum { KPX_ACT_NONE = 0, KPX_ACT_RELU = 1, KPX_ACT_LRELU = 2 , KPX_ACT_TANH = 3  };
 
@@ -59,6 +59,26 @@
                              int stride, int pad_t, int pad_l, int arith,
                              const float* y_in, int ld_y_in, int act_in,
                              void* workspace, size_t workspace_bytes, void* stream);
+
+size_t kpx_conv2d_sums_items(int N, int H, int W, int stride);
+int kpx_conv2d_fwd_stats_f32(const float* x, int N, int Hi, int Wi, int Cin, int ldx,
+                             const float* w_hwio, int KH, int KW, const float* bias,
+                             float* y, int Ho, int Wo, int Cout, int ldy,
+                             int stride, int pad_t, int pad_l, int arith, float* tile_stats, int groups,
+                             void* workspace, size_t workspace_bytes, void* stream);
+int kpx_conv2d_dgrad_bn_f32(const float* dy, int N, int Ho, int Wo, int Cout, int lddy,
+                            const float* w_hwio, int KH, int KW,
+                            float* dx, int Hi, int Wi, int Cin, int lddx,
+                            int stride, int pad_t, int pad_l, int arith,
+                            float* tile_stats, const float* bn_y, int ld_bn_y, const float* bn_beta, int groups,
+                            void* workspace, size_t workspace_bytes, void* stream);
+int kpx_conv2d_dgrad_act_sums_f32(const float* dy, int N, int Ho, int Wo, int Cout, int lddy,
+                                  const float* w_hwio, int KH, int KW,
+                                  float* dx, int Hi, int Wi, int Cin, int lddx,
+                                  int stride, int pad_t, int pad_l, int arith,
+                                  const float* y_in, int ld_y_in, int act_in, float* bias_sums,
+                                  void* workspace, size_t workspace_bytes, void* stream);
+int kpx_chan_sum_items_f32(const float* items, size_t n_items, int C, float* sum_out, void* stream);
 
 size_t kpx_conv2d_wgrad_workspace_bytes(int N, int Ho, int Wo, int Cin, int Cout, int KH, int KW);
 int kpx_conv2d_wgrad_f32(const float* x, int N, int Hi, int Wi, int Cin, int ldx,
diff --git a/unsupervised-keypoint-learning-for-guiding-class-conditional-video-prediction_amd/_lib.py b/unsupervised-keypoint-learning-for-guiding-class-conditional-video-prediction_amd/_lib.py
--- a/unsupervised-keypoint-learning-for-guiding-class-conditional-video-prediction_amd/_lib.py
+++ b/unsupervised-keypoint-learning-for-guiding-class-conditional-video-prediction_amd/_lib.py
@@ -20,7 +20,7 @@
 lib = ctypes.CDLL(LIB_PATH)
 
 P = c_void_p
-ABI_VERSION = 15
+ABI_VERSION = 16
 SIGNATURES = {
     'kpx_abi_version': (c_int, []),
     'kpx_reload_env': (c_int, []),
@@ -32,6 +32,14 @@
                                      P, c_int, c_int, c_int, c_int, c_int, c_int, c_int, c_int, P, c_size_t, P]),
     'kpx_conv2d_dgrad_act_f32': (c_int, [P, c_int, c_int, c_int, c_int, c_int, P, c_int, c_int,
                                          P, c_int, c_int, c_int, c_int, c_int, c_int, c_int, c_int, P, c_int, c_int, P, c_size_t, P]),
+    'kpx_conv2d_sums_items': (c_size_t, [c_int, c_int, c_int, c_int]),
+    'kpx_conv2d_fwd_stats_f32': (c_int, [P, c_int, c_int, c_int, c_int, c_int, P, c_int, c_int, P,
+                                         P, c_int, c_int, c_int, c_int, c_int, c_int, c_int, c_int, P, c_int, P, c_size_t, P]),
+    'kpx_conv2d_dgrad_bn_f32': (c_int, [P, c_int, c_int, c_int, c_int, c_int, P, c_int, c_int,
+                                        P, c_int, c_int, c_int, c_int, c_int, c_int, c_int, c_int, P, P, c_int, P, c_int, P, c_size_t, P]),
+    'kpx_conv2d_dgrad_act_sums_f32': (c_int, [P, c_int, c_int, c_int, c_int, c_int, P, c_int, c_int,
+                                              P, c_int, c_int, c_int, c_int, c_int, c_int, c_int, c_int, P, c_int, c_int, P, P, c_size_t, P]),
+    'kpx_chan_sum_items_f32': (c_int, [P, c_size_t, c_int, P, P]),
     'kpx_conv2d_wgrad_workspace_bytes': (c_size_t, [c_int, c_int, c_int, c_int, c_int, c_int, c_int]),
     'kpx_conv2d_wgrad_f32': (c_int, [P, c_int, c_int, c_int, c_int, c_int, P, c_int, c_int, c_int, c_int,
                                      P, c_int, c_int, c_int, c_int, c_int, c_int, P, c_size_t, P]),
diff --git a/unsupervised-keypoint-learning-for-guiding-class-conditional-video-prediction_amd/csrc/conv_gemm3.hip b/unsupervised-keypoint-learning-for-guiding-class-conditional-video-prediction_amd/csrc/conv_gemm3.hip
--- a/unsupervised-keypoint-learning-for-guiding-class-conditional-video-prediction_amd/csrc/conv_gemm3.hip
+++ b/unsupervised-keypoint-learning-for-guiding-class-conditional-video-prediction_amd/csrc/conv_gemm3.hip
@@ -4,9 +4,31 @@
 
 #define G3_PITCH 80
 
-template <int BM, int BN, int WM, int WN, bool BT, int TERMS, bool IO16 = false>
+template <int BN>
+__device__ __forceinline__ void g3_colsum_put(double* red, int wm, int c, int lh, double s0, double s1) {
+    s0 += __shfl_xor(s0, 32);
+    s1 += __shfl_xor(s1, 32);
+    if (lh == 0) { red[(wm * 2 + 0) * BN + c] = s0; red[(wm * 2 + 1) * BN + c] = s1; }
+}
+template <int BN, int WM>
+__device__ __forceinline__ void g3_colsum_write(const double* red, float* item, int n0, int Cout, int t) {
+    __syncthreads();
+    if (t < BN && n0 + t < Cout) {
+        double a0 = red[t], a1 = red[BN + t];
+#pragma unroll
+        for (int w = 1; w < WM; ++w) { a0 += red[(w * 2 + 0) * BN + t]; a1 += red[(w * 2 + 1) * BN + t]; }
+        const float h0 = (float)a0, h1 = (float)a1;
+        item[n0 + t] = h0;
+        item[Cout + n0 + t] = h1;
+        item[2 * Cout + n0 + t] = (float)(a0 - (double)h0);
+        item[3 * Cout + n0 + t] = (float)(a1 - (double)h1);
+    }
+}
+
+template <int BM, int BN, int WM, int WN, bool BT, int TERMS, bool IO16 = false, int EPI = KPX_G3_NONE>
 __global__ __launch_bounds__(WM * WN * 64, 2) void conv_gemm3_kernel(const ConvGeom g) {
     static_assert(!IO16 || TERMS == 1, "bf16 tensors carry one term");
+    static_assert(EPI == KPX_G3_NONE || (!IO16 && (EPI == KPX_G3_STATS) == !BT), "sums: fp32 tensors; statistics forward, the other two data gradient");
     constexpr int NT = WM * WN * 64, BK = 32, ESZ = IO16 ? 2 : 4;
     constexpr int TM = BM / (WM * 32), TN = BN / (WN * 32);
     constexpr int APL = BM * G3_PITCH, BPL = BN * G3_PITCH;
@@ -253,11 +275,14 @@
         }
         return;
     }
+    double* const red = reinterpret_cast<double*>(smem + BM * 4);
 #pragma unroll
     for (int n = 0; n < TN; ++n) {
         const int col = n0 + wcol + n * 32 + li;
         const bool cok = col < g.Cout;
         const float bv = (cok && g.bias) ? g.bias[col] : 0.f;
+        const float bb = (EPI == KPX_G3_BNBWD && cok) ? g.bn_beta[col] : 0.f;
+        double s0 = 0.0, s1 = 0.0;
 #pragma unroll
         for (int i = 0; i < TM; ++i) {
 #pragma unroll
@@ -265,6 +290,14 @@
                 const int pix = rowpix[wrow + i * 32 + (r & 3) + 8 * (r >> 2) + 4 * lh];
                 if (cok && pix >= 0) {
                     float v = acc[i][n][r] + bv;
+                    if (EPI == KPX_G3_BNBWD) {
+                        const float by = g.bn_y[(size_t)pix * g.ld_bn + col];
+                        v = by > 0.f ? v : 0.f;
+                        s0 += (double)v;
+                        s1 += (double)v * ((double)by - (double)bb);
+                        g.y[(size_t)pix * g.ldy + col] = v;
+                        continue;
+                    }
                     if (g.act == KPX_ACT_RELU) v = fmaxf(v, 0.f);
                     else if (g.act == KPX_ACT_LRELU) v = v > 0.f ? v : 0.01f * v;
                     else if (g.act == KPX_ACT_TANH) v = tanhf(v);
@@ -273,27 +306,36 @@
                                                       : g.mul_y[(size_t)pix * g.ld_mul + col];
                         v *= kpx_act_grad_from_y(my, g.mul_act);
                     }
+                    if (EPI == KPX_G3_STATS) { s0 += (double)v; s1 += (double)v * (double)v; }
+                    if (EPI == KPX_G3_BIAS) s0 += (double)v;
                     if (g.io16 & 2) { const __bf16 b = (__bf16)v; reinterpret_cast<unsigned short*>(g.y)[(size_t)pix * g.ldy + col] = __builtin_bit_cast(unsigned short, b); }
                     else g.y[(size_t)pix * g.ldy + col] = v;
                 }
             }
         }
+        if (EPI != KPX_G3_NONE) g3_colsum_put<BN>(red, wm, wcol + n * 32 + li, lh, s0, s1);
+    }
+    if (EPI != KPX_G3_NONE) {
+        const int mi = L / g.nt, mtg = g.st_mtg[blockIdx.y];
+        const int item = (mi / mtg) * g.st_ipg + g.st_it0[blockIdx.y] + mi % mtg;
+        g3_colsum_write<BN, WM>(red, g.sums + (size_t)item * 4 * g.Cout, n0, g.Cout, t);
     }
 }
 
 static std::atomic<unsigned long long> g3_attr_mask{0};
 
 template <int BN> struct g3_waves { static constexpr int wm = BN == 128 ? 2 : 4, wn = BN == 128 ? 4 : 2; };
-template <int BM, int BN, bool BT, int TERMS, bool IO16 = false>
+template <int BM, int BN, bool BT, int TERMS, bool IO16 = false, int EPI = KPX_G3_NONE>
 static int g3_launch_one(const ConvGeom& g, dim3 grid, hipStream_t s) {
     constexpr int lds = TERMS * (BM + BN) * G3_PITCH;
-    hipLaunchKernelGGL((conv_gemm3_kernel<BM, BN, g3_waves<BN>::wm, g3_waves<BN>::wn, BT, TERMS, IO16>), grid, dim3(g3_waves<BN>::wm * g3_waves<BN>::wn * 64), lds, s, g);
+    static_assert(lds >= BM * 4 + g3_waves<BN>::wm * 2 * BN * 8, "rowpix and the column sums overlay the stage");
+    hipLaunchKernelGGL((conv_gemm3_kernel<BM, BN, g3_waves<BN>::wm, g3_waves<BN>::wn, BT, TERMS, IO16, EPI>), grid, dim3(g3_waves<BN>::wm * g3_waves<BN>::wn * 64), lds, s, g);
     return kpx_launch_status();
 }
-template <int BM, int BN, bool BT, int TERMS, bool IO16 = false>
+template <int BM, int BN, bool BT, int TERMS, bool IO16 = false, int EPI = KPX_G3_NONE>
 static hipError_t g3_set_attr() {
     constexpr int lds = TERMS * (BM + BN) * G3_PITCH;
-    return hipFuncSetAttribute(reinterpret_cast<const void*>(conv_gemm3_kernel<BM, BN, g3_waves<BN>::wm, g3_waves<BN>::wn, BT, TERMS, IO16>),
+    return hipFuncSetAttribute(reinterpret_cast<const void*>(conv_gemm3_kernel<BM, BN, g3_waves<BN>::wm, g3_waves<BN>::wn, BT, TERMS, IO16, EPI>),
                                hipFuncAttributeMaxDynamicSharedMemorySize, lds);
 }
 
@@ -319,6 +361,12 @@
         if (e == hipSuccess) e = g3_set_attr<128, 128, true, 1, true>();
         if (e == hipSuccess) e = g3_set_attr<128, 64, false, 1, true>();
         if (e == hipSuccess) e = g3_set_attr<128, 64, true, 1, true>();
+        if (e == hipSuccess) e = g3_set_attr<128, 128, false, 3, false, KPX_G3_STATS>();
+        if (e == hipSuccess) e = g3_set_attr<128, 64, false, 3, false, KPX_G3_STATS>();
+        if (e == hipSuccess) e = g3_set_attr<128, 128, true, 3, false, KPX_G3_BNBWD>();
+        if (e == hipSuccess) e = g3_set_attr<128, 64, true, 3, false, KPX_G3_BNBWD>();
+        if (e == hipSuccess) e = g3_set_attr<128, 128, true, 3, false, KPX_G3_BIAS>();
+        if (e == hipSuccess) e = g3_set_attr<128, 64, true, 3, false, KPX_G3_BIAS>();
         if (e != hipSuccess) return -(int)e;
     }
     if (g.ncls <= 0) { g.ncls = 1; g.cls[0] = ConvClass{g.Ha, g.Wa, g.oy0, g.ox0, g.Tr, g.Tq, g.iy0, g.ix0, g.wr0, g.wq0, 0, 0}; }
@@ -331,6 +379,23 @@
     for (int i = 0; i < g.ncls; ++i) { g.cls[i].mt = (g.cls[i].M + BM - 1) / BM; if (g.cls[i].mt > mtmax) mtmax = g.cls[i].mt; }
     g.mt = mtmax;
     const dim3 grid((unsigned)(g.mt * g.nt), (unsigned)g.ncls, (unsigned)(g.ksplit > 1 ? g.ksplit : 1));
+    if (g.epi != KPX_G3_NONE) {
+        const int G = g.st_groups;
+        if (g.io16 || terms != 3 || g.ksplit > 1 || !g.sums || G < 1 || g.N % G != 0 || (g.epi == KPX_G3_STATS) != !bt) return KPX_EINVAL;
+        if (g.epi == KPX_G3_BNBWD && (!g.bn_y || !g.bn_beta || g.ld_bn < g.Cout || g.bias || g.act != KPX_ACT_NONE || g.mul_y)) return KPX_EINVAL;
+        if (g.epi == KPX_G3_BIAS && !g.mul_y) return KPX_EINVAL;
+        g.st_ipg = 0;
+        for (int i = 0; i < g.ncls; ++i) {
+            if (G > 1 && g.cls[i].M % (G * BM) != 0) return KPX_EINVAL;
+            g.st_mtg[i] = g.cls[i].mt / G;
+            g.st_it0[i] = g.st_ipg;
+            g.st_ipg += g.st_mtg[i];
+        }
+        if (g.epi == KPX_G3_STATS) { if (BN == 128) return g3_launch_one<128, 128, false, 3, false, KPX_G3_STATS>(g, grid, s); return g3_launch_one<128, 64, false, 3, false, KPX_G3_STATS>(g, grid, s); }
+        if (g.epi == KPX_G3_BNBWD) { if (BN == 128) return g3_launch_one<128, 128, true, 3, false, KPX_G3_BNBWD>(g, grid, s); return g3_launch_one<128, 64, true, 3, false, KPX_G3_BNBWD>(g, grid, s); }
+        if (g.epi == KPX_G3_BIAS) { if (BN == 128) return g3_launch_one<128, 128, true, 3, false, KPX_G3_BIAS>(g, grid, s); return g3_launch_one<128, 64, true, 3, false, KPX_G3_BIAS>(g, grid, s); }
+        return KPX_EINVAL;
+    }
 #define G3_GO(bn, btv, tv) return g3_launch_one<128, bn, btv, tv>(g, grid, s)
     if (g.io16 & 1) {
         if (BN == 128) { if (bt) return g3_launch_one<128, 128, true, 1, true>(g, grid, s); return g3_launch_one<128, 128, false, 1, true>(g, grid, s); }
diff --git a/unsupervised-keypoint-learning-for-guiding-class-conditional-video-prediction_amd/csrc/conv_geom.h b/unsupervised-keypoint-learning-for-guiding-class-conditional-video-prediction_amd/csrc/conv_geom.h
--- a/unsupervised-keypoint-learning-for-guiding-class-conditional-video-prediction_amd/csrc/conv_geom.h
+++ b/unsupervised-keypoint-learning-for-guiding-class-conditional-video-prediction_amd/csrc/conv_geom.h
@@ -22,7 +22,11 @@
     int terms;
     int merge;
     int io16;
+    int epi; float* sums; const float* bn_y; int ld_bn; const float* bn_beta;
+    int st_groups, st_ipg, st_it0[4], st_mtg[4];
 };
+enum { KPX_G3_NONE = 0, KPX_G3_STATS = 1, KPX_G3_BNBWD = 2, KPX_G3_BIAS = 3 };
+struct G3Sums { int epi; float* sums; const float* bn_y; int ld_bn; const float* bn_beta; int groups; };
 
 
 struct WgradGeom {
diff --git a/unsupervised-keypoint-learning-for-guiding-class-conditional-video-prediction_amd/csrc/conv_igemm.hip b/unsupervised-keypoint-learning-for-guiding-class-conditional-video-prediction_amd/csrc/conv_igemm.hip
--- a/unsupervised-keypoint-learning-for-guiding-class-conditional-video-prediction_amd/csrc/conv_igemm.hip
+++ b/unsupervised-keypoint-learning-for-guiding-class-conditional-video-prediction_amd/csrc/conv_igemm.hip
@@ -478,12 +478,27 @@
 
 static int fwd_impl(const float* x, int N, int Hi, int Wi, int Cin, int ldx, const float* w, int KH, int KW, const float* bias,
                     float* y, int Ho, int Wo, int Cout, int ldy, int stride, int pad_t, int pad_l, int act, int arith, int io16,
-                    void* workspace, size_t workspace_bytes, void* stream);
+                    void* workspace, size_t workspace_bytes, void* stream, const G3Sums* sums = nullptr);
 extern "C" int kpx_conv2d_fwd_f32(const float* x, int N, int Hi, int Wi, int Cin, int ldx,
                                   const float* w, int KH, int KW, const float* bias,
                                   float* y, int Ho, int Wo, int Cout, int ldy,
                                   int stride, int pad_t, int pad_l, int act, int arith, void* workspace, size_t workspace_bytes, void* stream) {
     return fwd_impl(x, N, Hi, Wi, Cin, ldx, w, KH, KW, bias, y, Ho, Wo, Cout, ldy, stride, pad_t, pad_l, act, arith, 0, workspace, workspace_bytes, stream);
+}
+extern "C" size_t kpx_conv2d_sums_items(int N, int H, int W, int stride) {
+    if (N <= 0 || H <= 0 || W <= 0 || stride < 1 || stride > 2) return 0;
+    size_t items = 0;
+    for (int ph = 0; ph < stride && ph < H; ++ph)
+        for (int pw = 0; pw < stride && pw < W; ++pw)
+            items += ((size_t)N * ((H - ph + stride - 1) / stride) * ((W - pw + stride - 1) / stride) + 127) / 128;
+    return 2 * items;
+}
+extern "C" int kpx_conv2d_fwd_stats_f32(const float* x, int N, int Hi, int Wi, int Cin, int ldx, const float* w, int KH, int KW, const float* bias,
+                                        float* y, int Ho, int Wo, int Cout, int ldy, int stride, int pad_t, int pad_l, int arith,
+                                        float* tile_stats, int groups, void* workspace, size_t workspace_bytes, void* stream) {
+    if (!tile_stats || groups < 1 || Cin < 16 || Cout < 16 || (KH == 3 && KW == 3 && stride == 1)) return KPX_EINVAL;
+    const G3Sums sums{KPX_G3_STATS, tile_stats, nullptr, 0, nullptr, groups};
+    return fwd_impl(x, N, Hi, Wi, Cin, ldx, w, KH, KW, bias, y, Ho, Wo, Cout, ldy, stride, pad_t, pad_l, KPX_ACT_NONE, arith, 0, workspace, workspace_bytes, stream, &sums);
 }
 extern "C" int kpx_conv2d_fwd_bf16(const void* x, int N, int Hi, int Wi, int Cin, int ldx, const float* w, int KH, int KW, const float* bias,
                                    void* y, int y_f32, int Ho, int Wo, int Cout, int ldy, int stride, int pad_t, int pad_l, int act,
@@ -494,7 +509,7 @@
 }
 static int fwd_impl(const float* x, int N, int Hi, int Wi, int Cin, int ldx, const float* w, int KH, int KW, const float* bias,
                     float* y, int Ho, int Wo, int Cout, int ldy, int stride, int pad_t, int pad_l, int act, int arith, int io16,
-                    void* workspace, size_t workspace_bytes, void* stream) {
+                    void* workspace, size_t workspace_bytes, void* stream, const G3Sums* sums) {
     if (!x || !w || !y || N <= 0 || Hi <= 0 || Wi <= 0 || Cin <= 0 || Cout <= 0 || Ho <= 0 || Wo <= 0 ||
         KH <= 0 || KW <= 0 || stride <= 0 || ldx < Cin || ldy < Cout || act < 0 || act > 3 || arith < 0 || arith > 1)
         return KPX_EINVAL;
@@ -529,6 +544,10 @@
         g.merge = Cin; g.Tq = 1; g.KW = 1; g.Cin = KW * Cin; g.wts = KW * Cin * Cout; g.vecA = 0;
     }
     if (io16 && !kpx_gemm3_eligible(&g)) return KPX_EINVAL;
+    if (sums) {
+        if (!kpx_gemm3_eligible(&g) || g.terms != 3) return KPX_EINVAL;
+        g.epi = sums->epi; g.sums = sums->sums; g.st_groups = sums->groups;
+    }
     if (!io16 && Cout <= 4 && Cin % 4 == 0 && Cin >= 256 && g.vecA && g.vecB == (Cout == 4))
         return launch_small_cout(g, kpx_stream(stream));
     if (g.vecA && g.vecB && !g.merge && Cin % 4 == 0) {
@@ -536,12 +555,14 @@
         g.ws_slab = (size_t)N * Ho * Wo * Cout;
         if (S > 1 && workspace && workspace_bytes >= (size_t)S * g.ws_slab * 4) { g.ksplit = S; g.ws = (float*)workspace; }
     }
+    if (sums && g.ksplit > 1) return KPX_EINVAL;
     return launch_gather_conv<false>(g, kpx_stream(stream));
 }
 
 static int dgrad_impl(const float* dy, int N, int Ho, int Wo, int Cout, int lddy, const float* w, int KH, int KW,
                       float* dx, int Hi, int Wi, int Cin, int lddx, int stride, int pad_t, int pad_l, int arith,
-                      const float* y_in, int ld_y_in, int act_in, void* workspace, size_t workspace_bytes, void* stream, int io16 = 0);
+                      const float* y_in, int ld_y_in, int act_in, void* workspace, size_t workspace_bytes, void* stream, int io16 = 0,
+                      const G3Sums* sums = nullptr);
 
 extern "C" int kpx_conv2d_dgrad_f32(const float* dy, int N, int Ho, int Wo, int Cout, int lddy,
                                     const float* w, int KH, int KW,
@@ -561,6 +582,25 @@
                       workspace, workspace_bytes, stream);
 }
 
+extern "C" int kpx_conv2d_dgrad_bn_f32(const float* dy, int N, int Ho, int Wo, int Cout, int lddy, const float* w, int KH, int KW,
+                                       float* dx, int Hi, int Wi, int Cin, int lddx, int stride, int pad_t, int pad_l, int arith,
+                                       float* tile_stats, const float* bn_y, int ld_bn_y, const float* bn_beta, int groups,
+                                       void* workspace, size_t workspace_bytes, void* stream) {
+    if (!tile_stats || !bn_y || !bn_beta || ld_bn_y < Cin || groups < 1 || Cin < 16 || Cout < 16 || (KH == 3 && KW == 3 && stride == 1)) return KPX_EINVAL;
+    const G3Sums sums{KPX_G3_BNBWD, tile_stats, bn_y, ld_bn_y, bn_beta, groups};
+    return dgrad_impl(dy, N, Ho, Wo, Cout, lddy, w, KH, KW, dx, Hi, Wi, Cin, lddx, stride, pad_t, pad_l, arith, nullptr, 0, KPX_ACT_NONE,
+                      workspace, workspace_bytes, stream, 0, &sums);
+}
+extern "C" int kpx_conv2d_dgrad_act_sums_f32(const float* dy, int N, int Ho, int Wo, int Cout, int lddy, const float* w, int KH, int KW,
+                                             float* dx, int Hi, int Wi, int Cin, int lddx, int stride, int pad_t, int pad_l, int arith,
+                                             const float* y_in, int ld_y_in, int act_in, float* bias_sums,
+                                             void* workspace, size_t workspace_bytes, void* stream) {
+    if (!bias_sums || !y_in || ld_y_in < Cin || (act_in != KPX_ACT_RELU && act_in != KPX_ACT_LRELU) || Cin < 16 || Cout < 16 || (KH == 3 && KW == 3 && stride == 1)) return KPX_EINVAL;
+    const G3Sums sums{KPX_G3_BIAS, bias_sums, nullptr, 0, nullptr, 1};
+    return dgrad_impl(dy, N, Ho, Wo, Cout, lddy, w, KH, KW, dx, Hi, Wi, Cin, lddx, stride, pad_t, pad_l, arith, y_in, ld_y_in, act_in,
+                      workspace, workspace_bytes, stream, 0, &sums);
+}
+
 extern "C" int kpx_conv_image_fwd_bf16(const float* x, int N, int Hi, int Wi, int Cin, const float* w, int KH, int KW, const float* bias,
                                        void* y, int Ho, int Wo, int Cout, int ldy, int stride, int pad_t, int pad_l, int act, void* stream) {
     if (!x || !w || !y || N <= 0 || Hi <= 0 || Wi <= 0 || Cin <= 0 || Cin > 4 || Cout <= 0 || Cout > 64 || Ho * Wo < 256 || stride < 1 || stride > 2 ||
@@ -594,7 +634,8 @@
 
 static int dgrad_impl(const float* dy, int N, int Ho, int Wo, int Cout, int lddy, const float* w, int KH, int KW,
                       float* dx, int Hi, int Wi, int Cin, int lddx, int stride, int pad_t, int pad_l, int arith,
-                      const float* y_in, int ld_y_in, int act_in, void* workspace, size_t workspace_bytes, void* stream, int io16) {
+                      const float* y_in, int ld_y_in, int act_in, void* workspace, size_t workspace_bytes, void* stream, int io16,
+                      const G3Sums* sums) {
     if (!dy || !w || !dx || N <= 0 || Hi <= 0 || Wi <= 0 || Cin <= 0 || Cout <= 0 || Ho <= 0 || Wo <= 0 ||
         KH <= 0 || KW <= 0 || stride <= 0 || lddy < Cout || lddx < Cin || arith < 0 || arith > 1)
         return KPX_EINVAL;
@@ -642,10 +683,16 @@
         }
     }
     if (io16 && !kpx_gemm3_eligible(&g)) return KPX_EINVAL;
+    if (sums) {
+        if (!kpx_gemm3_eligible(&g) || g.terms != 3) return KPX_EINVAL;
+        g.epi = sums->epi; g.sums = sums->sums; g.st_groups = sums->groups;
+        g.bn_y = sums->bn_y; g.ld_bn = sums->ld_bn; g.bn_beta = sums->bn_beta;
+    }
     if (g.vecA && g.vecB && Cout % 4 == 0) {
         const int S = dgrad_splitk_plan(N, Hi, Wi, Cin, Cout, KH, KW, stride);
         g.ws_slab = (size_t)N * Hi * Wi * Cin;
         if (S > 1 && workspace && workspace_bytes >= (size_t)S * g.ws_slab * 4) { g.ksplit = S; g.ws = (float*)workspace; }
     }
+    if (sums && g.ksplit > 1) return KPX_EINVAL;
     return launch_gather_conv<true>(g, kpx_stream(stream));
 }
diff --git a/unsupervised-keypoint-learning-for-guiding-class-conditional-video-prediction_amd/csrc/pointwise.hip b/unsupervised-keypoint-learning-for-guiding-class-conditional-video-prediction_amd/csrc/pointwise.hip
--- a/unsupervised-keypoint-learning-for-guiding-class-conditional-video-prediction_amd/csrc/pointwise.hip
+++ b/unsupervised-keypoint-learning-for-guiding-class-conditional-video-prediction_amd/csrc/pointwise.hip
@@ -233,6 +233,17 @@
     int nb; int rc = launch_chan_reduce(0, a, &nb, kpx_stream(stream));
     if (rc) return rc;
     hipLaunchKernelGGL(chan_sum_finalize_kernel, dim3(C), dim3(256), 0, kpx_stream(stream), (const double*)scratch, nb, C, sum_out);
+    return kpx_launch_status();
+}
+__global__ __launch_bounds__(256) void chan_items_finalize_kernel(const float* __restrict__ ts, size_t n, int C, float* out) {
+    const int c = blockIdx.x;
+    __shared__ double sm[2][4];
+    chan_wave_sums(nullptr, 0, ts, 0, n, true, C, c, sm);
+    if (threadIdx.x == 0) out[c] = (float)chan_sum4(sm[0]);
+}
+extern "C" int kpx_chan_sum_items_f32(const float* items, size_t n_items, int C, float* sum_out, void* stream) {
+    if (!items || !sum_out || C <= 0 || n_items == 0) return KPX_EINVAL;
+    hipLaunchKernelGGL(chan_items_finalize_kernel, dim3(C), dim3(256), 0, kpx_stream(stream), items, n_items, C, sum_out);
     return kpx_launch_status();
 }
 
diff --git a/unsupervised-keypoint-learning-for-guiding-class-conditional-video-prediction_amd/layers.py b/unsupervised-keypoint-learning-for-guiding-class-conditional-video-prediction_amd/layers.py
--- a/unsupervised-keypoint-learning-for-guiding-class-conditional-video-prediction_amd/layers.py
+++ b/unsupervised-keypoint-learning-for-guiding-class-conditional-video-prediction_amd/layers.py
@@ -12,7 +12,7 @@
 
 
 def conv(x, channels, kernel=4, stride=2, pad=0, use_bias=True, scope='conv_0', act=ACT_NONE, cin=None, head31=False, bias_grad=True, bn_stats=False,
-         f43_fwd=True, input_act=ACT_NONE, act_bwd_by_consumer=False, out_f32=False):
+         f43_fwd=True, input_act=ACT_NONE, act_bwd_by_consumer=False, out_f32=False, bn_groups=1):
     st = default_store()
     channels = int(channels)
     cin_ = int(cin) if cin is not None else int(x.shape[-1])
@@ -29,7 +29,7 @@
     w_, wg = st.param(kname)
     b_, bg = st.param(bname) if use_bias else (None, None)
     return ops.conv2d(x, w_, b_, stride=stride, pad=pad, act=act, cin=cin, w_grad_out=wg, b_grad_out=bg, bias_grad=bias_grad, bn_stats=bn_stats,
-                      input_act=input_act, act_bwd_by_consumer=act_bwd_by_consumer, out_dtype=torch.float32 if out_f32 else None)
+                      input_act=input_act, act_bwd_by_consumer=act_bwd_by_consumer, out_dtype=torch.float32 if out_f32 else None, bn_groups=bn_groups)
 
 
 def conv1x1_keypoints(x, channels, scope='conv_0'):
@@ -74,7 +74,7 @@
             wf, bf = st.folded_conv_bn(kname, bname, names[0], names[1], names[2], names[3], ops.BN_EPS)
             return ops.conv2d(x, wf, bf, stride=stride, pad=0, act=ACT_RELU, cin=cin)
     x = conv(x, channels, kernel=kernel, stride=stride, scope=conv_scope, cin=cin, bias_grad=not (EXACT_ZERO_BIAS_GRAD and train_mode),
-             bn_stats=bool(train_mode), f43_fwd=f43_fwd)
+             bn_stats=bool(train_mode), f43_fwd=f43_fwd, bn_groups=groups)
     if (TRACE is not None or F32_OUT_SCOPES) and not is_sym(x):
         st = default_store()
         with st.variable_scope(conv_scope):
diff --git a/unsupervised-keypoint-learning-for-guiding-class-conditional-video-prediction_amd/ops.py b/unsupervised-keypoint-learning-for-guiding-class-conditional-video-prediction_amd/ops.py
--- a/unsupervised-keypoint-learning-for-guiding-class-conditional-video-prediction_amd/ops.py
+++ b/unsupervised-keypoint-learning-for-guiding-class-conditional-video-prediction_amd/ops.py
@@ -88,6 +88,7 @@
 FUSE_BN_STATS = True
 FUSE_ACT_BWD = True
 FUSE_BN_BWD = True
+FUSE_GEMM3_SUMS = True
 FORK_BEFORE_DGRAD = 'capture'
 _side_streams = {}
 _side_dirty = {}
@@ -125,6 +126,7 @@
     if len(_grad_written) > 4096:
         _grad_written.clear()
     _pending_bwd_stats.clear()
+    _pending_bias_sums.clear()
 
 
 def _claim_grad(dst):
@@ -139,10 +141,11 @@
     _side_keep.clear()
     _pending_stats.clear()
     _pending_bwd_stats.clear()
+    _pending_bias_sums.clear()
 
 
 def graph_knobs():
-    return (_compute_dtype[0], SIDE_WGRAD, FUSE_BN_STATS, FUSE_BN_BWD, FUSE_ACT_BWD, FORK_BEFORE_DGRAD, WINO43, WINO43_MIN_WORKGROUPS, WINO43_NMIN)
+    return (_compute_dtype[0], SIDE_WGRAD, FUSE_BN_STATS, FUSE_BN_BWD, FUSE_GEMM3_SUMS, FUSE_ACT_BWD, FORK_BEFORE_DGRAD, WINO43, WINO43_MIN_WORKGROUPS, WINO43_NMIN)
 
 
 def normalize_device(device):
@@ -528,7 +531,12 @@
     return kh == 3 and kw == 3 and stride == 1 and pad_t == 1 and pad_l == 1 and ho == hi and wo == wi
 
 
-def conv_fwd_raw(x, ldx, cin, w, bias, y, ldy, stride, pad_t, pad_l, act, want_stats=False):
+def _gemm3_items(n, h, wd, stride, c, device):
+    items = lib.kpx_conv2d_sums_items(n, h, wd, stride)
+    return torch.empty(items * 2 * c, dtype=torch.float32, device=device), items
+
+
+def conv_fwd_raw(x, ldx, cin, w, bias, y, ldy, stride, pad_t, pad_l, act, want_stats=False, stat_groups=1):
     n, hi, wi = x.shape[0], x.shape[1], x.shape[2]
     ho, wo = y.shape[1], y.shape[2]
     kh, kw, _, cout = w.shape
@@ -553,6 +561,13 @@
         if y.dtype == BF16:
             yf, ldyf = torch.empty((n, ho, wo, cout), dtype=torch.float32, device=x.device), cout
     r = conv3x3_same(x, ldx, cin, w, bias, yf, ldyf, cout, act, False, want_stats=want_stats) if same3 else None
+    if r is None and want_stats and FUSE_GEMM3_SUMS and not same3 and act == ACT_NONE and yf is y:
+        slab, items = _gemm3_items(n, ho, wo, 1, cout, x.device)
+        if _took(lib.kpx_conv2d_fwd_stats_f32(x.data_ptr(), n, hi, wi, cin, ldx, w.data_ptr(), kh, kw, _ptr(bias), y.data_ptr(), ho, wo, cout, ldy, stride, pad_t, pad_l,
+                                              _arith(), slab.data_ptr(), stat_groups,
+                                              *_workspace('splitk', lib.kpx_conv2d_fwd_workspace_bytes(n, ho, wo, cin, cout, kh, kw), x.device), _stream()),
+                 'kpx_conv2d_fwd_stats_f32'):
+            return (slab, Fraction(items, n), stat_groups)
     if r is None:
         check(lib.kpx_conv2d_fwd_f32(x.data_ptr(), n, hi, wi, cin, ldx, w.data_ptr(), kh, kw, _ptr(bias), yf.data_ptr(), ho, wo, cout, ldyf, stride, pad_t, pad_l, act,
                                      _arith(), *_workspace('splitk', lib.kpx_conv2d_fwd_workspace_bytes(n, ho, wo, cin, cout, kh, kw), x.device), _stream()),
@@ -562,7 +577,7 @@
     return r.stats if r is not None else None
 
 
-def conv_dgrad_raw(dy, lddy, w, dx, lddx, cin, stride, pad_t, pad_l, bn_src=None, mul=None):
+def conv_dgrad_raw(dy, lddy, w, dx, lddx, cin, stride, pad_t, pad_l, bn_src=None, mul=None, bias_sums=None):
     n, ho, wo = dy.shape[0], dy.shape[1], dy.shape[2]
     hi, wi = dx.shape[1], dx.shape[2]
     kh, kw, _, cout = w.shape
@@ -592,7 +607,16 @@
     if r is None:
         ws = _workspace('splitk', lib.kpx_conv2d_dgrad_workspace_bytes(n, hi, wi, cin, cout, kh, kw, stride), dy.device)
         geom = (dy.data_ptr(), n, ho, wo, cout, lddy, w.data_ptr(), kh, kw, dxf.data_ptr(), hi, wi, cin, lddxf, stride, pad_t, pad_l, _arith())
-        if mul is not None:
+        sums = None if (not FUSE_GEMM3_SUMS or same3 or dxf is not dx or dx.dtype != torch.float32) else 'bn' if (bn_src is not None and mul is None) else 'bias' if (mul is not None and bias_sums is not None) else None
+        if sums is not None:
+            slab, items = _gemm3_items(n, hi, wi, stride, cin, dy.device)
+        if sums == 'bn' and _took(lib.kpx_conv2d_dgrad_bn_f32(*geom, slab.data_ptr(), bn_src[0].data_ptr(), bn_src[0].shape[3], bn_src[1].data_ptr(),
+                                                              bn_src[2] if len(bn_src) > 2 else 1, *ws, _stream()), 'kpx_conv2d_dgrad_bn_f32'):
+            return (slab, Fraction(items, n))
+        if sums == 'bias' and _took(lib.kpx_conv2d_dgrad_act_sums_f32(*geom, mul[0].data_ptr(), mul[0].shape[3], mul[1], slab.data_ptr(), *ws, _stream()),
+                                    'kpx_conv2d_dgrad_act_sums_f32'):
+            bias_sums.append((slab, items))
+        elif mul is not None:
             check(lib.kpx_conv2d_dgrad_act_f32(*geom, mul[0].data_ptr(), mul[0].shape[3], mul[1], *ws, _stream()), 'kpx_conv2d_dgrad_act_f32')
         else:
             check(lib.kpx_conv2d_dgrad_f32(*geom, *ws, _stream()), 'kpx_conv2d_dgrad_f32')
@@ -705,7 +729,7 @@
         pl, _, wo = same_pad(wd + 2 * pad, kw, stride)
         pad_t, pad_l = pad + pt, pad + pl
         y = torch.empty((n, ho, wo, cout), dtype=out_dtype if out_dtype is not None else act_dtype(), device=x.device)
-        st = conv_fwd_raw(x, ldx, cin, w, b, y, cout, stride, pad_t, pad_l, act, want_stats=bn_stats and act == ACT_NONE)
+        st = conv_fwd_raw(x, ldx, cin, w, b, y, cout, stride, pad_t, pad_l, act, want_stats=bool(bn_stats) and act == ACT_NONE, stat_groups=int(bn_stats) or 1)
         if st is not None:
             _pending_stats[y.data_ptr()] = st
         ctx.geom = (stride, pad_t, pad_l, act, cin, ldx)
@@ -728,6 +752,9 @@
         want_w = ctx.needs_input_grad[1]
         want_b = ctx.has_bias and ctx.needs_input_grad[2]
         dy_sum = dy
+        bsum = _pending_bias_sums.pop(dy.data_ptr(), None) if ctx.act_bwd_by_consumer else None
+        if bsum is not None and (bsum[2].shape != dy.shape or tuple(bsum[0].shape) != (bsum[1] * 2 * cout,)):
+            bsum = None
         if (dy.dtype == torch.float32 and x.dtype == BF16 and cout < 8 and w.shape[0] == 3 and w.shape[1] == 3 and stride == 1
                 and ctx.input_act == ACT_NONE):
             dy16 = torch.empty((dy.shape[0], dy.shape[1], dy.shape[2], 8), dtype=BF16, device=dy.device)
@@ -745,9 +772,12 @@
             dx = torch.empty(x.shape, dtype=x.dtype, device=x.device)
             if cin < cx:
                 fill_raw_(dx, 0.0)
+            got_bias = [] if (FUSE_BN_BWD and ctx.input_act != ACT_NONE) else None
             st = conv_dgrad_raw(dy, lddy, w, dx, cx, cin, stride, pad_t, pad_l,
-                                bn_src=(x, ctx.bn_src[0]) if ctx.bn_src is not None else None,
-                                mul=(x, ctx.input_act) if ctx.input_act != ACT_NONE else None)
+                                bn_src=(x, ctx.bn_src[0], ctx.bn_src[2]) if ctx.bn_src is not None else None,
+                                mul=(x, ctx.input_act) if ctx.input_act != ACT_NONE else None, bias_sums=got_bias)
+            if got_bias:
+                _pending_bias_sums[dx.data_ptr()] = (got_bias[0][0], got_bias[0][1], dx)
             if st is not None:
                 _pending_bwd_stats[dx.data_ptr()] = (st[0], st[1], ctx.bn_src[1], dx)
         if side:
@@ -757,7 +787,7 @@
                 st.wait_event(fork)
             else:
                 st.wait_stream(main)
-            _side_keep.append((dy, dy_sum, x))
+            _side_keep.append((dy, dy_sum, x, bsum))
             _side_dirty[skey] = True
             stream_ctx = torch.cuda.stream(st)
         else:
@@ -774,7 +804,11 @@
             if want_b:
                 direct = ctx.b_grad_out is not None and _claim_grad(ctx.b_grad_out)
                 db_buf = ctx.b_grad_out if direct else torch.empty(cout, dtype=torch.float32, device=x.device)
-                chan_sum_raw(dy_sum, cout, dy.shape[0] * dy.shape[1] * dy.shape[2], cout, db_buf)
+                if bsum is not None:
+                    fused_bias_uses['bias_sums_from_dgrad_epilogue'] += 1
+                    check(lib.kpx_chan_sum_items_f32(bsum[0].data_ptr(), bsum[1], cout, db_buf.data_ptr(), _stream()), 'kpx_chan_sum_items_f32')
+                else:
+                    chan_sum_raw(dy_sum, cout, dy.shape[0] * dy.shape[1] * dy.shape[2], cout, db_buf)
                 if ctx.b_grad_out is not None and not direct:
                     axpy_raw_(ctx.b_grad_out, db_buf)
                 db = None if ctx.b_grad_out is not None else db_buf
@@ -783,13 +817,15 @@
 
 _pending_stats = {}
 _pending_bwd_stats = {}
+_pending_bias_sums = {}
+fused_bias_uses = {'bias_sums_from_dgrad_epilogue': 0}
 _bn_counter = [0]
 fused_bn_uses = {'stats_from_conv_epilogue': 0, 'backward_sums_from_dgrad_epilogue': 0}
 
 
 def conv2d(x, w, b=None, stride=1, pad=0, act=ACT_NONE, cin=None, w_grad_out=None, b_grad_out=None, bias_grad=True, bn_stats=False,
-           input_act=ACT_NONE, act_bwd_by_consumer=False, out_dtype=None):
-    y = Conv2dFn.apply(x, w, b, w_grad_out, b_grad_out, stride, pad, act, cin, bias_grad, bn_stats and FUSE_BN_STATS,
+           input_act=ACT_NONE, act_bwd_by_consumer=False, out_dtype=None, bn_groups=1):
+    y = Conv2dFn.apply(x, w, b, w_grad_out, b_grad_out, stride, pad, act, cin, bias_grad, int(bn_groups) if (bn_stats and FUSE_BN_STATS) else 0,
                        getattr(x, '_kpx_bn', None) if FUSE_BN_BWD else None, input_act if FUSE_ACT_BWD else ACT_NONE,
                        act_bwd_by_consumer and FUSE_ACT_BWD, out_dtype)
     if bn_stats:
@@ -826,7 +862,7 @@
             sc = scratch.get('bn%d' % groups, lib.kpx_bn_train_scratch_bytes(c, groups), dev)
             slab_ptr, tpg = None, 0
             if tile_stats is not None:
-                slab, tpi = tile_stats
+                slab, tpi = tile_stats[0], tile_stats[1]
                 fused_bn_uses['stats_from_conv_epilogue'] += groups
                 slab_ptr, tpg = slab.data_ptr(), int(ng * tpi)
             entry = 'kpx_bn_train_fwd_bf16' if ctx.x16 else 'kpx_bn_train_fwd_f32'
@@ -887,12 +923,13 @@
 def batch_norm(x, gamma, beta, moving_mean, moving_var, train=True, act=ACT_RELU, groups=1, update_moving=True,
                g_grad_out=None, b_grad_out=None, out_f32=False):
     ts = getattr(x, '_kpx_tile_stats', None) if train else None
-    if ts is not None and (x.shape[0] % groups or tuple(ts[0].shape) != (x.shape[0] * ts[1] * 2 * x.shape[3],) or not _whole_tiles_per_group(x.shape[0], groups, ts[1])):
+    if ts is not None and (x.shape[0] % groups or tuple(ts[0].shape) != (x.shape[0] * ts[1] * 2 * x.shape[3],) or not _whole_tiles_per_group(x.shape[0], groups, ts[1])
+                           or (len(ts) > 2 and ts[2] != groups)):
         ts = None
     _bn_counter[0] += 1
     y = BatchNormFn.apply(x, gamma, beta, moving_mean, moving_var, g_grad_out, b_grad_out, train, act, groups, update_moving, ts, _bn_counter[0], out_f32)
     if train and act == ACT_RELU:
-        y._kpx_bn = (beta.detach(), _bn_counter[0])
+        y._kpx_bn = (beta.detach(), _bn_counter[0], groups)
     return y
 
 
```

Result: no change. 1415 (-0.1%).
